# dalek-cryptography/curve25519-dalek

Hardware: NVIDIA H100
Metric: Pippenger MSM points/sec (higher is better)
Workload: dtype exact integers: f64 limbs (radix 2^51, FP64 pipe) in the bucket kernel, u32 limbs (radix 2^25.5) elsewhere

## Files before the change

curve25519_dalek_b200/csrc/api.cu:

```cuda
#include <cstring>
#include <new>
#include <random>

#include "../../include/dalek_b200.h"
#include "engine.h"

extern "C" {

int dalek_b200_init(int device, dalek_b200_ctx **out)
{
    if (!out) return DALEK_E_INVALID_ARG;
    *out = nullptr;
    int count = 0;
    if (cudaGetDeviceCount(&count) != cudaSuccess || count <= 0 || device < 0 || device >= count) return DALEK_E_NO_DEVICE;
    cudaDeviceProp prop;
    if (cudaGetDeviceProperties(&prop, device) != cudaSuccess) return DALEK_E_NO_DEVICE;
    if (prop.major != 9 || prop.minor != 0) return DALEK_E_NO_DEVICE;
    if (cudaSetDevice(device) != cudaSuccess) return DALEK_E_CUDA;
    dalek_b200_ctx *ctx = new (std::nothrow) dalek_b200_ctx();
    if (!ctx) return DALEK_E_NOMEM;
    ctx->device = device;
    ctx->sm_count = prop.multiProcessorCount;
    try { std::random_device rd; for (int i = 0; i < 4; i++) ctx->hash_seed[i] ^= rd(); } catch (...) { }
    int prio_lo = 0, prio_hi = 0;
    cudaDeviceGetStreamPriorityRange(&prio_lo, &prio_hi);
    if (cudaStreamCreateWithPriority(&ctx->stream, cudaStreamNonBlocking, prio_hi) != cudaSuccess ||
        cudaStreamCreateWithPriority(&ctx->stream2, cudaStreamNonBlocking, prio_lo) != cudaSuccess ||
        cudaStreamCreateWithFlags(&ctx->stream_copy, cudaStreamNonBlocking) != cudaSuccess ||
        cudaStreamCreateWithPriority(&ctx->stream3, cudaStreamNonBlocking, prio_hi) != cudaSuccess ||
        cudaStreamCreateWithPriority(&ctx->stream_hash, cudaStreamNonBlocking, prio_hi) != cudaSuccess ||
        cudaEventCreate(&ctx->ev_a) != cudaSuccess || cudaEventCreate(&ctx->ev_b) != cudaSuccess ||
        cudaEventCreate(&ctx->ev_call0) != cudaSuccess || cudaEventCreate(&ctx->ev_call1) != cudaSuccess ||
        cudaEventCreateWithFlags(&ctx->ev_fork, cudaEventDisableTiming) != cudaSuccess ||
        cudaEventCreateWithFlags(&ctx->ev_join, cudaEventDisableTiming) != cudaSuccess ||
        cudaEventCreateWithFlags(&ctx->ev_join2, cudaEventDisableTiming) != cudaSuccess) {
        delete ctx;
        return DALEK_E_CUDA;
    }
    for (int i = 0; i < 8; i++)
        if (cudaEventCreateWithFlags(&ctx->ev_grp[i], cudaEventDisableTiming) != cudaSuccess ||
            cudaEventCreateWithFlags(&ctx->ev_hram[i], cudaEventDisableTiming) != cudaSuccess || cudaEventCreate(&ctx->ev_prep[i][0]) != cudaSuccess ||
            cudaEventCreate(&ctx->ev_prep[i][1]) != cudaSuccess) { delete ctx; return DALEK_E_CUDA; }
    *out = ctx;
    return DALEK_OK;
}

void dalek_b200_destroy(dalek_b200_ctx *ctx)
{
    if (!ctx) return;
    cudaSetDevice(ctx->device);
    cudaStreamSynchronize(ctx->stream);
    cudaStreamSynchronize(ctx->stream2);
    cudaStreamSynchronize(ctx->stream3);
    cudaStreamSynchronize(ctx->stream_hash);
    DevBuf *bufs[] = {&ctx->scalars, &ctx->points_in, &ctx->points, &ctx->digits, &ctx->counts, &ctx->offsets,
                      &ctx->sorted, &ctx->buckets, &ctx->red_a, &ctx->red_b, &ctx->red_c, &ctx->red_d, &ctx->key_pts,
                      &ctx->result, &ctx->flags, &ctx->misc0, &ctx->misc1, &ctx->misc2, &ctx->misc3,
                      &ctx->misc4, &ctx->misc5, &ctx->zs, &ctx->base_table, &ctx->ntasks, &ctx->task_off, &ctx->tasks, &ctx->task_sums, &ctx->msg_offs, &ctx->sum_desc, &ctx->sum_part, &ctx->key_table, &ctx->key_acc, &ctx->task_order, &ctx->sig_status, &ctx->misc6, &ctx->each_pow, &ctx->each_tab, &ctx->each_kstat, &ctx->comb_base_table, &ctx->prep_prod, &ctx->mb_ws[0], &ctx->mb_ws[1]};
    for (DevBuf *b : bufs) if (b->p) cudaFree(b->p);
    if (ctx->h_pinned) cudaFreeHost(ctx->h_pinned);
    cudaEventDestroy(ctx->ev_a); cudaEventDestroy(ctx->ev_b); cudaEventDestroy(ctx->ev_fork); cudaEventDestroy(ctx->ev_join);
    cudaEventDestroy(ctx->ev_join2); cudaEventDestroy(ctx->ev_call0); cudaEventDestroy(ctx->ev_call1);
    for (int i = 0; i < 8; i++) { cudaEventDestroy(ctx->ev_grp[i]); cudaEventDestroy(ctx->ev_hram[i]); cudaEventDestroy(ctx->ev_prep[i][0]); cudaEventDestroy(ctx->ev_prep[i][1]); }
    cudaStreamDestroy(ctx->stream_hash);
    cudaStreamDestroy(ctx->stream); cudaStreamDestroy(ctx->stream2); cudaStreamDestroy(ctx->stream_copy); cudaStreamDestroy(ctx->stream3);
    delete ctx;
}

const char *dalek_b200_last_error(const dalek_b200_ctx *ctx) { return ctx ? ctx->last_error.c_str() : "null context"; }

int dalek_b200_set_option(dalek_b200_ctx *ctx, const char *name, long value)
{
    if (!ctx || !name) return DALEK_E_INVALID_ARG;
    if (!strcmp(name, "window_bits")) { if (value != 0 && (value < 4 || value > 20)) return DALEK_E_INVALID_ARG; ctx->opt_window_bits = value; return 0; }
    if (!strcmp(name, "host_chunks")) { if (value < 1 || value > 8) return DALEK_E_INVALID_ARG; ctx->opt_host_chunks = value; return 0; }
    if (!strcmp(name, "decompress_f64")) { ctx->opt_decompress_f64 = value ? 1 : 0; return 0; }
    if (!strcmp(name, "trace")) { ctx->opt_trace = value ? 1 : 0; return 0; }
    if (!strcmp(name, "precomp_tables")) { ctx->opt_precomp_tables = value ? 1 : 0; return 0; }
    if (!strcmp(name, "double_base_comb")) { ctx->opt_double_base_comb = value ? 1 : 0; return 0; }
    if (!strcmp(name, "dedupe_keys")) { ctx->opt_dedupe_keys = value ? 1 : 0; return 0; }
    if (!strcmp(name, "verify_pieces")) { if (value < 1 || value > 8) return DALEK_E_INVALID_ARG; ctx->opt_verify_pieces = value; return 0; }
    if (!strcmp(name, "transcript_warp")) { ctx->opt_transcript_warp = value ? 1 : 0; return 0; }
    if (!strcmp(name, "transcript_blocks")) { ctx->opt_transcript_blocks = value ? 1 : 0; return 0; }
    if (!strcmp(name, "each_comb")) { if (value < 0 || value > 2) return DALEK_E_INVALID_ARG; ctx->opt_each_comb = value; return 0; }
    if (!strcmp(name, "small_straus")) { ctx->opt_small_straus = value ? 1 : 0; return 0; }
    if (!strcmp(name, "acc_tma")) { ctx->opt_acc_tma = value ? 1 : 0; return 0; }
    if (!strcmp(name, "field_f64")) { ctx->opt_field_f64 = value ? 1 : 0; return 0; }
    if (!strcmp(name, "verify_chunk")) { if (value < 0 || value > (1 << 20)) return DALEK_E_INVALID_ARG; ctx->opt_verify_chunk = value; return 0; }
    return DALEK_E_INVALID_ARG;
}

uint64_t dalek_b200_launch_count(const dalek_b200_ctx *ctx) { return ctx ? ctx->launches : 0; }

int dalek_b200_last_kernel_ms(const dalek_b200_ctx *ctx, float *ms, int *launches)
{
    if (!ctx) return DALEK_E_INVALID_ARG;
    if (ms) *ms = ctx->last_kernel_ms;
    if (launches) *launches = ctx->last_kernel_launches;
    return 0;
}

int dalek_b200_last_stage_ms(const dalek_b200_ctx *ctx, const char *stage, float *ms)
{
    if (!ctx || !stage || !ms) return DALEK_E_INVALID_ARG;
    if (!strcmp(stage, "bucket_accumulate")) { *ms = ctx->last_kernel_ms; return 0; }
    if (!strcmp(stage, "decompress_R")) { *ms = ctx->last_prep_ms; return 0; }
    return DALEK_E_INVALID_ARG;
}

int dalek_b200_last_call_ms(const dalek_b200_ctx *ctx, float *ms)
{
    if (!ctx || !ms) return DALEK_E_INVALID_ARG;
    *ms = ctx->last_call_ms;
    return 0;
}

}

static int run_msm(dalek_b200_ctx *ctx, const void *scalars, const void *points_in, bool on_device, int point_fmt, size_t n,
                   size_t n_window ,
                   ge_p3_raw *d_windows, MsmResult *d_result)
{
    int rc;
    const size_t pin = msm_point_bytes(point_fmt);
    cudaStream_t st = ctx->stream;
    const int c = msm_choose_window_bits(ctx, n_window);
    const bool straus = d_result && n == n_window && n < STRAUS_VT_THRESHOLD && ctx->opt_small_straus && ctx->opt_field_f64;
    const int kind = msm_prepared_kind(point_fmt, straus ? PK_PNIELS : PK_NIELS);
    const size_t psz = kind == PK_NIELS ? sizeof(ge_niels_packed) : sizeof(ge_pniels_packed);
    if ((rc = ws_reserve(ctx, ctx->points, std::max<size_t>(1, n) * psz))) return rc;
    if ((rc = ws_reserve(ctx, ctx->flags, 64))) return rc;
    CUDA_TRY(ctx, cudaMemsetAsync(ctx->flags.p, 0, 64, st));
    if (on_device) {
        if (straus) {
            if ((rc = msm_prepare_points(ctx, points_in, point_fmt, n, ctx->points.p, (int *)ctx->flags.p, kind))) return rc;
            if ((rc = straus_vartime_msm(ctx, (const uint32_t *)scalars, ctx->points.p, kind, n, d_result))) return rc;
        } else {
            CUDA_TRY(ctx, cudaEventRecord(ctx->ev_fork, st));
            CUDA_TRY(ctx, cudaStreamWaitEvent(ctx->stream2, ctx->ev_fork, 0));
            if ((rc = msm_prepare_points_on(ctx, ctx->stream2, points_in, point_fmt, n, ctx->points.p, (int *)ctx->flags.p))) return rc;
            CUDA_TRY(ctx, cudaEventRecord(ctx->ev_join, ctx->stream2));
            if ((rc = msm_accumulate_chunk(ctx, (const uint32_t *)scalars, (const ge_niels_packed *)ctx->points.p, n, c, true, 0, 0, ctx->ev_join))) return rc;
        }
    } else {
        if ((rc = ws_reserve(ctx, ctx->scalars, std::max<size_t>(1, n) * 32))) return rc;
        if ((rc = ws_reserve(ctx, ctx->points_in, std::max<size_t>(1, n) * pin))) return rc;
        int K = n >= (1u << 18) ? (int)std::min<long>(8, std::max<long>(1, ctx->opt_host_chunks)) : 1;
        CUDA_TRY(ctx, cudaEventRecord(ctx->ev_fork, st));
        CUDA_TRY(ctx, cudaStreamWaitEvent(ctx->stream_copy, ctx->ev_fork, 0));
        CUDA_TRY(ctx, cudaStreamWaitEvent(ctx->stream2, ctx->ev_fork, 0));
        for (int k = 0; k < K; k++) {
            const size_t i0 = n * k / K, i1 = n * (k + 1) / K, cnt = i1 - i0;
            char *ds = (char *)ctx->scalars.p + i0 * 32, *dp = (char *)ctx->points_in.p + i0 * pin;
            if (cnt) {
                CUDA_TRY(ctx, cudaMemcpyAsync(ds, (const char *)scalars + i0 * 32, cnt * 32, cudaMemcpyHostToDevice, ctx->stream_copy));
                CUDA_TRY(ctx, cudaMemcpyAsync(dp, (const char *)points_in + i0 * pin, cnt * pin, cudaMemcpyHostToDevice, ctx->stream_copy));
            }
            CUDA_TRY(ctx, cudaEventRecord(ctx->ev_grp[k], ctx->stream_copy));
            CUDA_TRY(ctx, cudaStreamWaitEvent(st, ctx->ev_grp[k], 0));
            char *dq = (char *)ctx->points.p + i0 * psz;
            if (straus) {
                if ((rc = msm_prepare_points(ctx, dp, point_fmt, cnt, dq, (int *)ctx->flags.p, kind))) return rc;
                if ((rc = straus_vartime_msm(ctx, (const uint32_t *)ds, dq, kind, cnt, d_result))) return rc;
            } else {
                CUDA_TRY(ctx, cudaStreamWaitEvent(ctx->stream2, ctx->ev_grp[k], 0));
                if ((rc = msm_prepare_points_on(ctx, ctx->stream2, dp, point_fmt, cnt, dq, (int *)ctx->flags.p))) return rc;
                CUDA_TRY(ctx, cudaEventRecord(ctx->ev_join, ctx->stream2));
                if ((rc = msm_accumulate_chunk(ctx, (const uint32_t *)ds, (const ge_niels_packed *)dq, cnt, c, k == 0, 0, 0, ctx->ev_join))) return rc;
            }
        }
    }
    if (!straus && (rc = msm_reduce_finish(ctx, c, d_windows, d_result))) return rc;
    return 0;
}

int msm_read_result(dalek_b200_ctx *ctx, const MsmResult *d_result, const int *d_bad, const uint32_t *d_enc,
                    uint8_t out_compressed[32], uint64_t out_limbs[20])
{
    int rc;
    cudaStream_t st = ctx->stream;
    if ((rc = pinned_reserve(ctx, sizeof(MsmResult) + 128))) return rc;
    MsmResult *h = (MsmResult *)ctx->h_pinned;
    int *h_bad = (int *)((char *)ctx->h_pinned + sizeof(MsmResult));
    uint8_t *h_enc = (uint8_t *)ctx->h_pinned + sizeof(MsmResult) + 64;
    CUDA_TRY(ctx, cudaMemcpyAsync(h, d_result, sizeof(MsmResult), cudaMemcpyDeviceToHost, st));
    CUDA_TRY(ctx, cudaMemcpyAsync(h_bad, d_bad, sizeof(int), cudaMemcpyDeviceToHost, st));
    if (d_enc) CUDA_TRY(ctx, cudaMemcpyAsync(h_enc, d_enc, 32, cudaMemcpyDeviceToHost, st));
    CUDA_TRY(ctx, cudaStreamSynchronize(st));
    float ms = 0.f;
    if ((ms = elapsed_ms(ctx->ev_a, ctx->ev_b)) >= 0.f) ctx->last_kernel_ms = ms;
    if (out_compressed) memcpy(out_compressed, d_enc ? h_enc : (const uint8_t *)h->compressed, 32);
    if (out_limbs) memcpy(out_limbs, h->limbs, 160);
    return *h_bad ? DALEK_NONE : DALEK_OK;
}

int msm_whole(dalek_b200_ctx *ctx, const void *scalars, const void *points, bool on_device, int point_fmt, size_t n,
              uint8_t out_compressed[32], uint64_t out_limbs[20])
{
    int rc;
    const int nwin = msm_window_count_for_bits(msm_choose_window_bits(ctx, n));
    if ((rc = ws_reserve(ctx, ctx->misc0, (size_t)nwin * sizeof(ge_p3_raw)))) return rc;
    if ((rc = ws_reserve(ctx, ctx->result, sizeof(MsmResult) + 32))) return rc;
    MsmResult *d_res = (MsmResult *)ctx->result.p;
    uint32_t *d_enc = point_fmt == DALEK_POINTS_RISTRETTO ? (uint32_t *)(d_res + 1) : nullptr;
    if ((rc = run_msm(ctx, scalars, points, on_device, point_fmt, n, n, (ge_p3_raw *)ctx->misc0.p, d_res))) return rc;
    if (d_enc && (rc = ristretto_encode_result(ctx, d_res, d_enc))) return rc;
    return msm_read_result(ctx, d_res, (const int *)ctx->flags.p, d_enc, out_compressed, out_limbs);
}

static int msm_common(dalek_b200_ctx *ctx, const void *scalars, const void *points, bool on_device, int point_fmt,
                      size_t n, uint8_t out_compressed[32], uint64_t out_limbs[20])
{
    if (!ctx || (n && (!scalars || !points)) || n >= (1ull << 31)) return DALEK_E_INVALID_ARG;
    CUDA_TRY(ctx, cudaSetDevice(ctx->device));
    CallTimer timer(ctx);
    return msm_whole(ctx, scalars, points, on_device, point_fmt, n, out_compressed, out_limbs);
}

static bool edwards_format(int point_fmt) { return point_fmt == DALEK_POINTS_COMPRESSED || point_fmt == DALEK_POINTS_EXTENDED; }

extern "C" {

int dalek_b200_edwards_vartime_msm(dalek_b200_ctx *ctx, const uint8_t *scalars, const void *points, int point_fmt,
                                   size_t n, uint8_t out_compressed[32], uint64_t out_limbs[20])
{
    if (!edwards_format(point_fmt)) return DALEK_E_INVALID_ARG;
    return msm_common(ctx, scalars, points, false, point_fmt, n, out_compressed, out_limbs);
}

int dalek_b200_edwards_vartime_msm_dev(dalek_b200_ctx *ctx, const void *d_scalars, const void *d_points, int point_fmt,
                                       size_t n, uint8_t out_compressed[32], uint64_t out_limbs[20])
{
    if (!edwards_format(point_fmt)) return DALEK_E_INVALID_ARG;
    return msm_common(ctx, d_scalars, d_points, true, point_fmt, n, out_compressed, out_limbs);
}

int dalek_b200_ristretto_vartime_msm(dalek_b200_ctx *ctx, const uint8_t *scalars, const uint8_t *points, size_t n,
                                     uint8_t out_compressed[32])
{
    if (!out_compressed) return DALEK_E_INVALID_ARG;
    return msm_common(ctx, scalars, points, false, DALEK_POINTS_RISTRETTO, n, out_compressed, nullptr);
}

int dalek_b200_msm_window_count(dalek_b200_ctx *ctx, size_t n_shard)
{
    if (!ctx) return DALEK_E_INVALID_ARG;
    return msm_window_count_for_bits(msm_choose_window_bits(ctx, n_shard));
}

size_t dalek_b200_msm_partial_bytes(dalek_b200_ctx *ctx, size_t n_shard)
{
    if (!ctx) return 0;
    return (size_t)msm_window_count_for_bits(msm_choose_window_bits(ctx, n_shard)) * 160 + 8;
}

void *dalek_b200_stream(dalek_b200_ctx *ctx) { return ctx ? (void *)ctx->stream : nullptr; }

}

__global__ void k_windows_to_record(const ge_p3_raw *__restrict__ win, int nwin, const int *__restrict__ bad, uint64_t *__restrict__ out)
{
    int w = blockIdx.x * blockDim.x + threadIdx.x;
    if (w == nwin) out[20 * (size_t)nwin] = (uint64_t)(*bad != 0);
    if (w >= nwin) return;
    ge_p3 p; ge_p3_raw r = win[w]; ge_p3_load_raw(p, r);
    fe_to_limbs51(out + 20 * w, p.X); fe_to_limbs51(out + 20 * w + 5, p.Y);
    fe_to_limbs51(out + 20 * w + 10, p.Z); fe_to_limbs51(out + 20 * w + 15, p.T);
}
__global__ void k_records_to_windows(const uint64_t *__restrict__ in, int ranks, int nwin, size_t rec_words,
                                     ge_p3_raw *__restrict__ win, int *__restrict__ any_bad)
{
    int t = blockIdx.x * blockDim.x + threadIdx.x;
    if (t >= ranks * nwin) return;
    const int r = t / nwin, w = t % nwin;
    const uint64_t *src = in + (size_t)r * rec_words + 20 * (size_t)w;
    ge_p3 p;
    fe_from_limbs51(p.X, src); fe_from_limbs51(p.Y, src + 5); fe_from_limbs51(p.Z, src + 10); fe_from_limbs51(p.T, src + 15);
    ge_p3_raw o; ge_p3_store_raw(o, p); win[t] = o;
    if (w == 0 && rec_words > 20 * (size_t)nwin && in[(size_t)r * rec_words + 20 * (size_t)nwin]) atomicOr(any_bad, 1);
}

static int partial_enqueue(dalek_b200_ctx *ctx, const void *scalars, const void *points, bool on_device, int point_fmt,
                           size_t n_local, size_t n_shard, int *nwin_out)
{
    if (!ctx || (n_local && (!scalars || !points)) || n_local > n_shard || !edwards_format(point_fmt) || n_local >= (1ull << 31))
        return DALEK_E_INVALID_ARG;
    CUDA_TRY(ctx, cudaSetDevice(ctx->device));
    int rc;
    const int c = msm_choose_window_bits(ctx, n_shard);
    const int nwin = msm_window_count_for_bits(c);
    if ((rc = ws_reserve(ctx, ctx->misc0, (size_t)nwin * sizeof(ge_p3_raw)))) return rc;
    if ((rc = ws_reserve(ctx, ctx->misc1, (size_t)nwin * 160 + 8))) return rc;
    if ((rc = run_msm(ctx, scalars, points, on_device, point_fmt, n_local, n_shard, (ge_p3_raw *)ctx->misc0.p, nullptr))) return rc;
    k_windows_to_record<<<(nwin + 1 + 63) / 64, 64, 0, ctx->stream>>>((const ge_p3_raw *)ctx->misc0.p, nwin, (const int *)ctx->flags.p,
                                                                     (uint64_t *)ctx->misc1.p);
    ctx->launches++;
    CUDA_TRY(ctx, cudaGetLastError());
    *nwin_out = nwin;
    return 0;
}

static void read_kernel_ms(dalek_b200_ctx *ctx)
{
    float ms = 0.f;
    if ((ms = elapsed_ms(ctx->ev_a, ctx->ev_b)) >= 0.f) ctx->last_kernel_ms = ms;
}

static int partial_common(dalek_b200_ctx *ctx, const void *scalars, const void *points, bool on_device, int point_fmt,
                          size_t n_local, size_t n_shard, uint64_t *out_windows)
{
    if (!ctx || !out_windows) return DALEK_E_INVALID_ARG;
    CallTimer timer(ctx);
    int rc, nwin = 0;
    if ((rc = partial_enqueue(ctx, scalars, points, on_device, point_fmt, n_local, n_shard, &nwin))) return rc;
    const size_t bytes = (size_t)nwin * 160 + 8;
    if ((rc = pinned_reserve(ctx, bytes))) return rc;
    CUDA_TRY(ctx, cudaMemcpyAsync(ctx->h_pinned, ctx->misc1.p, bytes, cudaMemcpyDeviceToHost, ctx->stream));
    CUDA_TRY(ctx, cudaStreamSynchronize(ctx->stream));
    read_kernel_ms(ctx);
    memcpy(out_windows, ctx->h_pinned, (size_t)nwin * 160);
    uint64_t status; memcpy(&status, (const char *)ctx->h_pinned + (size_t)nwin * 160, 8);
    return status ? DALEK_NONE : DALEK_OK;
}

int msm_partial_enqueue_record(dalek_b200_ctx *ctx, const void *scalars, const void *points, bool on_device, int point_fmt,
                               size_t n_local, size_t n_shard, void *d_out_record, int dst_device)
{
    if (!ctx || !d_out_record) return DALEK_E_INVALID_ARG;
    CUDA_TRY(ctx, cudaSetDevice(ctx->device));
    CUDA_TRY(ctx, cudaEventRecord(ctx->ev_call0, ctx->stream));
    ctx->async_open = true;
    int rc, nwin = 0;
    if ((rc = partial_enqueue(ctx, scalars, points, on_device, point_fmt, n_local, n_shard, &nwin))) return rc;
    if (dst_device >= 0 && dst_device != ctx->device)
        CUDA_TRY(ctx, cudaMemcpyPeerAsync(d_out_record, dst_device, ctx->misc1.p, ctx->device, (size_t)nwin * 160 + 8, ctx->stream));
    else
        CUDA_TRY(ctx, cudaMemcpyAsync(d_out_record, ctx->misc1.p, (size_t)nwin * 160 + 8, cudaMemcpyDeviceToDevice, ctx->stream));
    return DALEK_OK;
}

int msm_combine_records(dalek_b200_ctx *ctx, const void *records, bool on_device, size_t rec_bytes, int ranks, size_t n_shard,
                        uint8_t out_compressed[32], uint64_t out_limbs[20])
{
    if (!ctx || !records || ranks < 1 || ranks > 1024) return DALEK_E_INVALID_ARG;
    CUDA_TRY(ctx, cudaSetDevice(ctx->device));
    int rc;
    const int c = msm_choose_window_bits(ctx, n_shard);
    const int nwin = msm_window_count_for_bits(c);
    const size_t cnt = (size_t)ranks * nwin;
    if ((rc = ws_reserve(ctx, ctx->red_c, cnt * sizeof(ge_p3_raw)))) return rc;
    if ((rc = ws_reserve(ctx, ctx->flags, 64))) return rc;
    if ((rc = ws_reserve(ctx, ctx->result, sizeof(MsmResult)))) return rc;
    if ((rc = pinned_reserve(ctx, sizeof(MsmResult) + 64))) return rc;
    cudaStream_t st = ctx->stream;
    const void *d_rec = records;
    if (!on_device) {
        if ((rc = ws_reserve(ctx, ctx->red_d, (size_t)ranks * rec_bytes))) return rc;
        CUDA_TRY(ctx, cudaMemcpyAsync(ctx->red_d.p, records, (size_t)ranks * rec_bytes, cudaMemcpyHostToDevice, st));
        d_rec = ctx->red_d.p;
    }
    int *d_bad = (int *)ctx->flags.p + 8;
    CUDA_TRY(ctx, cudaMemsetAsync(d_bad, 0, 4, st));
    k_records_to_windows<<<(unsigned)((cnt + 63) / 64), 64, 0, st>>>((const uint64_t *)d_rec, ranks, nwin, rec_bytes / 8,
                                                                      (ge_p3_raw *)ctx->red_c.p, d_bad);
    ctx->launches++;
    if ((rc = msm_combine_windows(ctx, (const ge_p3_raw *)ctx->red_c.p, ranks, nwin, c, (MsmResult *)ctx->result.p))) return rc;
    MsmResult *h = (MsmResult *)ctx->h_pinned;
    int *h_bad = (int *)((char *)ctx->h_pinned + sizeof(MsmResult));
    CUDA_TRY(ctx, cudaMemcpyAsync(h, ctx->result.p, sizeof(MsmResult), cudaMemcpyDeviceToHost, st));
    CUDA_TRY(ctx, cudaMemcpyAsync(h_bad, d_bad, 4, cudaMemcpyDeviceToHost, st));
    if (ctx->async_open) CUDA_TRY(ctx, cudaEventRecord(ctx->ev_call1, st));
    CUDA_TRY(ctx, cudaStreamSynchronize(st));
    if (ctx->async_open) {
        float ms = 0.f;
        if ((ms = elapsed_ms(ctx->ev_call0, ctx->ev_call1)) >= 0.f) ctx->last_call_ms = ms;
        read_kernel_ms(ctx);
        ctx->async_open = false;
    }
    if (out_compressed) memcpy(out_compressed, h->compressed, 32);
    if (out_limbs) memcpy(out_limbs, h->limbs, 160);
    return *h_bad ? DALEK_NONE : DALEK_OK;
}

extern "C" {

int dalek_b200_edwards_msm_partial(dalek_b200_ctx *ctx, const uint8_t *scalars, const void *points, int point_fmt,
                                   size_t n_local, size_t n_shard, uint64_t *out_windows)
{
    return partial_common(ctx, scalars, points, false, point_fmt, n_local, n_shard, out_windows);
}

int dalek_b200_edwards_msm_partial_dev(dalek_b200_ctx *ctx, const void *d_scalars, const void *d_points, int point_fmt,
                                       size_t n_local, size_t n_shard, uint64_t *out_windows)
{
    return partial_common(ctx, d_scalars, d_points, true, point_fmt, n_local, n_shard, out_windows);
}

int dalek_b200_edwards_msm_partial_async(dalek_b200_ctx *ctx, const uint8_t *scalars, const void *points, int point_fmt,
                                         size_t n_local, size_t n_shard, void *d_out_record)
{
    return msm_partial_enqueue_record(ctx, scalars, points, false, point_fmt, n_local, n_shard, d_out_record, -1);
}

int dalek_b200_edwards_msm_partial_dev_async(dalek_b200_ctx *ctx, const void *d_scalars, const void *d_points, int point_fmt,
                                             size_t n_local, size_t n_shard, void *d_out_record)
{
    return msm_partial_enqueue_record(ctx, d_scalars, d_points, true, point_fmt, n_local, n_shard, d_out_record, -1);
}

int dalek_b200_edwards_msm_combine(dalek_b200_ctx *ctx, const uint64_t *windows, int ranks, size_t n_shard,
                                   uint8_t out_compressed[32], uint64_t out_limbs[20])
{
    if (!ctx) return DALEK_E_INVALID_ARG;
    const size_t rec = (size_t)msm_window_count_for_bits(msm_choose_window_bits(ctx, n_shard)) * 160;
    return msm_combine_records(ctx, windows, false, rec, ranks, n_shard, out_compressed, out_limbs);
}

int dalek_b200_edwards_msm_combine_dev(dalek_b200_ctx *ctx, const void *d_records, int ranks, size_t n_shard,
                                       uint8_t out_compressed[32], uint64_t out_limbs[20])
{
    if (!ctx) return DALEK_E_INVALID_ARG;
    return msm_combine_records(ctx, d_records, true, dalek_b200_msm_partial_bytes(ctx, n_shard), ranks, n_shard, out_compressed, out_limbs);
}

}
```

curve25519_dalek_b200/csrc/engine.h:

```cpp
#pragma once
#include <cuda_runtime.h>
#include <stddef.h>
#include <stdint.h>
#include <cstdio>
#include <string>
#include <utility>
#include <vector>

#include "../../include/dalek_b200.h"
#include "ge.cuh"

struct DevBuf {
    void *p = nullptr;
    size_t cap = 0;
};

struct dalek_b200_ctx {
    int device = 0;
    int sm_count = 132;
    cudaStream_t stream = nullptr;
    cudaStream_t stream2 = nullptr;
    cudaStream_t stream_copy = nullptr;
    cudaStream_t stream3 = nullptr;
    cudaStream_t stream_hash = nullptr;
    cudaEvent_t ev_hram[8] = {};
    cudaEvent_t ev_a = nullptr, ev_b = nullptr, ev_fork = nullptr, ev_join = nullptr, ev_join2 = nullptr;
    cudaEvent_t ev_call0 = nullptr, ev_call1 = nullptr;
    cudaEvent_t ev_prep[8][2] = {};
    int prep_pieces = 0;
    float last_prep_ms = 0.f;
    cudaEvent_t ev_grp[8] = {nullptr, nullptr, nullptr, nullptr, nullptr, nullptr, nullptr, nullptr};
    std::string last_error;
    uint64_t launches = 0;
    long opt_window_bits = 0;
    long opt_verify_chunk = 0;
    long opt_host_chunks = 8;
    long opt_trace = 0;
    long opt_precomp_tables = 0;
    long opt_double_base_comb = 1;
    long opt_dedupe_keys = 1;
    long opt_verify_pieces = 4;
    long opt_decompress_f64 = 1;
    long opt_acc_tma = 0;
    long opt_transcript_warp = 1;
    long opt_transcript_blocks = 1;
    long opt_each_comb = 1;
    long opt_small_straus = 1;
    long opt_field_f64 = 1;
    float last_kernel_ms = 0.f;
    float last_call_ms = 0.f;
    int last_kernel_launches = 0;
    bool async_open = false;
    DevBuf scalars, points_in, points, digits, counts, offsets, sorted, buckets, red_a, red_b, red_c,
        red_d, key_pts, result, flags, misc0, misc1, misc2, misc3, misc4, misc5, zs, base_table, ntasks, task_off, tasks, task_sums, msg_offs, sum_desc, sum_part, key_table, key_acc, task_order, sig_status, misc6, each_pow, each_tab, each_kstat;
    DevBuf prep_prod;
    uint32_t hash_seed[4] = {0x243F6A88u, 0x85A308D3u, 0x13198A2Eu, 0x03707344u};
    int sum_desc_c = -1;
    bool base_table_ready = false;
    bool each_attr_set = false;
    bool comb_attr_set = false;
    DevBuf comb_base_table;
    bool comb_base_table_ready = false;
    DevBuf mb_ws[2];
    void *h_pinned = nullptr;
    size_t h_pinned_cap = 0;
    size_t last_zs_n = 0;
    std::vector<std::pair<const char *, cudaEvent_t>> trace;
};

#define CUDA_TRY(ctx, expr)                                                                      \
    do {                                                                                         \
        cudaError_t _e = (expr);                                                                 \
        if (_e != cudaSuccess) {                                                                 \
            (ctx)->last_error = std::string(#expr) + ": " + cudaGetErrorString(_e);              \
            return -3;                                                                           \
        }                                                                                        \
    } while (0)

inline float elapsed_ms(cudaEvent_t a, cudaEvent_t b)
{
    float ms = 0.f;
    if (cudaEventElapsedTime(&ms, a, b) == cudaSuccess) return ms;
    cudaGetLastError();
    return -1.f;
}

struct CallTimer {
    dalek_b200_ctx *ctx;
    explicit CallTimer(dalek_b200_ctx *c) : ctx(c) { if (ctx) cudaEventRecord(ctx->ev_call0, ctx->stream); }
    ~CallTimer()
    {
        if (!ctx) return;
        float ms = 0.f;
        if (cudaEventRecord(ctx->ev_call1, ctx->stream) == cudaSuccess && cudaEventSynchronize(ctx->ev_call1) == cudaSuccess &&
            (ms = elapsed_ms(ctx->ev_call0, ctx->ev_call1)) >= 0.f)
            ctx->last_call_ms = ms;
    }
};

inline void trace_mark(dalek_b200_ctx *ctx, const char *name, cudaStream_t st)
{
    if (!ctx->opt_trace) return;
    cudaEvent_t e;
    if (cudaEventCreate(&e) != cudaSuccess) return;
    cudaEventRecord(e, st);
    ctx->trace.push_back({name, e});
}
inline void trace_dump(dalek_b200_ctx *ctx)
{
    if (!ctx->opt_trace) return;
    cudaDeviceSynchronize();
    for (auto &m : ctx->trace) {
        float ms = 0.f;
        cudaEventElapsedTime(&ms, ctx->ev_call0, m.second);
        fprintf(stderr, "[trace] %8.3f ms  %s\n", ms, m.first);
        cudaEventDestroy(m.second);
    }
    ctx->trace.clear();
}

inline bool flat_messages_ok(const uint8_t *msgs_flat, const uint64_t *offsets, size_t n)
{
    if (!n) return true;
    if (!offsets || offsets[0] != 0) return false;
    for (size_t i = 0; i < n; i++)
        if (offsets[i] > offsets[i + 1]) return false;
    return msgs_flat || offsets[n] == 0;
}

int ws_reserve(dalek_b200_ctx *ctx, DevBuf &b, size_t bytes);
int pinned_reserve(dalek_b200_ctx *ctx, size_t bytes);

enum { PK_NIELS = 0 , PK_PNIELS = 1  };

inline size_t msm_point_bytes(int point_fmt) { return point_fmt == DALEK_POINTS_EXTENDED ? 160 : 32; }

int msm_prepare_points(dalek_b200_ctx *ctx, const void *d_in, int point_fmt, size_t n, void *d_out,
                       int *d_bad, int kind = PK_NIELS);
int msm_prepared_kind(int point_fmt, int kind);

int msm_choose_window_bits(const dalek_b200_ctx *ctx, size_t n);
int msm_window_count_for_bits(int c);

struct MsmResult { uint32_t compressed[8]; uint64_t limbs[20]; uint32_t is_identity; uint32_t pad; };
int msm_accumulate_chunk(dalek_b200_ctx *ctx, const uint32_t *d_scalars, const ge_niels_packed *d_points, size_t n,
                         int c, bool first, int active_windows = 0, size_t flat = 0, cudaEvent_t points_ready = nullptr);
int msm_prepare_points_on(dalek_b200_ctx *ctx, cudaStream_t st, const void *d_in, int point_fmt, size_t n, void *d_out, int *d_bad,
                          int kind = PK_NIELS);
int msm_choose_window_bits_mixed(const dalek_b200_ctx *ctx, size_t n_short, int short_bits, size_t n_long);
int msm_reduce_finish(dalek_b200_ctx *ctx, int c, ge_p3_raw *d_windows, MsmResult *d_result, bool flat = false);
int msm_combine_windows(dalek_b200_ctx *ctx, const ge_p3_raw *d_windows, int ranks, int nwin, int c,
                        MsmResult *d_result);
int msm_read_result(dalek_b200_ctx *ctx, const MsmResult *d_result, const int *d_bad, const uint32_t *d_enc,
                    uint8_t out_compressed[32], uint64_t out_limbs[20]);

int msm_whole(dalek_b200_ctx *ctx, const void *scalars, const void *points, bool on_device, int point_fmt, size_t n,
              uint8_t out_compressed[32], uint64_t out_limbs[20]);

int msm_partial_enqueue_record(dalek_b200_ctx *ctx, const void *scalars, const void *points, bool on_device, int point_fmt,
                               size_t n_local, size_t n_shard, void *d_out_record, int dst_device);
int msm_combine_records(dalek_b200_ctx *ctx, const void *records, bool on_device, size_t rec_bytes, int ranks, size_t n_shard,
                        uint8_t out_compressed[32], uint64_t out_limbs[20]);

struct EachFront { const uint32_t *hs; const uint8_t *bad_s; const uint32_t *rep, *dense, *uniq; size_t nkeys; };
struct Sha512Prefix;
int verify_each_front(dalek_b200_ctx *ctx, const uint8_t *d_msgs, const uint64_t *d_offs, const uint32_t *d_sigs, const uint32_t *d_keys,
                      size_t n, EachFront *out, const Sha512Prefix *ph_dom = nullptr);

#define STRAUS_VT_THRESHOLD 190
int straus_vartime_msm(dalek_b200_ctx *ctx, const uint32_t *d_scalars, const void *d_points, int point_kind, size_t n,
                       MsmResult *d_result);

int straus_ct_msm(dalek_b200_ctx *ctx, const uint32_t *d_scalars, const void *d_points_pniels, size_t n,
                  MsmResult *d_result);
int base_table_ensure(dalek_b200_ctx *ctx);
#define COMB_BASE_DOUBLES (64 * 8 * 15)
int comb_base_table_ensure(dalek_b200_ctx *ctx);

int ristretto_encode_result(dalek_b200_ctx *ctx, const MsmResult *d_res, uint32_t *d_enc);
```

curve25519_dalek_b200/csrc/msm.cu:

```cuda
#include <algorithm>
#include <cstdio>
#include <utility>
#include <vector>

#include "../../include/dalek_b200.h"
#include "engine.h"
#include "ge64.cuh"
#include "warp4.cuh"
#include "warp4_f64.cuh"

static inline unsigned cdiv(size_t a, unsigned b) { return (unsigned)((a + b - 1) / b); }

int ws_reserve(dalek_b200_ctx *ctx, DevBuf &b, size_t bytes)
{
    if (bytes <= b.cap) return 0;
    if (b.p) { cudaFree(b.p); b.p = nullptr; b.cap = 0; }
    size_t want = bytes + bytes / 8 + 256;
    cudaError_t e = cudaMalloc(&b.p, want);
    if (e != cudaSuccess) { ctx->last_error = std::string("cudaMalloc: ") + cudaGetErrorString(e); return DALEK_E_NOMEM; }
    b.cap = want;
    return 0;
}

int pinned_reserve(dalek_b200_ctx *ctx, size_t bytes)
{
    if (bytes <= ctx->h_pinned_cap) return 0;
    if (ctx->h_pinned) cudaFreeHost(ctx->h_pinned);
    ctx->h_pinned = nullptr; ctx->h_pinned_cap = 0;
    cudaError_t e = cudaMallocHost(&ctx->h_pinned, bytes + 4096);
    if (e != cudaSuccess) { ctx->last_error = std::string("cudaMallocHost: ") + cudaGetErrorString(e); return DALEK_E_NOMEM; }
    ctx->h_pinned_cap = bytes + 4096;
    return 0;
}

template <int F64>
__global__ void __launch_bounds__(128, 3) k_prep_compressed(const uint4 *__restrict__ in, ge_niels_packed *__restrict__ out, size_t n,
                                  int *__restrict__ bad)
{
    size_t i = (size_t)blockIdx.x * blockDim.x + threadIdx.x;
    if (i >= n) return;
    uint4 a = in[2 * i], b = in[2 * i + 1];
    uint32_t s[8] = {a.x, a.y, a.z, a.w, b.x, b.y, b.z, b.w};
    fe x, y;
    uint32_t ok = ge_decompress_affine<F64>(x, y, s);
    if (!ok) { atomicOr(bad, 1); fe_0(x); fe_1(y); }
    ge_niels nl; ge_affine_to_niels(nl, x, y);
    ge_niels_packed p; ge_niels_pack(p, nl);
    uint4 *o = reinterpret_cast<uint4 *>(out + i);
#pragma unroll
    for (int k = 0; k < 6; k++) o[k] = make_uint4(p.w[4 * k], p.w[4 * k + 1], p.w[4 * k + 2], p.w[4 * k + 3]);
}

template <int F64>
__global__ void k_prep_ristretto(const uint32_t *__restrict__ in, ge_niels_packed *__restrict__ out, size_t n, int *__restrict__ bad)
{
    size_t i = (size_t)blockIdx.x * blockDim.x + threadIdx.x;
    if (i >= n) return;
    uint32_t enc[8];
#pragma unroll
    for (int k = 0; k < 8; k++) enc[k] = in[8 * i + k];
    ge_p3 P;
    if (!ristretto_decompress<F64>(P, enc)) { atomicOr(bad, 1); ge_p3_identity(P); }
    ge_niels nl; ge_affine_to_niels(nl, P.X, P.Y);
    ge_niels_packed pk; ge_niels_pack(pk, nl);
    out[i] = pk;
}

#define PREP_THREADS 256
#define PREP_PER_THREAD 4
#define PREP_GROUP (PREP_THREADS * PREP_PER_THREAD)
#define PREP_NW (PREP_THREADS / 32)

__device__ __forceinline__ void load_coord_f64(fe64 &h, const uint64_t *__restrict__ src)
{
    uint64_t l[5];
#pragma unroll
    for (int k = 0; k < 5; k++) l[k] = __ldg(src + k);
    fe t; fe_from_limbs51(t, l);
    fe64_from_fe_limbs(h, t);
}
__device__ __forceinline__ void store_coord(uint4 *o, const fe64 &v, uint32_t ok, uint32_t c)
{
    fe f;
    uint32_t w[8];
    fe64_to_fe(f, v); fe_tobytes_words(w, f);
#pragma unroll
    for (int q = 0; q < 8; q++) w[q] = ok ? w[q] : (q == 0 ? c : 0u);
    o[0] = make_uint4(w[0], w[1], w[2], w[3]);
    o[1] = make_uint4(w[4], w[5], w[6], w[7]);
}
__device__ __forceinline__ uint32_t load_z(fe64 &h, const uint64_t *__restrict__ in, size_t i)
{
    uint64_t l[5];
#pragma unroll
    for (int k = 0; k < 5; k++) l[k] = __ldg(in + 20 * i + 10 + k);
    fe t; fe_from_limbs51(t, l);
    fe64_from_fe_limbs(h, t);
    return 1u - (uint32_t)fe_iszero(t);
}
__device__ __forceinline__ void fe64_shfl_up(fe64 &o, const fe64 &f, int d)
{
#pragma unroll
    for (int k = 0; k < 5; k++) o.v[k] = __shfl_up_sync(0xffffffffu, f.v[k], d);
}
__device__ __forceinline__ void fe64_shfl_down(fe64 &o, const fe64 &f, int d)
{
#pragma unroll
    for (int k = 0; k < 5; k++) o.v[k] = __shfl_down_sync(0xffffffffu, f.v[k], d);
}
__device__ __forceinline__ void fe64_shfl_xor(fe64 &o, const fe64 &f, int m)
{
#pragma unroll
    for (int k = 0; k < 5; k++) o.v[k] = __shfl_xor_sync(0xffffffffu, f.v[k], m);
}
__device__ __forceinline__ void fe64_shfl_idx(fe64 &o, const fe64 &f, int src)
{
#pragma unroll
    for (int k = 0; k < 5; k++) o.v[k] = __shfl_sync(0xffffffffu, f.v[k], src);
}

__device__ __forceinline__ void warp_product(fe64 &p, const fe64 &x, int width)
{
    fe64 t;
    p = x;
#pragma unroll 1
    for (int m = width >> 1; m > 0; m >>= 1) { fe64_shfl_xor(t, p, m); fe64_mul(p, p, t); }
}

__device__ __forceinline__ void warp_other_products(const fe64 &x, fe64 &below, fe64 &above, fe64 &all)
{
    const uint32_t lane = threadIdx.x & 31;
    fe64 lo = x, hi = x, t;
#pragma unroll 1
    for (int d = 1; d < 32; d <<= 1) {
        fe64_shfl_up(t, lo, d);
        if (lane >= (uint32_t)d) fe64_mul(lo, lo, t);
        fe64_shfl_down(t, hi, d);
        if (lane + d < 32) fe64_mul(hi, hi, t);
    }
    fe64_shfl_idx(all, lo, 31);
    fe64_shfl_up(below, lo, 1); if (lane == 0) fe64_1(below);
    fe64_shfl_down(above, hi, 1); if (lane == 31) fe64_1(above);
}

template <bool INVERT>
__device__ __forceinline__ void block_inverse(fe64 &inv, const fe64 &acc, fe64 *s_warp, const fe64 *tot_inv)
{
    const uint32_t lane = threadIdx.x & 31, warp = threadIdx.x >> 5, nw = blockDim.x >> 5;
    fe64 below, above, all;
    warp_other_products(acc, below, above, all);
    if (lane == 0) s_warp[warp] = all;
    __syncthreads();
    if (warp == 0) {
        fe64 x, b, a, t;
        if (lane < nw) x = s_warp[lane]; else fe64_1(x);
        warp_other_products(x, b, a, all);
        if (INVERT) {
            const w20_role r = w20_roles();
            const double inv = w20_invert(w20_limb(all, r.i), r);
#pragma unroll
            for (uint32_t k = 0; k < 5; k++) t.v[k] = w20_shfl(inv, k);
        } else {
            t = *tot_inv;
        }
        fe64_mul(t, t, b); fe64_mul(t, t, a);
        if (lane < nw) s_warp[lane] = t;
    }
    __syncthreads();
    fe64_mul(inv, s_warp[warp], below); fe64_mul(inv, inv, above);
}

__global__ void __launch_bounds__(PREP_THREADS, 2)
k_prep_zprod(const uint64_t *__restrict__ in, fe64 *__restrict__ prod, size_t n)
{
    __shared__ fe64 s_warp[PREP_NW];
    const uint32_t tid = threadIdx.x, lane = tid & 31, warp = tid >> 5;
    const size_t g0 = (size_t)blockIdx.x * PREP_GROUP + tid;
    fe64 z[PREP_PER_THREAD], acc, t;
    uint32_t ok[PREP_PER_THREAD];
#pragma unroll
    for (int k = 0; k < PREP_PER_THREAD; k++) {
        const size_t i = g0 + (size_t)k * PREP_THREADS;
        if (i < n) ok[k] = load_z(z[k], in, i); else { ok[k] = 0; fe64_1(z[k]); }
    }
    acc = z[0];
    if (!ok[0]) fe64_1(acc);
#pragma unroll
    for (int k = 1; k < PREP_PER_THREAD; k++) { fe64_mul(t, acc, z[k]); fe64_cmov(acc, t, ok[k]); }
    warp_product(t, acc, 32);
    if (lane == 0) s_warp[warp] = t;
    __syncthreads();
    if (warp == 0) {
        if (lane < PREP_NW) acc = s_warp[lane]; else fe64_1(acc);
        warp_product(t, acc, PREP_NW);
        if (lane == 0) prod[blockIdx.x] = t;
    }
}

__global__ void __launch_bounds__(PREP_THREADS)
k_prep_invert(fe64 *__restrict__ prod, fe64 *__restrict__ pre, uint32_t G)
{
    __shared__ fe64 s_warp[PREP_NW];
    const uint32_t per = (G + blockDim.x - 1) / blockDim.x, b = min(threadIdx.x * per, G), e = min(b + per, G);
    fe64 acc, inv, t;
    fe64_1(acc);
    for (uint32_t k = b; k < e; k++) { fe64_mul(acc, acc, prod[k]); pre[k] = acc; }
    block_inverse<true>(inv, acc, s_warp, nullptr);
    for (uint32_t k = e; k-- > b;) {
        const fe64 x = prod[k];
        if (k > b) fe64_mul(t, inv, pre[k - 1]); else t = inv;
        prod[k] = t;
        fe64_mul(inv, inv, x);
    }
}

__global__ void __launch_bounds__(PREP_THREADS, 2)
k_prep_finish(const uint64_t *__restrict__ in, const fe64 *__restrict__ ginv, ge_niels_packed *__restrict__ out, size_t n)
{
    __shared__ fe64 s_warp[PREP_NW];
    __shared__ fe64 s_pre[PREP_PER_THREAD - 1][PREP_THREADS];
    const uint32_t tid = threadIdx.x;
    const size_t g0 = (size_t)blockIdx.x * PREP_GROUP + tid;
    fe64 acc, inv;
    uint32_t nz = 0;
    fe64_1(acc);
#pragma unroll 1
    for (int k = 0; k < PREP_PER_THREAD; k++) {
        const size_t i = g0 + (size_t)k * PREP_THREADS;
        if (k > 0) s_pre[k - 1][tid] = acc;
        if (i < n) {
            fe64 z, t;
            const uint32_t ok = load_z(z, in, i);
            fe64_mul(t, acc, z); fe64_cmov(acc, t, ok);
            nz |= ok << k;
        }
    }
    block_inverse<false>(inv, acc, s_warp, ginv + blockIdx.x);
#pragma unroll 1
    for (int k = PREP_PER_THREAD - 1; k >= 0; k--) {
        const size_t i = g0 + (size_t)k * PREP_THREADS;
        if (i >= n) continue;
        const uint32_t ok = (nz >> k) & 1u;
        const uint64_t *src = in + 20 * i;
        fe64 X, Y, zi, u, v;
        load_coord_f64(u, src + 10);
        if (k > 0) fe64_mul(zi, inv, s_pre[k - 1][tid]); else zi = inv;
        fe64_mul(v, inv, u); fe64_cmov(inv, v, ok);
        uint4 *o = reinterpret_cast<uint4 *>(out + i);
        load_coord_f64(X, src); load_coord_f64(Y, src + 5);
        fe64_add(u, Y, X); fe64_mul(v, u, zi);
        store_coord(o, v, ok, 1u);
        fe64_sub(u, Y, X); fe64_mul(v, u, zi);
        store_coord(o + 2, v, ok, 1u);
        load_coord_f64(u, src + 15);
        fe64_mul(v, u, zi); fe64_const_2d(u); fe64_mul(v, v, u);
        store_coord(o + 4, v, ok, 0u);
    }
}

__global__ void k_prep_extended_pniels(const uint64_t *__restrict__ in, ge_pniels_packed *__restrict__ out, size_t n)
{
    size_t i = (size_t)blockIdx.x * blockDim.x + threadIdx.x;
    if (i >= n) return;
    const ulonglong2 *src = reinterpret_cast<const ulonglong2 *>(in + 20 * i);
    uint64_t l[20];
#pragma unroll
    for (int k = 0; k < 10; k++) { ulonglong2 v = src[k]; l[2 * k] = v.x; l[2 * k + 1] = v.y; }
    ge_p3 p;
    fe_from_limbs51(p.X, l); fe_from_limbs51(p.Y, l + 5); fe_from_limbs51(p.Z, l + 10); fe_from_limbs51(p.T, l + 15);
    ge_pniels pn; ge_p3_to_pniels(pn, p);
    ge_pniels_packed pk; ge_pniels_pack(pk, pn);
    uint4 *o = reinterpret_cast<uint4 *>(out + i);
#pragma unroll
    for (int k = 0; k < 8; k++) o[k] = make_uint4(pk.w[4 * k], pk.w[4 * k + 1], pk.w[4 * k + 2], pk.w[4 * k + 3]);
}

int msm_prepared_kind(int point_fmt, int kind)
{
    return point_fmt == DALEK_POINTS_EXTENDED ? kind : PK_NIELS;
}

int msm_prepare_points_on(dalek_b200_ctx *ctx, cudaStream_t st, const void *d_in, int point_fmt, size_t n, void *d_out, int *d_bad,
                          int kind)
{
    if (n == 0) return 0;
    if (point_fmt == DALEK_POINTS_COMPRESSED) {
        if (ctx->opt_decompress_f64) k_prep_compressed<1><<<cdiv(n, 128), 128, 0, st>>>((const uint4 *)d_in, (ge_niels_packed *)d_out, n, d_bad);
        else k_prep_compressed<0><<<cdiv(n, 128), 128, 0, st>>>((const uint4 *)d_in, (ge_niels_packed *)d_out, n, d_bad);
    } else if (point_fmt == DALEK_POINTS_RISTRETTO) {
        if (ctx->opt_decompress_f64) k_prep_ristretto<1><<<cdiv(n, 128), 128, 0, st>>>((const uint32_t *)d_in, (ge_niels_packed *)d_out, n, d_bad);
        else k_prep_ristretto<0><<<cdiv(n, 128), 128, 0, st>>>((const uint32_t *)d_in, (ge_niels_packed *)d_out, n, d_bad);
    } else if (kind == PK_PNIELS) {
        k_prep_extended_pniels<<<cdiv(n, 128), 128, 0, st>>>((const uint64_t *)d_in, (ge_pniels_packed *)d_out, n);
    } else {
        const unsigned G = cdiv(n, PREP_GROUP);
        int rc;
        if ((rc = ws_reserve(ctx, ctx->prep_prod, 2 * (size_t)G * sizeof(fe64)))) return rc;
        fe64 *prod = (fe64 *)ctx->prep_prod.p;
        k_prep_zprod<<<G, PREP_THREADS, 0, st>>>((const uint64_t *)d_in, prod, n);
        k_prep_invert<<<1, PREP_THREADS, 0, st>>>(prod, prod + G, G);
        k_prep_finish<<<G, PREP_THREADS, 0, st>>>((const uint64_t *)d_in, prod, (ge_niels_packed *)d_out, n);
        ctx->launches += 2;
    }
    ctx->launches++;
    CUDA_TRY(ctx, cudaGetLastError());
    return 0;
}

int msm_prepare_points(dalek_b200_ctx *ctx, const void *d_in, int point_fmt, size_t n, void *d_out, int *d_bad, int kind)
{
    return msm_prepare_points_on(ctx, ctx->stream, d_in, point_fmt, n, d_out, d_bad, kind);
}

int msm_window_count_for_bits(int c) { return 256 / c + 1; }

int msm_choose_window_bits(const dalek_b200_ctx *ctx, size_t n)
{
    if (ctx->opt_window_bits >= 4 && ctx->opt_window_bits <= 20) return (int)ctx->opt_window_bits;
    int best = 4; double best_cost = 1e300;
    for (int c = 4; c <= 20; c++) {
        double W = (double)((253 + c - 1) / c);
        double cost = W * ((double)n + 4.0 * (double)(1u << (c - 1)));
        if (cost < best_cost) { best_cost = cost; best = c; }
    }
    return best;
}

int msm_choose_window_bits_mixed(const dalek_b200_ctx *ctx, size_t n_short, int short_bits, size_t n_long)
{
    if (ctx->opt_window_bits >= 4 && ctx->opt_window_bits <= 20) return (int)ctx->opt_window_bits;
    int best = 4; double best_cost = 1e300;
    for (int c = 4; c <= 20; c++) {
        double W = (double)((253 + c - 1) / c), Ws = (double)((short_bits + 1 + c - 1) / c);
        double cost = Ws * (double)n_short + W * ((double)n_long + 4.0 * (double)(1u << (c - 1)));
        if (cost < best_cost) { best_cost = cost; best = c; }
    }
    return best;
}

#define SORT_THREADS 512
#define SORT_COUNT_TILE 4096u
#define SORT_TILE 2048u
#define SORT_HIST_MAX 8192u
#define SORT_NC_MAX 4096u
#define SORT_FINE_MAX 12
#define SORT_BIN_MEAN 4096u
#define SORT_FINE_CAP 8192u

__device__ __forceinline__ int32_t next_digit(uint32_t s[8], uint32_t &carry, int c)
{
    const uint32_t v = (s[0] & ((1u << c) - 1)) + carry;
#pragma unroll
    for (int k = 0; k < 7; k++) s[k] = __funnelshift_r(s[k], s[k + 1], c);
    s[7] >>= c;
    if (v > (1u << (c - 1))) { carry = 1; return (int32_t)v - (int32_t)(1u << c); }
    carry = 0;
    return (int32_t)v;
}

__device__ __forceinline__ void load_scalar(uint32_t s[8], const uint4 *__restrict__ scalars, size_t i)
{
    const uint4 a = scalars[2 * i], b = scalars[2 * i + 1];
    s[0] = a.x; s[1] = a.y; s[2] = a.z; s[3] = a.w; s[4] = b.x; s[5] = b.y; s[6] = b.z; s[7] = b.w;
}

__device__ uint32_t block_excl_scan(uint32_t *v, uint32_t len, uint32_t *scr)
{
    const uint32_t t = threadIdx.x, lane = t & 31, wid = t >> 5, nw = blockDim.x >> 5;
    const uint32_t per = (len + blockDim.x - 1) / blockDim.x, b = min(t * per, len), e = min(b + per, len);
    __syncthreads();
    uint32_t sum = 0;
    for (uint32_t k = b; k < e; k++) sum += v[k];
    uint32_t incl = sum;
    for (int d = 1; d < 32; d <<= 1) { uint32_t x = __shfl_up_sync(0xffffffffu, incl, d); if (lane >= (uint32_t)d) incl += x; }
    if (lane == 31) scr[wid] = incl;
    __syncthreads();
    if (wid == 0) {
        const uint32_t x = lane < nw ? scr[lane] : 0;
        uint32_t y = x;
        for (int d = 1; d < 32; d <<= 1) { uint32_t z = __shfl_up_sync(0xffffffffu, y, d); if (lane >= (uint32_t)d) y += z; }
        if (lane < nw) scr[lane] = y - x;
        if (lane == 31) scr[32] = y;
    }
    __syncthreads();
    uint32_t run = scr[wid] + incl - sum;
    for (uint32_t k = b; k < e; k++) { const uint32_t x = v[k]; v[k] = run; run += x; }
    const uint32_t total = scr[32];
    __syncthreads();
    return total;
}

__device__ __forceinline__ uint32_t warp_claim(uint32_t *ctr, uint32_t key, bool live)
{
    const uint32_t lane = threadIdx.x & 31;
    const uint32_t peers = __match_any_sync(0xffffffffu, live ? key : 0xffffffffu);
    const uint32_t leader = __ffs(peers) - 1;
    uint32_t base = 0;
    if (live && lane == leader) base = atomicAdd(&ctr[key], (uint32_t)__popc(peers));
    base = __shfl_sync(0xffffffffu, base, leader);
    return base + __popc(peers & ((1u << lane) - 1));
}

__global__ void __launch_bounds__(SORT_THREADS)
k_sort_count(const uint4 *__restrict__ scalars, size_t n, int c, int nact, int F, uint32_t nc, int flat,
             uint32_t *__restrict__ ccount)
{
    __shared__ uint32_t h[SORT_HIST_MAX];
    const uint32_t nh = (flat ? 1u : (uint32_t)nact) * nc;
    for (uint32_t k = threadIdx.x; k < nh; k += SORT_THREADS) h[k] = 0;
    __syncthreads();
    for (uint32_t j = 0; j < SORT_COUNT_TILE / SORT_THREADS; j++) {
        const size_t i = (size_t)blockIdx.x * SORT_COUNT_TILE + j * SORT_THREADS + threadIdx.x;
        if (i >= n) break;
        uint32_t s[8], carry = 0;
        load_scalar(s, scalars, i);
        for (int w = 0; w < nact; w++) {
            const int32_t d = next_digit(s, carry, c);
            if (d) atomicAdd(&h[(flat ? 0u : (uint32_t)w * nc) + (((uint32_t)(d < 0 ? -d : d) - 1) >> F)], 1u);
        }
    }
    __syncthreads();
    for (uint32_t k = threadIdx.x; k < nh; k += SORT_THREADS)
        if (h[k]) atomicAdd(&ccount[k], h[k]);
}

__device__ __forceinline__ uint32_t extra_slices(uint32_t cnt) { return cnt > SORT_FINE_CAP ? (cnt - 1) / SORT_FINE_CAP : 0; }

__global__ void __launch_bounds__(SORT_THREADS)
k_sort_bins_scan(const uint32_t *__restrict__ ccount, uint32_t nc, int F, uint32_t nbuckets, uint32_t *__restrict__ ccursor,
                 uint32_t *__restrict__ xpre, uint32_t *__restrict__ xtot, uint32_t *__restrict__ counts,
                 uint32_t *__restrict__ fill)
{
    __shared__ uint32_t v[SORT_NC_MAX], scr[33];
    const size_t o = (size_t)blockIdx.x * nc;
    for (uint32_t k = threadIdx.x; k < nc; k += SORT_THREADS) v[k] = ccount[o + k];
    block_excl_scan(v, nc, scr);
    for (uint32_t k = threadIdx.x; k < nc; k += SORT_THREADS) { ccursor[o + k] = v[k]; v[k] = extra_slices(ccount[o + k]); }
    const uint32_t total = block_excl_scan(v, nc, scr);
    for (uint32_t k = threadIdx.x; k < nc; k += SORT_THREADS) xpre[o + k] = v[k];
    if (threadIdx.x == 0) xtot[blockIdx.x] = total;
    for (uint32_t k = 0; k < nc; k++) {
        if ((k + 1 < nc ? v[k + 1] : total) == v[k]) continue;
        const size_t b0 = (size_t)blockIdx.x * nbuckets + ((size_t)k << F);
        for (uint32_t f = threadIdx.x; f < (1u << F); f += SORT_THREADS) { counts[b0 + f] = 0; fill[b0 + f] = 0; }
    }
}

__global__ void __launch_bounds__(SORT_THREADS, 2)
k_sort_partition(const uint4 *__restrict__ scalars, size_t n, int c, int nact, int F, uint32_t nc, uint32_t nbuckets, size_t flat,
                 const uint32_t *__restrict__ ccount, uint32_t *__restrict__ ccursor, uint2 *__restrict__ records,
                 uint32_t *__restrict__ counts)
{
    constexpr int SPT = SORT_TILE / SORT_THREADS;
    extern __shared__ uint32_t sm[];
    uint2 *stage = reinterpret_cast<uint2 *>(sm);
    uint32_t *cnt = sm + 2 * SORT_TILE, *gbase = cnt + nc, *scr = gbase + nc;
    const uint32_t fmask = (1u << F) - 1;
    uint32_t s[SPT][8], carry[SPT];
    size_t idx[SPT];
#pragma unroll
    for (int j = 0; j < SPT; j++) {
        idx[j] = (size_t)blockIdx.x * SORT_TILE + j * SORT_THREADS + threadIdx.x;
        carry[j] = 0;
        if (idx[j] < n) load_scalar(s[j], scalars, idx[j]);
        else for (int k = 0; k < 8; k++) s[j][k] = 0;
    }
    for (int w = 0; w < nact; w++) {
        const uint32_t wb = flat ? 0u : (uint32_t)w;
        for (uint32_t k = threadIdx.x; k < nc; k += SORT_THREADS) cnt[k] = 0;
        __syncthreads();
        uint32_t bkt[SPT], rank[SPT], neg[SPT];
#pragma unroll
        for (int j = 0; j < SPT; j++) {
            const int32_t d = next_digit(s[j], carry[j], c);
            neg[j] = d < 0;
            bkt[j] = d ? (uint32_t)(d < 0 ? -d : d) - 1 : 0xffffffffu;
            if (d) rank[j] = atomicAdd(&cnt[bkt[j] >> F], 1u);
        }
        __syncthreads();
        for (uint32_t k = threadIdx.x; k < nc; k += SORT_THREADS) {
            const uint32_t v = cnt[k];
            gbase[k] = v ? atomicAdd(&ccursor[(size_t)wb * nc + k], v) : 0;
        }
        const uint32_t total = block_excl_scan(cnt, nc, scr);
#pragma unroll
        for (int j = 0; j < SPT; j++) {
            if (bkt[j] == 0xffffffffu) continue;
            const uint32_t cb = bkt[j] >> F;
            const uint32_t val = (flat ? (uint32_t)((size_t)w * flat + idx[j]) : (uint32_t)idx[j]) | (neg[j] << 31);
            stage[cnt[cb] + rank[j]] = make_uint2(val, (bkt[j] & fmask) | (cb << 16));
        }
        __syncthreads();
        uint2 *dst = records + (flat ? (size_t)0 : (size_t)w * n);
        for (uint32_t k0 = 0; k0 < total; k0 += SORT_THREADS) {
            const uint32_t k = k0 + threadIdx.x;
            const uint2 r = k < total ? stage[k] : make_uint2(0, 0);
            const uint32_t cb = r.y >> 16, f = r.y & 0xffffu;
            if (k < total) dst[gbase[cb] + (k - cnt[cb])] = make_uint2(r.x, f);
            const bool big = k < total && ccount[(size_t)wb * nc + cb] > SORT_FINE_CAP;
            if (__any_sync(0xffffffffu, big)) warp_claim(counts + (size_t)wb * nbuckets, (cb << F) | f, big);
        }
        __syncthreads();
    }
}

__global__ void __launch_bounds__(SORT_THREADS, 2)
k_sort_fine(const uint2 *__restrict__ records, const uint32_t *__restrict__ ccount, const uint32_t *__restrict__ ccursor,
            const uint32_t *__restrict__ xpre, const uint32_t *__restrict__ xtot, size_t n, int F, uint32_t nc,
            uint32_t nbuckets, uint32_t nwin, int flat, uint32_t *__restrict__ counts, uint32_t *__restrict__ offsets,
            uint32_t *__restrict__ sorted, uint32_t *__restrict__ fill)
{
    extern __shared__ uint32_t sm[];
    __shared__ uint32_t s_bin, s_slice;
    uint2 *recs = reinterpret_cast<uint2 *>(sm);
    uint32_t *out = sm + 2 * SORT_FINE_CAP, *h = out + SORT_FINE_CAP, *scr = h + (1u << F);
    const uint32_t nf = 1u << F, nbins = nwin * nc;
    uint32_t bin, slice = 0;
    if (blockIdx.x < nbins) {
        bin = nbins - 1 - blockIdx.x;
    } else {
        if (threadIdx.x == 0) {
            uint32_t t = blockIdx.x - nbins, w = 0;
            while (w < nwin && t >= xtot[w]) t -= xtot[w++];
            s_bin = nbins;
            if (w < nwin) {
                const uint32_t *x = xpre + (size_t)w * nc;
                uint32_t lo = 0, hi = nc - 1;
                while (lo < hi) { const uint32_t mid = (lo + hi + 1) / 2; if (x[mid] <= t) lo = mid; else hi = mid - 1; }
                s_bin = w * nc + lo;
                s_slice = t - x[lo] + 1;
            }
        }
        __syncthreads();
        bin = s_bin; slice = s_slice;
        if (bin >= nbins) return;
    }
    const uint32_t wb = bin / nc, cb = bin % nc;
    const uint32_t cnt = ccount[bin], base = ccursor[bin] - cnt;
    const size_t seg = flat ? (size_t)0 : (size_t)wb * n;
    const size_t b0 = (size_t)wb * nbuckets + ((size_t)cb << F);
    const uint2 *src = records + seg + base;
    uint32_t *dst = sorted + seg + base;
    constexpr uint32_t U = 4;
    if (cnt <= SORT_FINE_CAP) {
        for (uint32_t f = threadIdx.x; f < nf; f += SORT_THREADS) h[f] = 0;
        __syncthreads();
        for (uint32_t k0 = 0; k0 < cnt; k0 += U * SORT_THREADS) {
            uint2 r[U];
#pragma unroll
            for (uint32_t u = 0; u < U; u++) {
                const uint32_t k = k0 + u * SORT_THREADS + threadIdx.x;
                r[u] = k < cnt ? src[k] : make_uint2(0, 0);
            }
#pragma unroll
            for (uint32_t u = 0; u < U; u++) {
                const uint32_t k = k0 + u * SORT_THREADS + threadIdx.x;
                if (k < cnt) { recs[k] = r[u]; atomicAdd(&h[r[u].y], 1u); }
            }
        }
        __syncthreads();
        for (uint32_t f = threadIdx.x; f < nf; f += SORT_THREADS) counts[b0 + f] = h[f];
        block_excl_scan(h, nf, scr);
        for (uint32_t f = threadIdx.x; f < nf; f += SORT_THREADS) offsets[b0 + f] = base + h[f];
        __syncthreads();
        for (uint32_t k = threadIdx.x; k < cnt; k += SORT_THREADS) { const uint2 r = recs[k]; out[atomicAdd(&h[r.y], 1u)] = r.x; }
        __syncthreads();
        for (uint32_t k = threadIdx.x; k < cnt; k += SORT_THREADS) dst[k] = out[k];
        return;
    }
    for (uint32_t f = threadIdx.x; f < nf; f += SORT_THREADS) { h[f] = counts[b0 + f]; out[f] = 0; }
    block_excl_scan(h, nf, scr);
    if (slice == 0)
        for (uint32_t f = threadIdx.x; f < nf; f += SORT_THREADS) offsets[b0 + f] = base + h[f];
    const uint32_t lo = slice * SORT_FINE_CAP, m = min(SORT_FINE_CAP, cnt - lo);
    for (uint32_t k0 = 0; k0 < m; k0 += U * SORT_THREADS) {
        uint2 r[U];
#pragma unroll
        for (uint32_t u = 0; u < U; u++) {
            const uint32_t k = k0 + u * SORT_THREADS + threadIdx.x;
            r[u] = k < m ? src[lo + k] : make_uint2(0, 0);
        }
#pragma unroll
        for (uint32_t u = 0; u < U; u++) {
            const uint32_t k = k0 + u * SORT_THREADS + threadIdx.x;
            if (k < m) recs[k] = r[u];
            warp_claim(out, r[u].y, k < m);
        }
    }
    __syncthreads();
    for (uint32_t f = threadIdx.x; f < nf; f += SORT_THREADS)
        if (out[f]) out[f] = h[f] + atomicAdd(&fill[b0 + f], out[f]);
    __syncthreads();
    for (uint32_t k0 = 0; k0 < m; k0 += SORT_THREADS) {
        const uint32_t k = k0 + threadIdx.x;
        const uint2 r = k < m ? recs[k] : make_uint2(0, 0);
        const uint32_t pos = warp_claim(out, r.y, k < m);
        if (k < m) dst[pos] = r.x;
    }
}

#define SCAN_PART 4096u
__global__ void __launch_bounds__(1024) k_scan_partial(const uint32_t *__restrict__ in, uint32_t nbuckets, uint32_t parts,
                                                       uint32_t *__restrict__ part_sums)
{
    __shared__ uint32_t sh[32];
    uint32_t w = blockIdx.x / parts, part = blockIdx.x % parts;
    const uint32_t *src = in + (size_t)w * nbuckets;
    uint32_t base = part * SCAN_PART + threadIdx.x * 4, sum = 0;
#pragma unroll
    for (int k = 0; k < 4; k++) if (base + k < nbuckets) sum += src[base + k];
    for (int d = 16; d > 0; d >>= 1) sum += __shfl_down_sync(0xffffffffu, sum, d);
    if ((threadIdx.x & 31) == 0) sh[threadIdx.x >> 5] = sum;
    __syncthreads();
    if (threadIdx.x < 32) {
        uint32_t v = sh[threadIdx.x];
        for (int d = 16; d > 0; d >>= 1) v += __shfl_down_sync(0xffffffffu, v, d);
        if (threadIdx.x == 0) part_sums[blockIdx.x] = v;
    }
}
__global__ void k_scan_bases(uint32_t *__restrict__ part_sums, uint32_t parts)
{
    if (threadIdx.x) return;
    uint32_t *p = part_sums + (size_t)blockIdx.x * parts, run = 0;
    for (uint32_t k = 0; k < parts; k++) { uint32_t v = p[k]; p[k] = run; run += v; }
}
__global__ void __launch_bounds__(1024) k_scan_apply(const uint32_t *__restrict__ in, const uint32_t *__restrict__ part_base,
                                                     uint32_t nbuckets, uint32_t parts, uint32_t *__restrict__ out)
{
    __shared__ uint32_t sh[32];
    uint32_t w = blockIdx.x / parts, part = blockIdx.x % parts;
    const uint32_t *src = in + (size_t)w * nbuckets;
    uint32_t *dst = out + (size_t)w * nbuckets;
    uint32_t base = part * SCAN_PART + threadIdx.x * 4;
    uint32_t v[4], sum = 0;
#pragma unroll
    for (int k = 0; k < 4; k++) { v[k] = base + k < nbuckets ? src[base + k] : 0; sum += v[k]; }
    uint32_t incl = sum;
    for (int d = 1; d < 32; d <<= 1) { uint32_t t = __shfl_up_sync(0xffffffffu, incl, d); if ((threadIdx.x & 31) >= d) incl += t; }
    if ((threadIdx.x & 31) == 31) sh[threadIdx.x >> 5] = incl;
    __syncthreads();
    if (threadIdx.x < 32) {
        uint32_t x = sh[threadIdx.x], inc2 = x;
        for (int d = 1; d < 32; d <<= 1) { uint32_t t = __shfl_up_sync(0xffffffffu, inc2, d); if (threadIdx.x >= d) inc2 += t; }
        sh[threadIdx.x] = inc2 - x;
    }
    __syncthreads();
    uint32_t run = part_base[blockIdx.x] + sh[threadIdx.x >> 5] + incl - sum;
#pragma unroll
    for (int k = 0; k < 4; k++) { if (base + k < nbuckets) dst[base + k] = run; run += v[k]; }
}

#define TASK_LEN_MIN 64u
static uint32_t msm_task_len(size_t n, int nwin, uint32_t nb)
{
    const size_t total_buckets = (size_t)nwin * nb;
    const size_t want = total_buckets >= ((size_t)1 << 18) ? 2 * (n / nb) : (n * (size_t)nwin) >> 18;
    uint32_t len = TASK_LEN_MIN;
    while (len < want && len < (1u << 22)) len <<= 1;
    return len;
}
#ifndef ACC_MIN_BLOCKS
#define ACC_MIN_BLOCKS 4
#endif

__global__ void k_task_count(const uint32_t *__restrict__ counts, uint32_t total_buckets, uint32_t task_len,
                             uint32_t *__restrict__ ntasks, uint32_t *__restrict__ heavy)
{
    uint32_t t = blockIdx.x * blockDim.x + threadIdx.x;
    if (t >= total_buckets) return;
    uint32_t c = counts[t];
    uint32_t k = c <= task_len ? 1u : (c + task_len - 1) / task_len;
    ntasks[t] = k;
    if (k > 1) heavy[1 + atomicAdd(&heavy[0], 1u)] = t;
}

__global__ void k_task_bases(const uint32_t *__restrict__ ntasks, const uint32_t *__restrict__ task_off, uint32_t nbuckets,
                             int nwin, uint32_t *__restrict__ win_base )
{
    if (blockIdx.x || threadIdx.x) return;
    uint32_t run = 0;
    for (int w = 0; w < nwin; w++) {
        win_base[w] = run;
        size_t last = (size_t)w * nbuckets + nbuckets - 1;
        run += task_off[last] + ntasks[last];
    }
    win_base[nwin] = run;
}

__global__ void k_task_fill(const uint32_t *__restrict__ ntasks, const uint32_t *__restrict__ task_off,
                            const uint32_t *__restrict__ win_base, uint32_t nbuckets, uint32_t total_buckets,
                            uint2 *__restrict__ tasks)
{
    uint32_t t = blockIdx.x * blockDim.x + threadIdx.x;
    if (t >= total_buckets) return;
    uint32_t w = t / nbuckets;
    uint32_t base = win_base[w] + task_off[t], k = ntasks[t];
    for (uint32_t j = 0; j < k; j++) tasks[base + j] = make_uint2(t, j);
}

#define TASK_BINS 256u
__device__ __forceinline__ uint32_t task_key(uint32_t len, uint32_t task_len)
{
    return (uint32_t)(((uint64_t)len * (TASK_BINS - 1) + task_len - 1) / task_len);
}
__device__ __forceinline__ uint32_t task_length(const uint2 tk, const uint32_t *__restrict__ counts, uint32_t task_len)
{
    return min(task_len, counts[tk.x] - tk.y * task_len);
}

__global__ void __launch_bounds__(256)
k_task_hist(const uint2 *__restrict__ tasks, const uint32_t *__restrict__ counts, const uint32_t *__restrict__ total_ptr,
            uint32_t task_len, uint32_t *__restrict__ hist)
{
    __shared__ uint32_t sh[TASK_BINS];
    sh[threadIdx.x] = 0;
    __syncthreads();
    const uint32_t p = blockIdx.x * blockDim.x + threadIdx.x;
    if (p < *total_ptr) atomicAdd(&sh[task_key(task_length(tasks[p], counts, task_len), task_len)], 1u);
    __syncthreads();
    if (sh[threadIdx.x]) atomicAdd(&hist[threadIdx.x], sh[threadIdx.x]);
}

__global__ void __launch_bounds__(256) k_task_scan(const uint32_t *__restrict__ hist, uint32_t *__restrict__ start)
{
    __shared__ uint32_t sh[TASK_BINS];
    const uint32_t k = TASK_BINS - 1 - threadIdx.x;
    sh[threadIdx.x] = hist[k];
    __syncthreads();
    for (uint32_t d = 1; d < TASK_BINS; d <<= 1) {
        uint32_t v = threadIdx.x >= d ? sh[threadIdx.x - d] : 0;
        __syncthreads();
        sh[threadIdx.x] += v;
        __syncthreads();
    }
    start[k] = sh[threadIdx.x] - hist[k];
}

__global__ void __launch_bounds__(256)
k_task_scatter(const uint2 *__restrict__ tasks, const uint32_t *__restrict__ counts, const uint32_t *__restrict__ total_ptr,
               uint32_t task_len, const uint32_t *__restrict__ start, uint32_t *__restrict__ cursor, uint32_t *__restrict__ order)
{
    __shared__ uint32_t cnt[TASK_BINS], base[TASK_BINS];
    cnt[threadIdx.x] = 0;
    __syncthreads();
    const uint32_t p = blockIdx.x * blockDim.x + threadIdx.x;
    const bool live = p < *total_ptr;
    uint32_t key = 0, rank = 0;
    if (live) { key = task_key(task_length(tasks[p], counts, task_len), task_len); rank = atomicAdd(&cnt[key], 1u); }
    __syncthreads();
    if (cnt[threadIdx.x]) base[threadIdx.x] = start[threadIdx.x] + atomicAdd(&cursor[threadIdx.x], cnt[threadIdx.x]);
    __syncthreads();
    if (live) order[base[key] + rank] = p;
}

__device__ __forceinline__ void load_p3(ge_p3 &p, const ge_p3_raw *src)
{
    const uint4 *s = reinterpret_cast<const uint4 *>(src);
    ge_p3_raw r;
#pragma unroll
    for (int q = 0; q < 10; q++) { uint4 v = s[q]; r.w[4 * q] = v.x; r.w[4 * q + 1] = v.y; r.w[4 * q + 2] = v.z; r.w[4 * q + 3] = v.w; }
    ge_p3_load_raw(p, r);
}

template <int F64, int TMA>
__global__ void __launch_bounds__(128, ACC_MIN_BLOCKS)
k_bucket_accumulate(const ge_niels_packed *__restrict__ points, const uint32_t *__restrict__ sorted,
                    const uint32_t *__restrict__ counts, const uint32_t *__restrict__ offsets,
                    const uint32_t *__restrict__ ntasks, const uint2 *__restrict__ tasks, const uint32_t *__restrict__ order,
                    const uint32_t *__restrict__ win_base, int w0, int w1, size_t n, uint32_t nbuckets, uint32_t task_len,
                    ge_p3_raw *__restrict__ buckets, ge_p3_raw *__restrict__ task_sums, int first)
{
    constexpr int NQ = sizeof(ge_niels_packed) / 16;
    constexpr int TSTRIDE = NQ * 16 + 16;
    __shared__ uint4 s_pts[(F64 && !TMA) ? 2 : 1][(F64 && !TMA) ? NQ : 1][(F64 && !TMA) ? 128 : 1];
    __shared__ __align__(16) unsigned char s_bulk[(F64 && TMA) ? 2 : 1][(F64 && TMA) ? 128 : 1][(F64 && TMA) ? TSTRIDE : 16];
    __shared__ __align__(8) unsigned long long s_bar[(F64 && TMA) ? 2 : 1][(F64 && TMA) ? 128 : 1];
    const uint32_t total_tasks = win_base[w1];
    const uint32_t slot = blockIdx.x * 128u + threadIdx.x;
    if (slot >= total_tasks) return;
    const uint32_t p = order[slot];
    const uint2 tk = tasks[p];
    const uint32_t t = tk.x, w = t / nbuckets;
    const uint32_t cnt = counts[t], start = tk.y * task_len;
    const uint32_t len = min(task_len, cnt - start);
    const bool split = ntasks[t] != 1;
    if (!first && len == 0) return;
    const bool fold_old = !first && !split;
    const uint32_t *idx = sorted + (size_t)w * n + offsets[t] + start;
    ge_p3 acc;
    if (F64) {
        ge64_p3 acc64;
        if (fold_old) {
            ge_p3 old; load_p3(old, buckets + t);
            fe64_from_fe(acc64.X, old.X); fe64_from_fe(acc64.Y, old.Y); fe64_from_fe(acc64.Z, old.Z); fe64_from_fe(acc64.T, old.T);
        } else {
            ge64_identity(acc64);
        }
        uint32_t e_next = len ? idx[0] : 0;
        if (TMA) {
            const uint32_t bar0 = (uint32_t)__cvta_generic_to_shared(&s_bar[0][threadIdx.x]);
            const uint32_t bar1 = (uint32_t)__cvta_generic_to_shared(&s_bar[1][threadIdx.x]);
            asm volatile("mbarrier.init.shared::cta.b64 [%0], 1;" ::"r"(bar0) : "memory");
            asm volatile("mbarrier.init.shared::cta.b64 [%0], 1;" ::"r"(bar1) : "memory");
            asm volatile("fence.mbarrier_init.release.cluster;" ::: "memory");
            asm volatile("fence.proxy.async.shared::cta;" ::: "memory");
        }
        auto prefetch = [&](uint32_t e, int buf) {
            const uint32_t pi = e & 0x7fffffffu;
            const char *src = reinterpret_cast<const char *>(points) + (size_t)pi * (NQ * 16);
            if (TMA) {
                const uint32_t bar = (uint32_t)__cvta_generic_to_shared(&s_bar[buf][threadIdx.x]);
                const uint32_t dst = (uint32_t)__cvta_generic_to_shared(&s_bulk[buf][threadIdx.x][0]);
                asm volatile("mbarrier.arrive.expect_tx.shared::cta.b64 _, [%0], %1;" ::"r"(bar), "r"(NQ * 16) : "memory");
                asm volatile("cp.async.bulk.shared::cluster.global.mbarrier::complete_tx::bytes [%0], [%1], %2, [%3];"
                             ::"r"(dst), "l"(src), "r"(NQ * 16), "r"(bar) : "memory");
            } else {
#pragma unroll
                for (int q = 0; q < NQ; q++) {
                    uint32_t dst = (uint32_t)__cvta_generic_to_shared(&s_pts[buf][q][threadIdx.x]);
                    asm volatile("cp.async.cg.shared.global [%0], [%1], 16;" ::"r"(dst), "l"(src + 16 * q) : "memory");
                }
            }
        };
        if (len) prefetch(e_next, 0);
        if (!TMA) asm volatile("cp.async.commit_group;" ::: "memory");
        for (uint32_t k = 0; k < len; k++) {
            const uint32_t e = e_next, neg = e >> 31;
            const int buf = k & 1;
            if (k + 1 < len) { e_next = idx[k + 1]; prefetch(e_next, buf ^ 1); }
            uint32_t words[NQ * 4];
            if (TMA) {
                const uint32_t bar = (uint32_t)__cvta_generic_to_shared(&s_bar[buf][threadIdx.x]);
                const uint32_t parity = (k >> 1) & 1u;
                uint32_t done;
                do {
                    asm volatile("{ .reg .pred p; mbarrier.try_wait.parity.shared::cta.b64 p, [%1], %2; selp.u32 %0, 1, 0, p; }"
                                 : "=r"(done) : "r"(bar), "r"(parity) : "memory");
                } while (!done);
                const uint4 *sp = reinterpret_cast<const uint4 *>(&s_bulk[buf][threadIdx.x][0]);
#pragma unroll
                for (int q = 0; q < NQ; q++) { uint4 v = sp[q]; words[4 * q] = v.x; words[4 * q + 1] = v.y; words[4 * q + 2] = v.z; words[4 * q + 3] = v.w; }
            } else {
                asm volatile("cp.async.commit_group;" ::: "memory");
                asm volatile("cp.async.wait_group 1;" ::: "memory");
#pragma unroll
                for (int q = 0; q < NQ; q++) { uint4 v = s_pts[buf][q][threadIdx.x]; words[4 * q] = v.x; words[4 * q + 1] = v.y; words[4 * q + 2] = v.z; words[4 * q + 3] = v.w; }
            }
            ge_niels_packed pk;
#pragma unroll
            for (int q = 0; q < 24; q++) pk.w[q] = words[q];
            ge64_niels nl; ge64_niels_unpack(nl, pk);
            ge64_madd(acc64, acc64, nl, neg);
        }
        ge64_to_p3(acc, acc64);
    } else {
    if (fold_old) load_p3(acc, buckets + t); else ge_p3_identity(acc);
    for (uint32_t k = 0; k < len; k++) {
        uint32_t e = idx[k];
        uint32_t neg = e >> 31, pi = e & 0x7fffffffu;
        const uint4 *src = reinterpret_cast<const uint4 *>(reinterpret_cast<const ge_niels_packed *>(points) + pi);
        ge_niels_packed pk;
#pragma unroll
        for (int q = 0; q < 6; q++) { uint4 v = __ldg(src + q); pk.w[4 * q] = v.x; pk.w[4 * q + 1] = v.y; pk.w[4 * q + 2] = v.z; pk.w[4 * q + 3] = v.w; }
        ge_niels nl; ge_niels_unpack(nl, pk);
        ge_madd(acc, acc, nl, neg);
    }
    }
    ge_p3_raw r; ge_p3_store_raw(r, acc);
    uint4 *o = reinterpret_cast<uint4 *>(!split ? buckets + t : task_sums + p);
#pragma unroll
    for (int q = 0; q < 10; q++) o[q] = make_uint4(r.w[4 * q], r.w[4 * q + 1], r.w[4 * q + 2], r.w[4 * q + 3]);
}


__global__ void __launch_bounds__(128)
k_heavy_fixup(const uint32_t *__restrict__ heavy, const uint32_t *__restrict__ ntasks, const uint32_t *__restrict__ task_off,
              const uint32_t *__restrict__ win_base, uint32_t nbuckets, uint32_t w0, uint32_t w1,
              const ge_p3_raw *__restrict__ task_sums, ge_p3_raw *__restrict__ buckets, int first)
{
    const uint32_t lane = threadIdx.x & 31, role = lane & 3, grp = lane >> 2;
    const uint32_t nwarps = (gridDim.x * blockDim.x) >> 5;
    const uint32_t nheavy = heavy[0];
    for (uint32_t h = (blockIdx.x * blockDim.x + threadIdx.x) >> 5; h < nheavy; h += nwarps) {
        uint32_t tb = heavy[1 + h];
        if (tb / nbuckets < w0 || tb / nbuckets >= w1) continue;
        uint32_t kk = ntasks[tb];
        uint32_t base = win_base[tb / nbuckets] + task_off[tb];
        w4_point acc, x;
        if (first || grp != 0) w4_identity(acc); else w4_load(acc, buckets + tb);
        for (uint32_t j0 = 0; j0 < kk; j0 += 8) {
            uint32_t j = j0 + grp;
            if (j < kk) w4_load(x, task_sums + base + j); else w4_identity(x);
            w4_add(acc, x, role);
        }
        for (int d = 16; d >= 4; d >>= 1) { w4_shfl_down(x, acc, d); w4_add(acc, x, role); }
        if (grp == 0) w4_store(buckets + tb, acc, role);
    }
}

__device__ __forceinline__ void load_p3_f64(ge64_p3 &o, const ge_p3_raw *src)
{
    ge_p3 q; load_p3(q, src);
    fe64_from_fe_limbs(o.X, q.X); fe64_from_fe_limbs(o.Y, q.Y); fe64_from_fe_limbs(o.Z, q.Z); fe64_from_fe_limbs(o.T, q.T);
}

__global__ void __launch_bounds__(32)
k_chunk_reduce_f64(const ge_p3_raw *__restrict__ S_in, uint32_t n_in, uint32_t m, uint32_t n_out, uint32_t nwin,
                   ge_p3_raw *__restrict__ S_out, ge_p3_raw *__restrict__ W_out)
{
    const uint32_t t = blockIdx.x * blockDim.x + threadIdx.x;
    if (t >= n_out * nwin) return;
    const uint32_t w = t / n_out, q = t % n_out;
    const ge_p3_raw *S = S_in + (size_t)w * n_in + (size_t)q * m;
    fe64 d2; fe64_const_2d(d2);
    ge64_p3 run, acc, x;
    load_p3_f64(run, S + (m - 1));
    acc = run;
    ge_p3 nxt;
    if (m > 1) load_p3(nxt, S + (m - 2));
#pragma unroll 1
    for (uint32_t r = m - 1; r-- > 0;) {
        fe64_from_fe_limbs(x.X, nxt.X); fe64_from_fe_limbs(x.Y, nxt.Y); fe64_from_fe_limbs(x.Z, nxt.Z); fe64_from_fe_limbs(x.T, nxt.T);
        if (r > 0) load_p3(nxt, S + (r - 1));
        ge64_add_p3(run, run, x, d2);
        ge64_add_p3(acc, acc, run, d2);
    }
    ge_p3 o; ge_p3_raw raw;
    ge64_to_p3(o, run); ge_p3_store_raw(raw, o);
    uint4 *d = reinterpret_cast<uint4 *>(S_out + t);
#pragma unroll
    for (int k = 0; k < 10; k++) d[k] = make_uint4(raw.w[4 * k], raw.w[4 * k + 1], raw.w[4 * k + 2], raw.w[4 * k + 3]);
    ge64_to_p3(o, acc); ge_p3_store_raw(raw, o);
    d = reinterpret_cast<uint4 *>(W_out + t);
#pragma unroll
    for (int k = 0; k < 10; k++) d[k] = make_uint4(raw.w[4 * k], raw.w[4 * k + 1], raw.w[4 * k + 2], raw.w[4 * k + 3]);
}

__global__ void __launch_bounds__(128)
k_chunk_reduce(const ge_p3_raw *__restrict__ S_in, uint32_t n_in, uint32_t m, uint32_t one_based, uint32_t n_out,
               uint32_t nwin, ge_p3_raw *__restrict__ S_out, ge_p3_raw *__restrict__ W_out)
{
    const uint32_t t = (blockIdx.x * blockDim.x + threadIdx.x) >> 5;
    if (t >= n_out * nwin) return;
    const w20_role rl = w20_roles();
    const double d2 = w20_const_2d(rl);
    const uint32_t w = t / n_out, q = t % n_out;
    const ge_p3_raw *S = S_in + (size_t)w * n_in + (size_t)q * m;
    double run = w20_load(S + (m - 1), rl), acc = run;
#pragma unroll 1
    for (uint32_t r = m - 1; r-- > 1;) {
        w20_add(run, w20_load(S + r, rl), d2, rl);
        w20_add(acc, run, d2, rl);
    }
    if (m > 1) {
        w20_add(run, w20_load(S, rl), d2, rl);
        if (one_based) w20_add(acc, run, d2, rl);
    } else if (!one_based) {
        acc = w20_identity(rl);
    }
    w20_store(S_out + t, run);
    w20_store(W_out + t, acc);
}

#define SUM_PIECE 256u
__global__ void __launch_bounds__(128)
k_plain_sum(const ge_p3_raw *__restrict__ pool, const uint2 *__restrict__ desc, ge_p3_raw *__restrict__ out)
{
    __shared__ ge_p3_raw sh[32];
    const uint32_t role = threadIdx.x & 3, grp = threadIdx.x >> 2;
    const uint2 d = desc[blockIdx.x];
    const ge_p3_raw *a = pool + d.x;
    const uint32_t len = d.y;
    w4_point acc, x;
    w4_identity(acc);
    for (uint32_t i0 = 0; i0 < len; i0 += 32) {
        uint32_t i = i0 + grp;
        if (i < len) w4_load(x, a + i); else w4_identity(x);
        w4_add(acc, x, role);
    }
    w4_store(&sh[grp], acc, role);
    __syncthreads();
    for (uint32_t d = 16; d > 0; d >>= 1) {
        if (threadIdx.x < 32 * ((d + 7) / 8)) {
            uint32_t g2 = grp < d ? grp + d : grp;
            w4_load(acc, &sh[grp]); w4_load(x, &sh[g2]);
            w4_add(acc, x, role);
        }
        __syncthreads();
        if (grp < d) w4_store(&sh[grp], acc, role);
        __syncthreads();
    }
    if (grp == 0) { w4_load(acc, &sh[0]); w4_store(out + blockIdx.x, acc, role); }
}

struct LevelInfo { int nlevels; int log2m[16]; };
__global__ void __launch_bounds__(128)
k_finish_windows(const ge_p3_raw *__restrict__ S_top, const ge_p3_raw *__restrict__ A, LevelInfo li, uint32_t nwin,
                 ge_p3_raw *__restrict__ out)
{
    const uint32_t w = (blockIdx.x * blockDim.x + threadIdx.x) >> 5;
    if (w >= nwin) return;
    const w20_role rl = w20_roles();
    double t;
    if (li.nlevels > 0) {
        const double d2 = w20_const_2d(rl);
        t = w20_load(A + (size_t)(li.nlevels - 1) * nwin + w, rl);
#pragma unroll 1
        for (int l = li.nlevels - 2; l >= 0; l--) {
#pragma unroll 1
            for (int k = 0; k < li.log2m[l]; k++) w20_dbl(t, rl);
            w20_add(t, w20_load(A + (size_t)l * nwin + w, rl), d2, rl);
        }
    } else {
        t = w20_load(S_top + w, rl);
    }
    w20_store(out + w, t);
}

__global__ void __launch_bounds__(32)
k_combine(const ge_p3_raw *__restrict__ windows, int ranks, int nwin, int c, MsmResult *__restrict__ res)
{
    const w20_role r = w20_roles();
    uint32_t s[8];
    ge_p3 total;
    w20_encode(s, total, w20_horner(windows, ranks, nwin, c, r), r);
    if (threadIdx.x != 0) return;
#pragma unroll
    for (int i = 0; i < 8; i++) res->compressed[i] = s[i];
    fe_to_limbs51(res->limbs, total.X); fe_to_limbs51(res->limbs + 5, total.Y);
    fe_to_limbs51(res->limbs + 10, total.Z); fe_to_limbs51(res->limbs + 15, total.T);
    res->is_identity = ge_is_identity(total);
    res->pad = 0;
}

static int msm_sort_fine_bits(size_t entries_per_window, int c, int hist_windows)
{
    int lg = std::max(0, c - 1 - SORT_FINE_MAX);
    while (lg < c - 1 && ((size_t)SORT_BIN_MEAN << lg) < entries_per_window && (2u << lg) <= SORT_NC_MAX &&
           ((size_t)hist_windows << (lg + 1)) <= SORT_HIST_MAX)
        lg++;
    return c - 1 - lg;
}

int msm_accumulate_chunk(dalek_b200_ctx *ctx, const uint32_t *d_scalars, const ge_niels_packed *d_points, size_t n,
                         int c, bool first, int active_windows, size_t flat, cudaEvent_t points_ready)
{
    const int nwin_d = msm_window_count_for_bits(c);
    const int nact = active_windows > 0 && active_windows < nwin_d ? active_windows : nwin_d;
    const int nwin = flat ? 1 : nwin_d;
    const uint32_t nb = 1u << (c - 1);
    const size_t total_buckets = (size_t)nwin * nb;
    const uint32_t task_len = flat ? msm_task_len(n * (size_t)nact, 1, nb) : msm_task_len(n, nact, nb);
    const size_t max_tasks = total_buckets + (std::max<size_t>(1, n) * nact) / task_len + 1;
    const size_t max_heavy = (std::max<size_t>(1, n) * nact) / task_len + 1;
    const uint32_t parts = (nb + SCAN_PART - 1) / SCAN_PART;
    const int F = msm_sort_fine_bits(flat ? n * (size_t)nact : n, c, flat ? 1 : nact);
    const uint32_t nc = nb >> F;
    cudaStream_t st = ctx->stream;
    int rc;
    if ((rc = ws_reserve(ctx, ctx->counts, (total_buckets + (size_t)nwin * nc + 1 + max_heavy) * 4))) return rc;
    if ((rc = ws_reserve(ctx, ctx->offsets, (total_buckets + (size_t)nwin * parts + 2 * (size_t)nwin * nc + nwin) * 4))) return rc;
    if ((rc = ws_reserve(ctx, ctx->ntasks, total_buckets * 4))) return rc;
    if ((rc = ws_reserve(ctx, ctx->task_off, total_buckets * 4 + (nwin + 1) * 4))) return rc;
    if ((rc = ws_reserve(ctx, ctx->tasks, max_tasks * 8))) return rc;
    if ((rc = ws_reserve(ctx, ctx->task_sums, max_tasks * sizeof(ge_p3_raw)))) return rc;
    if ((rc = ws_reserve(ctx, ctx->task_order, (3 * TASK_BINS + max_tasks) * 4))) return rc;
    if ((rc = ws_reserve(ctx, ctx->digits, std::max<size_t>(1, n) * nact * 8))) return rc;
    if ((rc = ws_reserve(ctx, ctx->sorted, std::max<size_t>(1, n) * nact * 4))) return rc;
    if ((rc = ws_reserve(ctx, ctx->buckets, total_buckets * sizeof(ge_p3_raw)))) return rc;
    uint32_t *counts = (uint32_t *)ctx->counts.p, *offsets = (uint32_t *)ctx->offsets.p;
    uint32_t *ntasks = (uint32_t *)ctx->ntasks.p, *task_off = (uint32_t *)ctx->task_off.p;
    uint32_t *win_base = task_off + total_buckets;
    uint32_t *ccount = counts + total_buckets, *heavy = ccount + (size_t)nwin * nc;
    uint32_t *part_sums = offsets + total_buckets, *ccursor = part_sums + (size_t)nwin * parts;
    uint32_t *xpre = ccursor + (size_t)nwin * nc, *xtot = xpre + (size_t)nwin * nc;
    uint2 *tasks = (uint2 *)ctx->tasks.p;
    uint32_t *t_hist = (uint32_t *)ctx->task_order.p, *t_cursor = t_hist + TASK_BINS, *t_start = t_cursor + TASK_BINS;
    uint32_t *order = t_start + TASK_BINS;
    ge_p3_raw *task_sums = (ge_p3_raw *)ctx->task_sums.p;
    uint2 *records = (uint2 *)ctx->digits.p;
    uint32_t *sorted = (uint32_t *)ctx->sorted.p;
    ge_p3_raw *buckets = (ge_p3_raw *)ctx->buckets.p;

    const size_t part_smem = SORT_TILE * 8 + (2 * (size_t)nc + 33) * 4;
    const size_t fine_smem = SORT_FINE_CAP * 12 + ((1u << F) + 33) * 4;
    CUDA_TRY(ctx, cudaFuncSetAttribute(k_sort_partition, cudaFuncAttributeMaxDynamicSharedMemorySize, (int)part_smem));
    CUDA_TRY(ctx, cudaFuncSetAttribute(k_sort_fine, cudaFuncAttributeMaxDynamicSharedMemorySize, (int)fine_smem));
    CUDA_TRY(ctx, cudaMemsetAsync(ccount, 0, ((size_t)nwin * nc + 1) * 4, st));
    CUDA_TRY(ctx, cudaMemsetAsync(t_hist, 0, 2 * TASK_BINS * 4, st));
    if (n) {
        k_sort_count<<<cdiv(n, SORT_COUNT_TILE), SORT_THREADS, 0, st>>>((const uint4 *)d_scalars, n, c, nact, F, nc, flat ? 1 : 0, ccount);
        ctx->launches++;
    }
    k_sort_bins_scan<<<nwin, SORT_THREADS, 0, st>>>(ccount, nc, F, nb, ccursor, xpre, xtot, counts, ntasks);
    if (n) {
        k_sort_partition<<<cdiv(n, SORT_TILE), SORT_THREADS, part_smem, st>>>((const uint4 *)d_scalars, n, c, nact, F, nc, nb, flat,
                                                                              ccount, ccursor, records, counts);
        ctx->launches++;
    }
    const size_t extra = n * (size_t)nact / SORT_FINE_CAP;
    k_sort_fine<<<(unsigned)(nwin * nc + extra), SORT_THREADS, fine_smem, st>>>(records, ccount, ccursor, xpre, xtot, n, F, nc, nb,
                                                                               (uint32_t)nwin, flat ? 1 : 0, counts, offsets, sorted, ntasks);
    k_task_count<<<cdiv(total_buckets, 256), 256, 0, st>>>(counts, (uint32_t)total_buckets, task_len, ntasks, heavy);
    k_scan_partial<<<nwin * parts, 1024, 0, st>>>(ntasks, nb, parts, part_sums);
    k_scan_bases<<<nwin, 32, 0, st>>>(part_sums, parts);
    k_scan_apply<<<nwin * parts, 1024, 0, st>>>(ntasks, part_sums, nb, parts, task_off);
    k_task_bases<<<1, 32, 0, st>>>(ntasks, task_off, nb, nwin, win_base);
    k_task_fill<<<cdiv(total_buckets, 256), 256, 0, st>>>(ntasks, task_off, win_base, nb, (uint32_t)total_buckets, tasks);
    k_task_hist<<<cdiv(max_tasks, 256), 256, 0, st>>>(tasks, counts, win_base + nwin, task_len, t_hist);
    k_task_scan<<<1, 256, 0, st>>>(t_hist, t_start);
    k_task_scatter<<<cdiv(max_tasks, 256), 256, 0, st>>>(tasks, counts, win_base + nwin, task_len, t_start, t_cursor, order);
    ctx->launches += 11;
    if (points_ready) CUDA_TRY(ctx, cudaStreamWaitEvent(st, points_ready, 0));
    if (first) CUDA_TRY(ctx, cudaEventRecord(ctx->ev_a, st));
    {
        const unsigned grid = cdiv(max_tasks, 128);
        const int f = first ? 1 : 0;
#define LAUNCH_ACC(F64_, TMA_) k_bucket_accumulate<F64_, TMA_><<<grid, 128, 0, st>>>(d_points, sorted, counts, offsets, ntasks, tasks, order, win_base, 0, nwin, n, nb, task_len, buckets, task_sums, f)
        const bool tma = ctx->opt_field_f64 && ctx->opt_acc_tma;
        if (tma) LAUNCH_ACC(1, 1); else if (ctx->opt_field_f64) LAUNCH_ACC(1, 0); else LAUNCH_ACC(0, 0);
#undef LAUNCH_ACC
        k_heavy_fixup<<<ctx->sm_count * 4, 128, 0, st>>>(heavy, ntasks, task_off, win_base, nb, 0u, (uint32_t)nwin, task_sums, buckets, f);
        ctx->launches += 2;
    }
    CUDA_TRY(ctx, cudaEventRecord(ctx->ev_b, st));
    ctx->last_kernel_launches = first ? 1 : ctx->last_kernel_launches + 1;
    CUDA_TRY(ctx, cudaGetLastError());
    return 0;
}

int msm_reduce_finish(dalek_b200_ctx *ctx, int c, ge_p3_raw *d_windows, MsmResult *d_result, bool flat)
{
    const int nwin = flat ? 1 : msm_window_count_for_bits(c);
    const int desc_key = c + (flat ? 64 : 0);
    const uint32_t nb = 1u << (c - 1);
    cudaStream_t st = ctx->stream;
    int rc;
    ge_p3_raw *buckets = (ge_p3_raw *)ctx->buckets.p;
    LevelInfo li; li.nlevels = 0;
    std::vector<uint32_t> lvl_m, lvl_nout;
    size_t pool_pts = 0;
    {
        uint32_t n_in = nb; bool first = true;
        while (n_in > 1) {
            uint32_t m = first ? std::min<uint32_t>(n_in, 16) : std::min<uint32_t>(n_in, 8);
            uint32_t n_out = (n_in + m - 1) / m;
            lvl_m.push_back(m); lvl_nout.push_back(n_out);
            int lg = 0; while ((1u << lg) < m) lg++;
            li.log2m[li.nlevels++] = lg;
            pool_pts += 2 * (size_t)n_out * nwin;
            n_in = n_out; first = false;
        }
    }
    if ((rc = ws_reserve(ctx, ctx->red_a, std::max<size_t>(1, pool_pts) * sizeof(ge_p3_raw)))) return rc;
    if ((rc = ws_reserve(ctx, ctx->red_b, (size_t)16 * nwin * sizeof(ge_p3_raw)))) return rc;
    ge_p3_raw *pool = (ge_p3_raw *)ctx->red_a.p, *A = (ge_p3_raw *)ctx->red_b.p;
    const ge_p3_raw *S_in = buckets;
    uint32_t n_in = nb;
    size_t pos = 0;
    std::vector<std::pair<size_t, uint32_t>> w_arrays;
    for (int l = 0; l < li.nlevels; l++) {
        uint32_t m = lvl_m[l], n_out = lvl_nout[l];
        ge_p3_raw *S_out = pool + pos, *W_out = pool + pos + (size_t)n_out * nwin;
        if (l == 0 && ctx->opt_field_f64 && n_in % m == 0)
            k_chunk_reduce_f64<<<cdiv((size_t)n_out * nwin, 32), 32, 0, st>>>(S_in, n_in, m, n_out, nwin, S_out, W_out);
        else
            k_chunk_reduce<<<cdiv((size_t)n_out * nwin * 32, 128), 128, 0, st>>>(S_in, n_in, m, l == 0 ? 1u : 0u, n_out, nwin, S_out, W_out);
        ctx->launches++;
        w_arrays.push_back({pos + (size_t)n_out * nwin, n_out});
        S_in = S_out; n_in = n_out; pos += 2 * (size_t)n_out * nwin;
    }
    {
        std::vector<uint2> d1, d2;
        for (int l = 0; l < li.nlevels; l++)
            for (int w = 0; w < nwin; w++) {
                uint32_t off = (uint32_t)(w_arrays[l].first + (size_t)w * w_arrays[l].second), len = w_arrays[l].second;
                uint32_t first_piece = (uint32_t)d1.size();
                for (uint32_t o = 0; o < len; o += SUM_PIECE) d1.push_back(make_uint2(off + o, std::min(SUM_PIECE, len - o)));
                d2.push_back(make_uint2(first_piece, (uint32_t)d1.size() - first_piece));
            }
        const size_t n1 = d1.size(), n2 = d2.size();
        if ((rc = ws_reserve(ctx, ctx->sum_desc, (n1 + n2) * sizeof(uint2)))) return rc;
        if ((rc = ws_reserve(ctx, ctx->sum_part, n1 * sizeof(ge_p3_raw)))) return rc;
        uint2 *dd1 = (uint2 *)ctx->sum_desc.p, *dd2 = dd1 + n1;
        if (ctx->sum_desc_c != desc_key) {
            CUDA_TRY(ctx, cudaMemcpyAsync(dd1, d1.data(), n1 * sizeof(uint2), cudaMemcpyHostToDevice, st));
            CUDA_TRY(ctx, cudaMemcpyAsync(dd2, d2.data(), n2 * sizeof(uint2), cudaMemcpyHostToDevice, st));
            CUDA_TRY(ctx, cudaStreamSynchronize(st));
            ctx->sum_desc_c = desc_key;
        }
        ge_p3_raw *parts = (ge_p3_raw *)ctx->sum_part.p;
        k_plain_sum<<<(unsigned)n1, 128, 0, st>>>(pool, dd1, parts);
        k_plain_sum<<<(unsigned)n2, 128, 0, st>>>(parts, dd2, A);
        ctx->launches += 2;
    }
    k_finish_windows<<<cdiv((size_t)nwin * 32, 128), 128, 0, st>>>(S_in, A, li, nwin, d_windows);
    ctx->launches++;
    if (d_result) {
        k_combine<<<1, 32, 0, st>>>(d_windows, 1, nwin, c, d_result);
        ctx->launches++;
    }
    CUDA_TRY(ctx, cudaGetLastError());
    return 0;
}

int msm_combine_windows(dalek_b200_ctx *ctx, const ge_p3_raw *d_windows, int ranks, int nwin, int c, MsmResult *d_result)
{
    k_combine<<<1, 32, 0, ctx->stream>>>(d_windows, ranks, nwin, c, d_result);
    ctx->launches++;
    CUDA_TRY(ctx, cudaGetLastError());
    return 0;
}
```

curve25519_dalek_b200/engine.py:

```python
import ctypes as C
import os

HERE = os.path.dirname(os.path.abspath(__file__))
POINTS_RISTRETTO = 2
POINTS_COMPRESSED = 0
POINTS_EXTENDED = 1

_lib = None


def library_path():
    return os.environ.get("DALEK_B200_LIB") or os.path.join(HERE, "libdalek_b200.so")


def load_library():
    global _lib
    if _lib is not None:
        return _lib
    path = library_path()
    if not os.path.exists(path):
        raise RuntimeError("libdalek_b200.so is missing: run `python -m curve25519_dalek_b200.build` "
                           "(or __graft_entry__.build()); there is no CPU fallback")
    lib = C.CDLL(path)
    vp, sz, u8p, u64p = C.c_void_p, C.c_size_t, C.c_char_p, C.c_void_p
    lib.dalek_b200_init.argtypes = [C.c_int, C.POINTER(vp)]
    lib.dalek_b200_destroy.argtypes = [vp]
    lib.dalek_b200_destroy.restype = None
    lib.dalek_b200_last_error.argtypes = [vp]
    lib.dalek_b200_last_error.restype = C.c_char_p
    lib.dalek_b200_set_option.argtypes = [vp, C.c_char_p, C.c_long]
    lib.dalek_b200_launch_count.argtypes = [vp]
    lib.dalek_b200_launch_count.restype = C.c_uint64
    lib.dalek_b200_last_kernel_ms.argtypes = [vp, C.POINTER(C.c_float), C.POINTER(C.c_int)]
    lib.dalek_b200_last_call_ms.argtypes = [vp, C.POINTER(C.c_float)]
    lib.dalek_b200_last_stage_ms.argtypes = [vp, C.c_char_p, C.POINTER(C.c_float)]
    for name in ("dalek_b200_edwards_vartime_msm", "dalek_b200_edwards_ct_msm", "dalek_b200_edwards_vartime_msm_dev"):
        getattr(lib, name).argtypes = [vp, vp, vp, C.c_int, sz, vp, vp]
    lib.dalek_b200_msm_window_count.argtypes = [vp, sz]
    lib.dalek_b200_edwards_msm_partial.argtypes = [vp, vp, vp, C.c_int, sz, sz, vp]
    lib.dalek_b200_edwards_msm_partial_dev.argtypes = [vp, vp, vp, C.c_int, sz, sz, vp]
    lib.dalek_b200_edwards_msm_combine.argtypes = [vp, vp, C.c_int, sz, vp, vp]
    lib.dalek_b200_edwards_msm_combine_dev.argtypes = [vp, vp, C.c_int, sz, vp, vp]
    lib.dalek_b200_edwards_msm_partial_async.argtypes = [vp, vp, vp, C.c_int, sz, sz, vp]
    lib.dalek_b200_edwards_msm_partial_dev_async.argtypes = [vp, vp, vp, C.c_int, sz, sz, vp]
    lib.dalek_b200_msm_partial_bytes.argtypes = [vp, sz]
    lib.dalek_b200_msm_partial_bytes.restype = sz
    lib.dalek_b200_stream.argtypes = [vp]
    lib.dalek_b200_stream.restype = vp
    lib.dalek_b200_init_multi.argtypes = [C.POINTER(C.c_int), C.c_int, C.POINTER(vp)]
    lib.dalek_b200_destroy_multi.argtypes = [vp]
    lib.dalek_b200_destroy_multi.restype = None
    lib.dalek_b200_multi_device_count.argtypes = [vp]
    lib.dalek_b200_multi_ctx.argtypes = [vp, C.c_int]
    lib.dalek_b200_multi_ctx.restype = vp
    lib.dalek_b200_multi_last_error.argtypes = [vp]
    lib.dalek_b200_multi_last_error.restype = C.c_char_p
    lib.dalek_b200_edwards_vartime_msm_multi.argtypes = [vp, vp, vp, C.c_int, sz, vp, vp]
    lib.dalek_b200_ristretto_double_base_batch.argtypes = [vp, vp, vp, vp, vp, sz, vp]
    lib.dalek_b200_ristretto_vartime_msm.argtypes = [vp, vp, vp, sz, vp]
    lib.ed25519_b200_verify_batch.argtypes = [vp, vp, vp, vp, vp, sz]
    lib.ed25519_b200_verify_batch_flat.argtypes = [vp, vp, vp, vp, vp, sz]
    lib.ed25519_b200_verify_batch_flat_dev.argtypes = [vp, vp, vp, vp, vp, sz, sz]
    lib.ed25519_b200_verify_batches_flat.argtypes = [vp, vp, vp, vp, vp, sz, sz, vp]
    lib.ed25519_b200_verify_batch_flat_points.argtypes = [vp, vp, vp, vp, vp, vp, sz]
    lib.ed25519_b200_verify_batch_flat_points_dev.argtypes = [vp, vp, vp, vp, vp, vp, sz]
    lib.ed25519_b200_verify_batches_flat_points.argtypes = [vp, vp, vp, vp, vp, vp, sz, sz, vp]
    lib.ed25519_b200_verify_batches_flat_points_dev.argtypes = [vp, vp, vp, vp, vp, vp, sz, sz, vp]
    lib.ed25519_b200_verify_batches_flat_dev.argtypes = [vp, vp, vp, vp, vp, sz, sz, vp]
    lib.dalek_b200_precomp_new.argtypes = [vp, vp, C.c_int, sz, C.POINTER(vp)]
    lib.dalek_b200_precomp_len.argtypes = [vp]
    lib.dalek_b200_precomp_len.restype = sz
    lib.dalek_b200_precomp_destroy.argtypes = [vp]
    lib.dalek_b200_precomp_destroy.restype = None
    lib.dalek_b200_precomp_mixed_msm.argtypes = [vp, vp, vp, sz, vp, vp, C.c_int, sz, vp, vp]
    lib.dalek_b200_edwards_decompress_batch.argtypes = [vp, vp, sz, vp, vp]
    lib.dalek_b200_ristretto_decompress_batch.argtypes = [vp, vp, sz, vp, vp]
    lib.dalek_b200_edwards_compress_batch.argtypes = [vp, vp, sz, vp]
    lib.dalek_b200_ristretto_double_and_compress_batch.argtypes = [vp, vp, sz, vp]
    lib.ed25519_b200_verify_each_flat.argtypes = [vp, vp, vp, vp, vp, sz, C.c_int, vp]
    lib.ed25519_b200_verify_each_flat_dev.argtypes = [vp, vp, vp, vp, vp, sz, C.c_int, vp]
    lib.dalek_b200_scalar_from_wide_batch.argtypes = [vp, vp, sz, vp]
    lib.dalek_b200_scalar_invert_batch.argtypes = [vp, vp, sz, vp, vp]
    lib.ed25519_b200_last_zs.argtypes = [vp, vp, sz]
    lib.dalek_b200_edwards_mul_base_batch.argtypes = [vp, vp, sz, vp, vp]
    lib.ed25519_b200_sign_batch_flat.argtypes = [vp, vp, vp, vp, sz, vp, vp]
    lib.ed25519_b200_verifying_keys.argtypes = [vp, vp, sz, vp]
    lib.ed25519_b200_sign_flat.argtypes = [vp, vp, sz, vp, vp, sz, vp]
    lib.ed25519_b200_sign_prehashed.argtypes = [vp, vp, sz, vp, sz, vp, sz, vp]
    lib.ed25519_b200_verify_prehashed_each.argtypes = [vp, vp, vp, sz, vp, vp, sz, C.c_int, vp]
    lib.dalek_b200_edwards_to_montgomery_batch.argtypes = [vp, vp, sz, vp]
    lib.dalek_b200_x25519_batch.argtypes = [vp, vp, vp, sz, vp, vp]
    lib.dalek_b200_x25519_batch_dev.argtypes = [vp, vp, vp, sz, vp, vp]
    lib.dalek_b200_x25519_public_keys.argtypes = [vp, vp, sz, vp]
    lib.dalek_b200_mul_batch.argtypes = [vp, vp, sz, vp, C.c_int, sz, sz, C.c_int, vp, vp]
    lib.dalek_b200_mul_batch_dev.argtypes = [vp, vp, sz, vp, C.c_int, sz, sz, C.c_int, vp, vp]
    lib.dalek_b200_edwards_torsion_batch.argtypes = [vp, vp, C.c_int, sz, vp]
    lib.dalek_b200_vartime_double_base_batch.argtypes = [vp, vp, vp, C.c_int, sz, vp, vp]
    lib.dalek_b200_vartime_double_base_batch_dev.argtypes = [vp, vp, vp, C.c_int, sz, vp, vp]
    lib.dalek_b200_msm_batch.argtypes = [vp, vp, vp, C.c_int, vp, sz, C.c_int, vp, vp, vp]
    lib.dalek_b200_msm_batch_dev.argtypes = [vp, vp, vp, C.c_int, vp, sz, C.c_int, vp, vp, vp]
    lib.dalek_b200_ristretto_from_uniform_bytes_batch.argtypes = [vp, vp, sz, vp]
    lib.dalek_b200_ristretto_hash_from_bytes_batch.argtypes = [vp, vp, vp, sz, vp]
    lib.dalek_b200_edwards_hash_to_curve_batch.argtypes = [vp, vp, vp, sz, vp, sz, vp]
    lib.dalek_b200_edwards_encode_to_curve_batch.argtypes = [vp, vp, vp, sz, vp, sz, vp]
    lib.dalek_b200_ristretto_map_to_curve_batch.argtypes = [vp, vp, sz, vp]
    lib.dalek_b200_ristretto_lizard_encode_batch.argtypes = [vp, vp, sz, vp]
    lib.dalek_b200_ristretto_lizard_decode_batch.argtypes = [vp, vp, C.c_int, sz, vp, vp]
    lib.dalek_b200_ristretto_map_to_curve_inverse_batch.argtypes = [vp, vp, C.c_int, sz, vp, vp]
    _lib = lib
    return lib


class EngineError(RuntimeError):
    pass


class SignatureError(Exception):
    KINDS = {1: "Verify", 2: "ArrayLength", 3: "ScalarFormat", 4: "PointDecompression", 5: "PrehashedContextLength"}

    def __init__(self, code):
        self.code = code
        self.kind = self.KINDS.get(code, "Unknown")
        super().__init__(self.kind)


def _ptr(obj):
    if obj is None:
        return None
    if isinstance(obj, int):
        return obj
    if isinstance(obj, bytes):
        return C.cast(C.c_char_p(obj), C.c_void_p).value
    if isinstance(obj, bytearray):
        return C.addressof((C.c_char * len(obj)).from_buffer(obj)) if len(obj) else None
    if isinstance(obj, C.Array):
        return C.addressof(obj)
    if hasattr(obj, "data_ptr"):
        return obj.data_ptr()
    if hasattr(obj, "ctypes"):
        return obj.ctypes.data
    raise TypeError("unsupported buffer type %r" % type(obj))


class Engine:

    def __init__(self, device=0):
        self.lib = load_library()
        h = C.c_void_p()
        rc = self.lib.dalek_b200_init(device, C.byref(h))
        if rc != 0:
            raise EngineError("dalek_b200_init(device=%d) failed with %d: no usable sm_90 CUDA device "
                              "(the engine has no CPU fallback)" % (device, rc))
        self.h = h
        self.device = device

    def close(self):
        if getattr(self, "h", None):
            self.lib.dalek_b200_destroy(self.h)
            self.h = None

    def __del__(self):
        try:
            self.close()
        except Exception:
            pass

    def _check(self, rc):
        if rc < 0:
            raise EngineError("engine error %d: %s" % (rc, self.lib.dalek_b200_last_error(self.h).decode()))
        return rc

    def set_option(self, name, value):
        self._check(self.lib.dalek_b200_set_option(self.h, name.encode(), int(value)))

    def launch_count(self):
        return int(self.lib.dalek_b200_launch_count(self.h))

    def last_call_ms(self):
        ms = C.c_float()
        self.lib.dalek_b200_last_call_ms(self.h, C.byref(ms))
        return float(ms.value)

    def last_stage_ms(self, stage):
        ms = C.c_float()
        self._check(self.lib.dalek_b200_last_stage_ms(self.h, stage.encode(), C.byref(ms)))
        return float(ms.value)

    def last_kernel_ms(self):
        ms, n = C.c_float(), C.c_int()
        self.lib.dalek_b200_last_kernel_ms(self.h, C.byref(ms), C.byref(n))
        return ms.value, n.value

    def edwards_vartime_msm(self, scalars, points, n, point_fmt=POINTS_COMPRESSED, device_ptrs=False, want_limbs=False):
        out = (C.c_uint8 * 32)()
        limbs = (C.c_uint64 * 20)() if want_limbs else None
        fn = self.lib.dalek_b200_edwards_vartime_msm_dev if device_ptrs else self.lib.dalek_b200_edwards_vartime_msm
        keep = (scalars, points)
        rc = self._check(fn(self.h, _ptr(scalars), _ptr(points), point_fmt, n, C.addressof(out),
                            C.addressof(limbs) if want_limbs else None))
        del keep
        return rc, bytes(out), (list(limbs) if want_limbs else None)

    def edwards_ct_msm(self, scalars, points, n, point_fmt=POINTS_COMPRESSED, want_limbs=False):
        out = (C.c_uint8 * 32)()
        limbs = (C.c_uint64 * 20)() if want_limbs else None
        rc = self._check(self.lib.dalek_b200_edwards_ct_msm(self.h, _ptr(scalars), _ptr(points), point_fmt, n,
                                                            C.addressof(out), C.addressof(limbs) if want_limbs else None))
        return rc, bytes(out), (list(limbs) if want_limbs else None)

    def msm_window_count(self, n_shard):
        return self._check(self.lib.dalek_b200_msm_window_count(self.h, n_shard))

    def msm_partial_bytes(self, n_shard):
        return int(self.lib.dalek_b200_msm_partial_bytes(self.h, n_shard))

    def stream_ptr(self):
        return int(self.lib.dalek_b200_stream(self.h) or 0)

    def edwards_msm_partial(self, scalars, points, n_local, n_shard, point_fmt=POINTS_COMPRESSED, device_ptrs=False):
        nwin = self.msm_window_count(n_shard)
        out = (C.c_uint64 * (20 * nwin))()
        fn = self.lib.dalek_b200_edwards_msm_partial_dev if device_ptrs else self.lib.dalek_b200_edwards_msm_partial
        rc = self._check(fn(self.h, _ptr(scalars), _ptr(points), point_fmt, n_local, n_shard, C.addressof(out)))
        return rc, out

    def edwards_msm_combine(self, windows, ranks, n_shard, want_limbs=False):
        out = (C.c_uint8 * 32)()
        limbs = (C.c_uint64 * 20)() if want_limbs else None
        self._check(self.lib.dalek_b200_edwards_msm_combine(self.h, _ptr(windows) if not isinstance(windows, C.Array) else C.addressof(windows),
                                                            ranks, n_shard, C.addressof(out),
                                                            C.addressof(limbs) if want_limbs else None))
        return bytes(out), (list(limbs) if want_limbs else None)

    def edwards_msm_partial_async(self, scalars, points, n_local, n_shard, d_out_record, point_fmt=POINTS_COMPRESSED,
                                  device_ptrs=False):
        fn = self.lib.dalek_b200_edwards_msm_partial_dev_async if device_ptrs else self.lib.dalek_b200_edwards_msm_partial_async
        return self._check(fn(self.h, _ptr(scalars), _ptr(points), point_fmt, n_local, n_shard, _ptr(d_out_record)))

    def edwards_msm_combine_dev(self, d_records, ranks, n_shard, want_limbs=False):
        out = (C.c_uint8 * 32)()
        limbs = (C.c_uint64 * 20)() if want_limbs else None
        rc = self._check(self.lib.dalek_b200_edwards_msm_combine_dev(self.h, _ptr(d_records), ranks, n_shard, C.addressof(out),
                                                                     C.addressof(limbs) if want_limbs else None))
        return rc, bytes(out), (list(limbs) if want_limbs else None)

    def ristretto_double_base_batch(self, a, b, G, H, n, out=None):
        if out is not None:
            rc = self._check(self.lib.dalek_b200_ristretto_double_base_batch(self.h, _ptr(a), _ptr(b), _ptr(G), _ptr(H), n, _ptr(out)))
            return rc, out
        buf = (C.c_uint8 * (32 * max(n, 1)))()
        rc = self._check(self.lib.dalek_b200_ristretto_double_base_batch(self.h, _ptr(a), _ptr(b), _ptr(G), _ptr(H), n,
                                                                         C.addressof(buf)))
        return rc, bytes(buf)[:32 * n]

    def ristretto_vartime_msm(self, scalars, points, n):
        out = (C.c_uint8 * 32)()
        rc = self._check(self.lib.dalek_b200_ristretto_vartime_msm(self.h, _ptr(scalars), _ptr(points), n, C.addressof(out)))
        return rc, bytes(out)

    def scalar_from_wide_batch(self, wide, n):
        out = (C.c_uint8 * (32 * max(n, 1)))()
        self._check(self.lib.dalek_b200_scalar_from_wide_batch(self.h, _ptr(wide), n, C.addressof(out)))
        return bytes(out)[:32 * n]

    def scalar_invert_batch(self, scalars, n):
        out = (C.c_uint8 * (32 * max(n, 1)))()
        prod = (C.c_uint8 * 32)()
        self._check(self.lib.dalek_b200_scalar_invert_batch(self.h, _ptr(scalars), n, C.addressof(out), C.addressof(prod)))
        return bytes(out)[:32 * n], bytes(prod)

    def decompress_batch(self, encodings, n, ristretto=False):
        limbs = (C.c_uint64 * (20 * max(n, 1)))()
        ok = (C.c_uint8 * max(n, 1))()
        fn = self.lib.dalek_b200_ristretto_decompress_batch if ristretto else self.lib.dalek_b200_edwards_decompress_batch
        rc = self._check(fn(self.h, _ptr(encodings), n, C.addressof(limbs), C.addressof(ok)))
        return rc, limbs, bytes(ok)[:n]

    def compress_batch(self, limbs, n):
        out = (C.c_uint8 * (32 * max(n, 1)))()
        self._check(self.lib.dalek_b200_edwards_compress_batch(self.h, _ptr(limbs), n, C.addressof(out)))
        return bytes(out)[:32 * n]

    def ristretto_double_and_compress_batch(self, limbs, n):
        out = (C.c_uint8 * (32 * max(n, 1)))()
        self._check(self.lib.dalek_b200_ristretto_double_and_compress_batch(self.h, _ptr(limbs), n, C.addressof(out)))
        return bytes(out)[:32 * n]

    def edwards_to_montgomery_batch(self, limbs, n):
        out = (C.c_uint8 * (32 * max(n, 1)))()
        self._check(self.lib.dalek_b200_edwards_to_montgomery_batch(self.h, _ptr(limbs), n, C.addressof(out)))
        return bytes(out)[:32 * n]

    def x25519_batch(self, scalars, us, n, device_ptrs=False, want_contributory=False, out=None, contributory=None):
        if device_ptrs:
            if out is None or (want_contributory and contributory is None):
                import torch
                dev = torch.device("cuda", self.device)
                if out is None:
                    out = torch.empty(32 * max(n, 1), dtype=torch.uint8, device=dev)
                if want_contributory and contributory is None:
                    contributory = torch.empty(max(n, 1), dtype=torch.uint8, device=dev)
            self._check(self.lib.dalek_b200_x25519_batch_dev(self.h, _ptr(scalars), _ptr(us), n, _ptr(out),
                                                             _ptr(contributory) if want_contributory else None))
            return out, (contributory if want_contributory else None)
        res = (C.c_uint8 * (32 * max(n, 1)))()
        flags = (C.c_uint8 * max(n, 1))() if want_contributory else None
        self._check(self.lib.dalek_b200_x25519_batch(self.h, _ptr(scalars), _ptr(us), n, C.addressof(res),
                                                     C.addressof(flags) if want_contributory else None))
        return bytes(res)[:32 * n], (bytes(flags)[:n] if want_contributory else None)

    def x25519_public_keys(self, scalars, n):
        out = (C.c_uint8 * (32 * max(n, 1)))()
        self._check(self.lib.dalek_b200_x25519_public_keys(self.h, _ptr(scalars), n, C.addressof(out)))
        return bytes(out)[:32 * n]

    def mul_batch(self, scalars, n_scalars, points, n_points, n, point_fmt=POINTS_COMPRESSED, clamped=False, device_ptrs=False,
                  out=None, want_ok=False):
        flags = 1 if clamped else 0
        if device_ptrs:
            ok = None
            if out is None or want_ok:
                import torch
                dev = torch.device("cuda", self.device)
                if out is None:
                    out = torch.empty(32 * max(n, 1), dtype=torch.uint8, device=dev)
                if want_ok:
                    ok = torch.empty(max(n, 1), dtype=torch.uint8, device=dev)
            rc = self._check(self.lib.dalek_b200_mul_batch_dev(self.h, _ptr(scalars), n_scalars, _ptr(points), point_fmt, n_points, n,
                                                               flags, _ptr(out), _ptr(ok)))
            return rc, out, ok
        res = (C.c_uint8 * (32 * max(n, 1)))() if out is None else out
        ok = (C.c_uint8 * max(n, 1))() if want_ok else None
        rc = self._check(self.lib.dalek_b200_mul_batch(self.h, _ptr(scalars), n_scalars, _ptr(points), point_fmt, n_points, n, flags,
                                                       _ptr(res), C.addressof(ok) if want_ok else None))
        return rc, (bytes(res)[:32 * n] if out is None else out), (bytes(ok)[:n] if want_ok else None)

    def vartime_double_base_batch(self, ab, points, n, point_fmt=POINTS_COMPRESSED, device_ptrs=False, out=None, want_ok=False):
        if device_ptrs:
            ok = None
            if out is None or want_ok:
                import torch
                dev = torch.device("cuda", self.device)
                if out is None:
                    out = torch.empty(32 * max(n, 1), dtype=torch.uint8, device=dev)
                if want_ok:
                    ok = torch.empty(max(n, 1), dtype=torch.uint8, device=dev)
            rc = self._check(self.lib.dalek_b200_vartime_double_base_batch_dev(self.h, _ptr(ab), _ptr(points), point_fmt, n, _ptr(out),
                                                                               _ptr(ok)))
            return rc, out, ok
        res = (C.c_uint8 * (32 * max(n, 1)))() if out is None else out
        ok = (C.c_uint8 * max(n, 1))() if want_ok else None
        rc = self._check(self.lib.dalek_b200_vartime_double_base_batch(self.h, _ptr(ab), _ptr(points), point_fmt, n, _ptr(res),
                                                                       C.addressof(ok) if want_ok else None))
        return rc, (bytes(res)[:32 * n] if out is None else out), (bytes(ok)[:n] if want_ok else None)

    def msm_batch(self, scalars, points, offsets, m, point_fmt=POINTS_COMPRESSED, constant_time=False, device_ptrs=False,
                  want_limbs=False):
        out = (C.c_uint8 * (32 * max(m, 1)))()
        ok = (C.c_uint8 * max(m, 1))()
        limbs = (C.c_uint64 * (20 * max(m, 1)))() if want_limbs else None
        fn = self.lib.dalek_b200_msm_batch_dev if device_ptrs else self.lib.dalek_b200_msm_batch
        keep = (scalars, points, offsets)
        rc = self._check(fn(self.h, _ptr(scalars), _ptr(points), point_fmt, _ptr(offsets), m, 1 if constant_time else 0,
                            C.addressof(out), C.addressof(limbs) if want_limbs else None, C.addressof(ok)))
        del keep
        return rc, bytes(out)[:32 * m], bytes(ok)[:m], (list(limbs)[:20 * m] if want_limbs else None)

    def torsion_batch(self, points, n, point_fmt=POINTS_COMPRESSED):
        out = (C.c_uint8 * max(n, 1))()
        self._check(self.lib.dalek_b200_edwards_torsion_batch(self.h, _ptr(points), point_fmt, n, C.addressof(out)))
        return bytes(out)[:n]

    def ristretto_from_uniform_bytes_batch(self, data, n):
        out = (C.c_uint8 * (32 * max(n, 1)))()
        self._check(self.lib.dalek_b200_ristretto_from_uniform_bytes_batch(self.h, _ptr(data), n, C.addressof(out)))
        return bytes(out)[:32 * n]

    def ristretto_hash_from_bytes_batch(self, msgs_flat, offsets, n):
        out = (C.c_uint8 * (32 * max(n, 1)))()
        self._check(self.lib.dalek_b200_ristretto_hash_from_bytes_batch(self.h, _ptr(msgs_flat), _ptr(offsets), n, C.addressof(out)))
        return bytes(out)[:32 * n]

    def _edwards_h2c(self, fn, msgs_flat, offsets, n, dst):
        out = (C.c_uint8 * (32 * max(n, 1)))()
        dst = bytes(dst)
        self._check(fn(self.h, _ptr(msgs_flat), _ptr(offsets), n, _ptr(dst) if dst else None, len(dst), C.addressof(out)))
        return bytes(out)[:32 * n]

    def edwards_hash_to_curve_batch(self, msgs_flat, offsets, n, dst):
        return self._edwards_h2c(self.lib.dalek_b200_edwards_hash_to_curve_batch, msgs_flat, offsets, n, dst)

    def edwards_encode_to_curve_batch(self, msgs_flat, offsets, n, dst):
        return self._edwards_h2c(self.lib.dalek_b200_edwards_encode_to_curve_batch, msgs_flat, offsets, n, dst)

    def ristretto_map_to_curve_batch(self, data, n):
        out = (C.c_uint8 * (32 * max(n, 1)))()
        self._check(self.lib.dalek_b200_ristretto_map_to_curve_batch(self.h, _ptr(data), n, C.addressof(out)))
        return bytes(out)[:32 * n]

    def ristretto_lizard_encode_batch(self, data, n):
        out = (C.c_uint8 * (32 * max(n, 1)))()
        self._check(self.lib.dalek_b200_ristretto_lizard_encode_batch(self.h, _ptr(data), n, C.addressof(out)))
        return bytes(out)[:32 * n]

    def ristretto_lizard_decode_batch(self, points, n, point_fmt=POINTS_RISTRETTO):
        out = (C.c_uint8 * (16 * max(n, 1)))()
        st = (C.c_uint8 * max(n, 1))()
        rc = self._check(self.lib.dalek_b200_ristretto_lizard_decode_batch(self.h, _ptr(points), point_fmt, n, C.addressof(out),
                                                                           C.addressof(st)))
        return rc, bytes(out)[:16 * n], bytes(st)[:n]

    def ristretto_map_to_curve_inverse_batch(self, points, n, point_fmt=POINTS_RISTRETTO):
        out = (C.c_uint8 * (512 * max(n, 1)))()
        mask = (C.c_uint16 * max(n, 1))()
        rc = self._check(self.lib.dalek_b200_ristretto_map_to_curve_inverse_batch(self.h, _ptr(points), point_fmt, n,
                                                                                  C.addressof(out), C.addressof(mask)))
        return rc, bytes(out)[:512 * n], list(mask)[:n]

    def verify_batch_raw(self, messages, sigs, pubkeys):
        n = len(messages)
        bufs = [C.create_string_buffer(m, max(len(m), 1)) for m in messages]
        ptrs = (C.c_void_p * max(n, 1))(*[C.addressof(b) for b in bufs])
        lens = (C.c_size_t * max(n, 1))(*[len(m) for m in messages])
        return self._check(self.lib.ed25519_b200_verify_batch(self.h, C.addressof(ptrs), C.addressof(lens),
                                                              _ptr(sigs), _ptr(pubkeys), n))

    def verify_batch_flat(self, msgs_flat, offsets, sigs, pubkeys, n, device_ptrs=False, msgs_bytes=0):
        if device_ptrs:
            return self._check(self.lib.ed25519_b200_verify_batch_flat_dev(self.h, _ptr(msgs_flat), _ptr(offsets), _ptr(sigs),
                                                                           _ptr(pubkeys), n, msgs_bytes))
        return self._check(self.lib.ed25519_b200_verify_batch_flat(self.h, _ptr(msgs_flat), _ptr(offsets), _ptr(sigs),
                                                                   _ptr(pubkeys), n))

    def verify_batch_flat_points(self, msgs_flat, offsets, sigs, pubkeys, key_points, n, device_ptrs=False):
        fn = self.lib.ed25519_b200_verify_batch_flat_points_dev if device_ptrs else self.lib.ed25519_b200_verify_batch_flat_points
        return self._check(fn(self.h, _ptr(msgs_flat), _ptr(offsets), _ptr(sigs), _ptr(pubkeys), _ptr(key_points), n))

    def verify_batches_flat(self, msgs_flat, offsets, sigs, pubkeys, n, batch_size, device_ptrs=False):
        nb = (n + batch_size - 1) // batch_size
        verdicts = (C.c_int32 * max(nb, 1))()
        fn = self.lib.ed25519_b200_verify_batches_flat_dev if device_ptrs else self.lib.ed25519_b200_verify_batches_flat
        rc = self._check(fn(self.h, _ptr(msgs_flat), _ptr(offsets), _ptr(sigs), _ptr(pubkeys), n, batch_size, C.addressof(verdicts)))
        return rc, list(verdicts)[:nb]

    def verify_batches_flat_points(self, msgs_flat, offsets, sigs, pubkeys, key_points, n, batch_size, device_ptrs=False):
        nb = (n + batch_size - 1) // batch_size
        verdicts = (C.c_int32 * max(nb, 1))()
        fn = self.lib.ed25519_b200_verify_batches_flat_points_dev if device_ptrs else self.lib.ed25519_b200_verify_batches_flat_points
        rc = self._check(fn(self.h, _ptr(msgs_flat), _ptr(offsets), _ptr(sigs), _ptr(pubkeys), _ptr(key_points), n, batch_size, C.addressof(verdicts)))
        return rc, list(verdicts)[:nb]

    def verify_each_flat(self, msgs_flat, offsets, sigs, pubkeys, n, strict=False, device_ptrs=False):
        res = (C.c_uint8 * max(n, 1))()
        fn = self.lib.ed25519_b200_verify_each_flat_dev if device_ptrs else self.lib.ed25519_b200_verify_each_flat
        rc = self._check(fn(self.h, _ptr(msgs_flat), _ptr(offsets), _ptr(sigs), _ptr(pubkeys), n, 1 if strict else 0, C.addressof(res)))
        return rc, list(res)[:n]

    def last_zs(self, n):
        out = (C.c_uint8 * (16 * max(n, 1)))()
        self._check(self.lib.ed25519_b200_last_zs(self.h, C.addressof(out), n))
        return bytes(out)[:16 * n]

    def mul_base_batch(self, scalars, n, want_compressed=True):
        limbs = (C.c_uint64 * (20 * max(n, 1)))()
        comp = (C.c_uint8 * (32 * max(n, 1)))() if want_compressed else None
        self._check(self.lib.dalek_b200_edwards_mul_base_batch(self.h, _ptr(scalars), n, C.addressof(limbs),
                                                               C.addressof(comp) if want_compressed else None))
        return limbs, (bytes(comp)[:32 * n] if want_compressed else None)

    def verifying_keys(self, seeds, n):
        out = (C.c_uint8 * (32 * max(n, 1)))()
        self._check(self.lib.ed25519_b200_verifying_keys(self.h, _ptr(seeds), n, C.addressof(out)))
        return bytes(out)[:32 * n]

    def sign_flat(self, seeds, n_seeds, msgs_flat, offsets, n):
        out = (C.c_uint8 * (64 * max(n, 1)))()
        self._check(self.lib.ed25519_b200_sign_flat(self.h, _ptr(seeds), n_seeds, _ptr(msgs_flat), _ptr(offsets), n,
                                                    C.addressof(out)))
        return bytes(out)[:64 * n]

    def sign_prehashed(self, seeds, n_seeds, prehashes, n, context=None):
        out = (C.c_uint8 * (64 * max(n, 1)))()
        ctx = bytes(context) if context is not None else b""
        rc = self._check(self.lib.ed25519_b200_sign_prehashed(self.h, _ptr(seeds), n_seeds, _ptr(prehashes), n,
                                                              _ptr(ctx) if ctx else None, len(ctx), C.addressof(out)))
        return rc, bytes(out)[:64 * n]

    def verify_prehashed_each(self, prehashes, sigs, pubkeys, n, context=None, strict=False):
        res = (C.c_uint8 * max(n, 1))()
        ctx = bytes(context) if context is not None else b""
        rc = self._check(self.lib.ed25519_b200_verify_prehashed_each(self.h, _ptr(prehashes), _ptr(ctx) if ctx else None, len(ctx),
                                                                     _ptr(sigs), _ptr(pubkeys), n, 1 if strict else 0,
                                                                     C.addressof(res)))
        return rc, list(res)[:n]

    def sign_batch_flat(self, seeds, msgs_flat, offsets, n):
        pks = (C.c_uint8 * (32 * max(n, 1)))()
        sigs = (C.c_uint8 * (64 * max(n, 1)))()
        self._check(self.lib.ed25519_b200_sign_batch_flat(self.h, _ptr(seeds), _ptr(msgs_flat), _ptr(offsets), n,
                                                          C.addressof(pks), C.addressof(sigs)))
        return bytes(pks)[:32 * n], bytes(sigs)[:64 * n]


class MultiEngine:

    def __init__(self, devices):
        self.lib = load_library()
        devs = (C.c_int * len(devices))(*devices)
        h = C.c_void_p()
        rc = self.lib.dalek_b200_init_multi(devs, len(devices), C.byref(h))
        if rc != 0:
            raise EngineError("dalek_b200_init_multi(%r) failed with %d (the engine has no CPU fallback)" % (list(devices), rc))
        self.h = h
        self.devices = list(devices)

    def close(self):
        if getattr(self, "h", None):
            self.lib.dalek_b200_destroy_multi(self.h)
            self.h = None

    def __del__(self):
        try:
            self.close()
        except Exception:
            pass

    def set_option(self, name, value):
        for i in range(len(self.devices)):
            rc = self.lib.dalek_b200_set_option(self.lib.dalek_b200_multi_ctx(self.h, i), name.encode(), int(value))
            if rc:
                raise EngineError("set_option(%s) failed" % name)

    def last_call_ms(self):
        ms = C.c_float()
        self.lib.dalek_b200_last_call_ms(self.lib.dalek_b200_multi_ctx(self.h, 0), C.byref(ms))
        return float(ms.value)

    def edwards_vartime_msm(self, scalars, points, n, point_fmt=POINTS_COMPRESSED, want_limbs=False):
        out = (C.c_uint8 * 32)()
        limbs = (C.c_uint64 * 20)() if want_limbs else None
        keep = (scalars, points)
        rc = self.lib.dalek_b200_edwards_vartime_msm_multi(self.h, _ptr(scalars), _ptr(points), point_fmt, n, C.addressof(out),
                                                           C.addressof(limbs) if want_limbs else None)
        del keep
        if rc < 0:
            raise EngineError("engine error %d: %s" % (rc, self.lib.dalek_b200_multi_last_error(self.h).decode()))
        return rc, bytes(out), (list(limbs) if want_limbs else None)


_default = None


def default_engine():
    global _default
    if _default is None:
        _default = Engine(int(os.environ.get("LOCAL_RANK", "0")))
    return _default


def _msm_batch(scalar_lists, point_lists, fmt, constant_time, engine):
    import array
    scalar_lists, point_lists = [list(s) for s in scalar_lists], [list(p) for p in point_lists]
    assert len(scalar_lists) == len(point_lists), "one point list per scalar list"
    for s, p in zip(scalar_lists, point_lists):
        assert len(s) == len(p), "scalars and points must have the same length"
    m = len(scalar_lists)
    none = [any(q is None for q in p) for p in point_lists]
    if constant_time and any(none):
        raise ValueError("multiscalar_mul takes points, not Options")
    offs = array.array("Q", [0])
    for s, skip in zip(scalar_lists, none):
        offs.append(offs[-1] + (0 if skip else len(s)))
    flat_s = b"".join(b"".join(s) for s, skip in zip(scalar_lists, none) if not skip)
    flat_p = b"".join(b"".join(p) for p, skip in zip(point_lists, none) if not skip)
    eng = engine or default_engine()
    rc, out, ok, _ = eng.msm_batch(flat_s, flat_p, offs.tobytes(), m, point_fmt=fmt, constant_time=constant_time)
    return [None if (skip or not ok[j]) else out[32 * j:32 * j + 32] for j, skip in enumerate(none)]


def _expect_all(results):
    if any(r is None for r in results):
        raise ValueError("should return some point")
    return results


class EdwardsPoint:

    @staticmethod
    def optional_multiscalar_mul(scalars, points, engine=None):
        scalars, points = list(scalars), list(points)
        assert len(scalars) == len(points), "scalars and points must have the same length"
        if any(p is None for p in points):
            return None
        eng = engine or default_engine()
        rc, comp, _ = eng.edwards_vartime_msm(b"".join(scalars), b"".join(points), len(scalars))
        return None if rc == 1 else comp

    @staticmethod
    def vartime_multiscalar_mul(scalars, points, engine=None):
        r = EdwardsPoint.optional_multiscalar_mul(scalars, points, engine)
        if r is None:
            raise ValueError("should return some point")
        return r

    @staticmethod
    def multiscalar_mul(scalars, points, engine=None):
        scalars, points = list(scalars), list(points)
        assert len(scalars) == len(points), "scalars and points must have the same length"
        eng = engine or default_engine()
        rc, comp, _ = eng.edwards_ct_msm(b"".join(scalars), b"".join(points), len(scalars))
        return comp

    @staticmethod
    def optional_multiscalar_mul_batch(scalar_lists, point_lists, engine=None):
        return _msm_batch(scalar_lists, point_lists, POINTS_COMPRESSED, False, engine)

    @staticmethod
    def vartime_multiscalar_mul_batch(scalar_lists, point_lists, engine=None):
        return _expect_all(_msm_batch(scalar_lists, point_lists, POINTS_COMPRESSED, False, engine))

    @staticmethod
    def multiscalar_mul_batch(scalar_lists, point_lists, engine=None):
        return _msm_batch(scalar_lists, point_lists, POINTS_COMPRESSED, True, engine)

    @staticmethod
    def to_montgomery_batch(limbs, n=None, engine=None):
        n = len(limbs) // 20 if n is None else n
        eng = engine or default_engine()
        raw = eng.edwards_to_montgomery_batch(limbs, n)
        return [raw[32 * i:32 * i + 32] for i in range(n)]

    @staticmethod
    def mul_batch(scalars, points, engine=None):
        return _mul_batch(scalars, points, POINTS_COMPRESSED, False, engine)

    @staticmethod
    def mul_clamped_batch(bytes_list, points, engine=None):
        return _mul_batch(bytes_list, points, POINTS_COMPRESSED, True, engine)

    @staticmethod
    def vartime_double_scalar_mul_basepoint_batch(a_list, points, b_list, engine=None):
        return _double_base_batch(a_list, points, b_list, POINTS_COMPRESSED, engine)

    @staticmethod
    def is_small_order_batch(points, engine=None):
        return [bool(f & 1) for f in _torsion_flags(points, engine)]

    @staticmethod
    def is_torsion_free_batch(points, engine=None):
        return [bool(f & 2) for f in _torsion_flags(points, engine)]

    @staticmethod
    def hash_to_curve_batch(messages, dst, engine=None):
        eng = engine or default_engine()
        flat, offs, n = _flat_messages(messages)
        raw = eng.edwards_hash_to_curve_batch(flat, offs, n, dst)
        return [raw[32 * i:32 * i + 32] for i in range(n)]

    @staticmethod
    def encode_to_curve_batch(messages, dst, engine=None):
        eng = engine or default_engine()
        flat, offs, n = _flat_messages(messages)
        raw = eng.edwards_encode_to_curve_batch(flat, offs, n, dst)
        return [raw[32 * i:32 * i + 32] for i in range(n)]


def _mul_batch(scalars, points, fmt, clamped, engine):
    single_s, ss = _items(scalars, 32, "scalars")
    single_p, ps = _items(points, 32, "points")
    if not single_s and not single_p and len(ss) != len(ps):
        raise ValueError("scalars and points must have the same length (or one of them be a single item)")
    n = len(ps) if single_s else len(ss)
    if n == 0:
        return []
    if not clamped and any(s[31] & 0x80 for s in ss):
        raise ValueError("a scalar has bit 255 set")
    eng = engine or default_engine()
    rc, raw, _ = eng.mul_batch(b"".join(ss), len(ss), b"".join(ps), len(ps), n, fmt, clamped=clamped)
    if rc == 1:
        raise ValueError("a point does not decode")
    outs = [raw[32 * i:32 * i + 32] for i in range(n)]
    return outs[0] if single_s and single_p else outs


def _double_base_batch(a_list, points, b_list, fmt, engine):
    _, as_ = _items(a_list, 32, "scalars")
    _, bs = _items(b_list, 32, "scalars")
    _, ps = _items(points, 32, "points")
    if not len(as_) == len(bs) == len(ps):
        raise ValueError("a_list, points and b_list must have the same length")
    n = len(ps)
    if n == 0:
        return []
    if any((a[31] | b[31]) & 0x80 for a, b in zip(as_, bs)):
        raise ValueError("a scalar has bit 255 set")
    eng = engine or default_engine()
    rc, raw, _ = eng.vartime_double_base_batch(b"".join(a + b for a, b in zip(as_, bs)), b"".join(ps), n, fmt)
    if rc == 1:
        raise ValueError("a point does not decode")
    return [raw[32 * i:32 * i + 32] for i in range(n)]


def _torsion_flags(points, engine):
    _, ps = _items(points, 32, "points")
    if not ps:
        return []
    eng = engine or default_engine()
    flags = eng.torsion_batch(b"".join(ps), len(ps))
    if any(f == 0 for f in flags):
        raise ValueError("a point does not decode")
    return flags


def _flat_messages(messages):
    msgs = [bytes(m) for m in messages]
    n = len(msgs)
    offs = (C.c_uint64 * (n + 1))()
    acc = 0
    for i, m in enumerate(msgs):
        offs[i] = acc
        acc += len(m)
    offs[n] = acc
    flat = b"".join(msgs) + b"\0"
    return flat, offs, n


X25519_BASEPOINT_BYTES = bytes([9]) + bytes(31)


def _x25519_items(xs):
    single = isinstance(xs, (bytes, bytearray))
    items = [bytes(xs)] if single else [bytes(x) for x in xs]
    if any(len(x) != 32 for x in items):
        raise ValueError("X25519 secrets and u coordinates are 32 bytes each")
    return single, items


def x25519(scalars, us, engine=None):
    single, ks = _x25519_items(scalars)
    _, vs = _x25519_items(us)
    if len(ks) != len(vs):
        raise ValueError("scalars and us must have the same length")
    eng = engine or default_engine()
    raw, _ = eng.x25519_batch(b"".join(ks), b"".join(vs), len(ks))
    outs = [raw[32 * i:32 * i + 32] for i in range(len(ks))]
    return outs[0] if single else outs


def x25519_public_keys(secrets, engine=None):
    single, ks = _x25519_items(secrets)
    eng = engine or default_engine()
    raw = eng.x25519_public_keys(b"".join(ks), len(ks))
    outs = [raw[32 * i:32 * i + 32] for i in range(len(ks))]
    return outs[0] if single else outs


def _items(xs, size, what):
    single = isinstance(xs, (bytes, bytearray))
    items = [bytes(xs)] if single else [bytes(x) for x in xs]
    if any(len(x) != size for x in items):
        raise ValueError("%s are %d bytes each" % (what, size))
    return single, items


def ed25519_verifying_keys(seeds, engine=None):
    single, ks = _items(seeds, 32, "Ed25519 seeds")
    eng = engine or default_engine()
    raw = eng.verifying_keys(b"".join(ks), len(ks))
    outs = [raw[32 * i:32 * i + 32] for i in range(len(ks))]
    return outs[0] if single else outs


def _sign_args(seeds, n):
    single_key, ks = _items(seeds, 32, "Ed25519 seeds")
    if not single_key and len(ks) not in (1, n):
        raise ValueError("one seed, or one seed per message")
    return ks


def ed25519_sign(seeds, messages, engine=None):
    single = isinstance(messages, (bytes, bytearray))
    msgs = [bytes(messages)] if single else [bytes(m) for m in messages]
    ks = _sign_args(seeds, len(msgs))
    eng = engine or default_engine()
    flat, offs, n = _flat_messages(msgs)
    raw = eng.sign_flat(b"".join(ks), len(ks) if n else 0, flat, offs, n) if n else b""
    outs = [raw[64 * i:64 * i + 64] for i in range(n)]
    return outs[0] if single else outs


def _prehash_items(prehashed):
    single = isinstance(prehashed, (bytes, bytearray)) or hasattr(prehashed, "digest")
    items = [prehashed] if single else list(prehashed)
    out = [bytes(p.digest()) if hasattr(p, "digest") else bytes(p) for p in items]
    if any(len(p) != 64 for p in out):
        raise ValueError("Ed25519ph prehashes are 64-byte digests")
    return single, out


def ed25519_sign_prehashed(seeds, prehashed, context=None, engine=None):
    single, phs = _prehash_items(prehashed)
    ks = _sign_args(seeds, len(phs))
    eng = engine or default_engine()
    n = len(phs)
    rc, raw = eng.sign_prehashed(b"".join(ks), len(ks) if n else 0, b"".join(phs), n, context)
    if rc:
        raise SignatureError(rc)
    outs = [raw[64 * i:64 * i + 64] for i in range(n)]
    return outs[0] if single else outs


def ed25519_verify_prehashed(prehashed, signatures, verifying_keys, context=None, strict=False, engine=None):
    single, phs = _prehash_items(prehashed)
    _, sigs = _items([signatures] if single else signatures, 64, "signatures")
    _, keys = _items([verifying_keys] if single else verifying_keys, 32, "verifying keys")
    if not (len(phs) == len(sigs) == len(keys)):
        raise ValueError("prehashes, signatures and verifying keys must have the same length")
    if context is not None and len(bytes(context)) > 255:
        raise ValueError("an Ed25519ph context is at most 255 bytes")
    eng = engine or default_engine()
    _, res = eng.verify_prehashed_each(b"".join(phs), b"".join(sigs), b"".join(keys), len(phs), context, strict)
    return res[0] if single else res


class _Precomputation:
    _FMT = POINTS_COMPRESSED

    def __init__(self, static_points, engine=None, fmt=None):
        self.eng = engine or default_engine()
        fmt = self._FMT if fmt is None else fmt
        if fmt == POINTS_EXTENDED:
            buf, n = static_points
        else:
            pts = list(static_points)
            buf, n = b"".join(pts), len(pts)
        h = C.c_void_p()
        rc = self.eng._check(self.eng.lib.dalek_b200_precomp_new(self.eng.h, _ptr(buf) if n else None, fmt, n, C.byref(h)))
        if rc == 1:
            raise ValueError("a static point does not decode")
        self.h = h

    def __len__(self):
        return int(self.eng.lib.dalek_b200_precomp_len(self.h))

    def is_empty(self):
        return len(self) == 0

    def close(self):
        if getattr(self, "h", None):
            self.eng.lib.dalek_b200_precomp_destroy(self.h)
            self.h = None

    def __del__(self):
        try:
            self.close()
        except Exception:
            pass

    def optional_mixed_multiscalar_mul(self, static_scalars, dynamic_scalars, dynamic_points, dynamic_fmt=None):
        ss, ds, dp = list(static_scalars), list(dynamic_scalars), list(dynamic_points)
        assert len(ss) <= len(self), "more static scalars than static points"
        assert len(ds) == len(dp), "dynamic scalars and points must have the same length"
        if any(p is None for p in dp):
            return None
        out = (C.c_uint8 * 32)()
        sb, db, pb = b"".join(ss), b"".join(ds), b"".join(dp)
        rc = self.eng._check(self.eng.lib.dalek_b200_precomp_mixed_msm(
            self.eng.h, self.h, _ptr(sb) if ss else None, len(ss), _ptr(db) if ds else None, _ptr(pb) if dp else None,
            self._FMT if dynamic_fmt is None else dynamic_fmt, len(ds), C.addressof(out), None))
        return None if rc == 1 else bytes(out)

    def vartime_mixed_multiscalar_mul(self, static_scalars, dynamic_scalars, dynamic_points):
        r = self.optional_mixed_multiscalar_mul(static_scalars, dynamic_scalars, dynamic_points)
        if r is None:
            raise ValueError("should return some point")
        return r

    def vartime_multiscalar_mul(self, static_scalars):
        return self.vartime_mixed_multiscalar_mul(static_scalars, [], [])


class VartimeEdwardsPrecomputation(_Precomputation):
    _FMT = POINTS_COMPRESSED


class VartimeRistrettoPrecomputation(_Precomputation):
    _FMT = POINTS_RISTRETTO


class RistrettoPoint:

    @staticmethod
    def vartime_multiscalar_mul(scalars, points, engine=None):
        scalars, points = list(scalars), list(points)
        assert len(scalars) == len(points)
        eng = engine or default_engine()
        rc, comp = eng.ristretto_vartime_msm(b"".join(scalars), b"".join(points), len(scalars))
        if rc == 1:
            raise ValueError("should return some point")
        return comp

    @staticmethod
    def optional_multiscalar_mul_batch(scalar_lists, point_lists, engine=None):
        return _msm_batch(scalar_lists, point_lists, POINTS_RISTRETTO, False, engine)

    @staticmethod
    def vartime_multiscalar_mul_batch(scalar_lists, point_lists, engine=None):
        return _expect_all(_msm_batch(scalar_lists, point_lists, POINTS_RISTRETTO, False, engine))

    @staticmethod
    def multiscalar_mul_batch(scalar_lists, point_lists, engine=None):
        return _msm_batch(scalar_lists, point_lists, POINTS_RISTRETTO, True, engine)

    @staticmethod
    def double_base_batch(a, b, G, H, engine=None):
        eng = engine or default_engine()
        n = len(a) // 32
        rc, out = eng.ristretto_double_base_batch(a, b, G, H, n)
        if rc == 1:
            raise ValueError("G or H is not a valid Ristretto encoding")
        return out

    @staticmethod
    def mul_batch(scalars, points, engine=None):
        return _mul_batch(scalars, points, POINTS_RISTRETTO, False, engine)

    @staticmethod
    def vartime_double_scalar_mul_basepoint_batch(a_list, points, b_list, engine=None):
        return _double_base_batch(a_list, points, b_list, POINTS_RISTRETTO, engine)

    @staticmethod
    def from_uniform_bytes_batch(data, engine=None):
        items = [bytes(x) for x in data]
        if any(len(x) != 64 for x in items):
            raise ValueError("from_uniform_bytes takes 64 bytes per item")
        eng = engine or default_engine()
        raw = eng.ristretto_from_uniform_bytes_batch(b"".join(items), len(items))
        return [raw[32 * i:32 * i + 32] for i in range(len(items))]

    @staticmethod
    def hash_from_bytes_batch(messages, engine=None):
        eng = engine or default_engine()
        flat, offs, n = _flat_messages(messages)
        raw = eng.ristretto_hash_from_bytes_batch(flat, offs, n)
        return [raw[32 * i:32 * i + 32] for i in range(n)]

    @staticmethod
    def map_to_curve_batch(data, engine=None):
        _, items = _items(list(data), 32, "map_to_curve inputs")
        if not items:
            return []
        eng = engine or default_engine()
        raw = eng.ristretto_map_to_curve_batch(b"".join(items), len(items))
        return [raw[32 * i:32 * i + 32] for i in range(len(items))]

    @staticmethod
    def lizard_encode_batch(data, engine=None):
        _, items = _items(list(data), 16, "Lizard payloads")
        if not items:
            return []
        eng = engine or default_engine()
        raw = eng.ristretto_lizard_encode_batch(b"".join(items), len(items))
        return [raw[32 * i:32 * i + 32] for i in range(len(items))]

    @staticmethod
    def lizard_decode_batch(points, engine=None):
        _, items = _items(list(points), 32, "points")
        if not items:
            return []
        eng = engine or default_engine()
        _, raw, st = eng.ristretto_lizard_decode_batch(b"".join(items), len(items))
        if any(s == 2 for s in st):
            raise ValueError("a point does not decode")
        return [raw[16 * i:16 * i + 16] if st[i] == 0 else None for i in range(len(items))]

    @staticmethod
    def map_to_curve_inverse_batch(points, engine=None):
        _, items = _items(list(points), 32, "points")
        if not items:
            return []
        eng = engine or default_engine()
        rc, raw, masks = eng.ristretto_map_to_curve_inverse_batch(b"".join(items), len(items))
        if rc == 1:
            raise ValueError("a point does not decode")
        return [[raw[512 * i + 32 * j:512 * i + 32 * j + 32] if masks[i] >> j & 1 else None for j in range(16)]
                for i in range(len(items))]


def verify_batch(messages, signatures, verifying_keys, engine=None):
    messages, signatures, verifying_keys = list(messages), list(signatures), list(verifying_keys)
    if not (len(messages) == len(signatures) == len(verifying_keys)):
        raise SignatureError(2)
    eng = engine or default_engine()
    rc = eng.verify_batch_raw(messages, b"".join(signatures), b"".join(verifying_keys))
    if rc != 0:
        raise SignatureError(rc)
    return None
```

include/dalek_b200.h:

```cpp
#ifndef DALEK_B200_H
#define DALEK_B200_H
#include <stddef.h>
#include <stdint.h>

#ifdef __cplusplus
extern "C" {
#endif

typedef struct dalek_b200_ctx dalek_b200_ctx;

#define DALEK_OK 0
#define DALEK_NONE 1
#define ED25519_ERR_VERIFY 1
#define ED25519_ERR_ARRAY_LENGTH 2
#define ED25519_ERR_SCALAR_FORMAT 3
#define ED25519_ERR_POINT_DECOMPRESSION 4
#define ED25519_ERR_PREHASHED_CONTEXT_LENGTH 5
#define DALEK_E_INVALID_ARG (-1)
#define DALEK_E_NO_DEVICE (-2)
#define DALEK_E_CUDA (-3)
#define DALEK_E_NOMEM (-4)

#define DALEK_POINTS_COMPRESSED 0
#define DALEK_POINTS_EXTENDED 1
#define DALEK_POINTS_RISTRETTO 2

int dalek_b200_init(int device, dalek_b200_ctx **out);
void dalek_b200_destroy(dalek_b200_ctx *ctx);
const char *dalek_b200_last_error(const dalek_b200_ctx *ctx);
int dalek_b200_set_option(dalek_b200_ctx *ctx, const char *name, long value);
uint64_t dalek_b200_launch_count(const dalek_b200_ctx *ctx);
int dalek_b200_last_kernel_ms(const dalek_b200_ctx *ctx, float *ms, int *launches);
int dalek_b200_last_stage_ms(const dalek_b200_ctx *ctx, const char *stage, float *ms);
int dalek_b200_last_call_ms(const dalek_b200_ctx *ctx, float *ms);

int dalek_b200_edwards_vartime_msm(dalek_b200_ctx *ctx, const uint8_t *scalars, const void *points,
                                   int point_fmt, size_t n, uint8_t out_compressed[32],
                                   uint64_t out_limbs[20]);
int dalek_b200_edwards_ct_msm(dalek_b200_ctx *ctx, const uint8_t *scalars, const void *points,
                              int point_fmt, size_t n, uint8_t out_compressed[32],
                              uint64_t out_limbs[20]);
int dalek_b200_edwards_vartime_msm_dev(dalek_b200_ctx *ctx, const void *d_scalars, const void *d_points,
                                       int point_fmt, size_t n, uint8_t out_compressed[32],
                                       uint64_t out_limbs[20]);

int dalek_b200_msm_window_count(dalek_b200_ctx *ctx, size_t n_shard);
size_t dalek_b200_msm_partial_bytes(dalek_b200_ctx *ctx, size_t n_shard);
int dalek_b200_edwards_msm_partial(dalek_b200_ctx *ctx, const uint8_t *scalars, const void *points,
                                   int point_fmt, size_t n_local, size_t n_shard,
                                   uint64_t *out_windows);
int dalek_b200_edwards_msm_partial_dev(dalek_b200_ctx *ctx, const void *d_scalars, const void *d_points,
                                       int point_fmt, size_t n_local, size_t n_shard,
                                       uint64_t *out_windows);
int dalek_b200_edwards_msm_combine(dalek_b200_ctx *ctx, const uint64_t *windows, int ranks,
                                   size_t n_shard, uint8_t out_compressed[32], uint64_t out_limbs[20]);
int dalek_b200_edwards_msm_partial_async(dalek_b200_ctx *ctx, const uint8_t *scalars, const void *points,
                                         int point_fmt, size_t n_local, size_t n_shard, void *d_out_record);
int dalek_b200_edwards_msm_partial_dev_async(dalek_b200_ctx *ctx, const void *d_scalars, const void *d_points,
                                             int point_fmt, size_t n_local, size_t n_shard, void *d_out_record);
int dalek_b200_edwards_msm_combine_dev(dalek_b200_ctx *ctx, const void *d_records, int ranks, size_t n_shard,
                                       uint8_t out_compressed[32], uint64_t out_limbs[20]);
void *dalek_b200_stream(dalek_b200_ctx *ctx);

typedef struct dalek_b200_multi dalek_b200_multi;
int dalek_b200_init_multi(const int *devices, int ndev, dalek_b200_multi **out);
void dalek_b200_destroy_multi(dalek_b200_multi *m);
int dalek_b200_multi_device_count(const dalek_b200_multi *m);
dalek_b200_ctx *dalek_b200_multi_ctx(dalek_b200_multi *m, int i);
const char *dalek_b200_multi_last_error(const dalek_b200_multi *m);
int dalek_b200_edwards_vartime_msm_multi(dalek_b200_multi *m, const uint8_t *scalars, const void *points,
                                         int point_fmt, size_t n, uint8_t out_compressed[32],
                                         uint64_t out_limbs[20]);

typedef struct dalek_b200_precomp dalek_b200_precomp;
int dalek_b200_precomp_new(dalek_b200_ctx *ctx, const void *static_points, int point_fmt, size_t n,
                           dalek_b200_precomp **out);
size_t dalek_b200_precomp_len(const dalek_b200_precomp *pre);
void dalek_b200_precomp_destroy(dalek_b200_precomp *pre);
int dalek_b200_precomp_mixed_msm(dalek_b200_ctx *ctx, const dalek_b200_precomp *pre,
                                 const uint8_t *static_scalars, size_t n_static,
                                 const uint8_t *dynamic_scalars, const void *dynamic_points,
                                 int dynamic_fmt, size_t n_dynamic, uint8_t out_compressed[32],
                                 uint64_t out_limbs[20]);

int dalek_b200_edwards_decompress_batch(dalek_b200_ctx *ctx, const uint8_t *in, size_t n,
                                        uint64_t *out_limbs, uint8_t *ok);
int dalek_b200_edwards_compress_batch(dalek_b200_ctx *ctx, const uint64_t *limbs, size_t n, uint8_t *out);
int dalek_b200_ristretto_decompress_batch(dalek_b200_ctx *ctx, const uint8_t *in, size_t n,
                                          uint64_t *out_limbs, uint8_t *ok);
int dalek_b200_ristretto_double_and_compress_batch(dalek_b200_ctx *ctx, const uint64_t *limbs, size_t n,
                                                   uint8_t *out);
int dalek_b200_edwards_to_montgomery_batch(dalek_b200_ctx *ctx, const uint64_t *limbs, size_t n, uint8_t *out);

int dalek_b200_x25519_batch(dalek_b200_ctx *ctx, const uint8_t *scalars, const uint8_t *us, size_t n,
                            uint8_t *out, uint8_t *contributory);
int dalek_b200_x25519_batch_dev(dalek_b200_ctx *ctx, const void *d_scalars, const void *d_us, size_t n,
                                void *d_out, void *d_contributory);
int dalek_b200_x25519_public_keys(dalek_b200_ctx *ctx, const uint8_t *scalars, size_t n, uint8_t *out);

#define DALEK_MUL_CLAMPED 1
int dalek_b200_mul_batch(dalek_b200_ctx *ctx, const uint8_t *scalars, size_t n_scalars, const void *points, int point_fmt,
                         size_t n_points, size_t n, int flags, uint8_t *out , uint8_t *ok );
int dalek_b200_mul_batch_dev(dalek_b200_ctx *ctx, const void *d_scalars, size_t n_scalars, const void *d_points, int point_fmt,
                             size_t n_points, size_t n, int flags, void *d_out, void *d_ok);
int dalek_b200_edwards_torsion_batch(dalek_b200_ctx *ctx, const void *points, int point_fmt, size_t n, uint8_t *out);

int dalek_b200_vartime_double_base_batch(dalek_b200_ctx *ctx, const uint8_t *ab ,
                                         const void *points, int point_fmt, size_t n,
                                         uint8_t *out , uint8_t *ok );
int dalek_b200_vartime_double_base_batch_dev(dalek_b200_ctx *ctx, const void *d_ab, const void *d_points, int point_fmt,
                                             size_t n, void *d_out, void *d_ok);

int dalek_b200_msm_batch(dalek_b200_ctx *ctx, const uint8_t *scalars , const void *points, int point_fmt,
                         const uint64_t *offsets , size_t m, int constant_time, uint8_t *out ,
                         uint64_t *out_limbs , uint8_t *ok );
int dalek_b200_msm_batch_dev(dalek_b200_ctx *ctx, const void *d_scalars, const void *d_points, int point_fmt, const void *d_offsets,
                             size_t m, int constant_time, uint8_t *out, uint64_t *out_limbs, uint8_t *ok);

int dalek_b200_ristretto_from_uniform_bytes_batch(dalek_b200_ctx *ctx, const uint8_t *in, size_t n, uint8_t *out);
int dalek_b200_ristretto_hash_from_bytes_batch(dalek_b200_ctx *ctx, const uint8_t *msgs_flat, const uint64_t *msg_offsets,
                                               size_t n, uint8_t *out);
int dalek_b200_edwards_hash_to_curve_batch(dalek_b200_ctx *ctx, const uint8_t *msgs_flat, const uint64_t *msg_offsets,
                                           size_t n, const uint8_t *dst, size_t dst_len, uint8_t *out);
int dalek_b200_edwards_encode_to_curve_batch(dalek_b200_ctx *ctx, const uint8_t *msgs_flat, const uint64_t *msg_offsets,
                                             size_t n, const uint8_t *dst, size_t dst_len, uint8_t *out);

int dalek_b200_ristretto_map_to_curve_batch(dalek_b200_ctx *ctx, const uint8_t *in, size_t n, uint8_t *out);
int dalek_b200_ristretto_lizard_encode_batch(dalek_b200_ctx *ctx, const uint8_t *data, size_t n, uint8_t *out);
int dalek_b200_ristretto_lizard_decode_batch(dalek_b200_ctx *ctx, const void *points, int point_fmt, size_t n,
                                             uint8_t *data_out, uint8_t *status);
int dalek_b200_ristretto_map_to_curve_inverse_batch(dalek_b200_ctx *ctx, const void *points, int point_fmt, size_t n,
                                                    uint8_t *out, uint16_t *mask);

int dalek_b200_scalar_from_wide_batch(dalek_b200_ctx *ctx, const uint8_t *in, size_t n, uint8_t *out);
int dalek_b200_scalar_invert_batch(dalek_b200_ctx *ctx, const uint8_t *in, size_t n, uint8_t *out,
                                   uint8_t out_product[32]);

int dalek_b200_ristretto_double_base_batch(dalek_b200_ctx *ctx, const uint8_t *a, const uint8_t *b,
                                           const uint8_t G[32], const uint8_t H[32], size_t n,
                                           uint8_t *out);
int dalek_b200_ristretto_vartime_msm(dalek_b200_ctx *ctx, const uint8_t *scalars,
                                     const uint8_t *points, size_t n, uint8_t out_compressed[32]);

int ed25519_b200_verify_batch(dalek_b200_ctx *ctx, const uint8_t *const *msgs, const size_t *msg_lens,
                              const uint8_t *sigs, const uint8_t *pubkeys, size_t n);
int ed25519_b200_verify_batch_flat(dalek_b200_ctx *ctx, const uint8_t *msgs_flat,
                                   const uint64_t *msg_offsets, const uint8_t *sigs,
                                   const uint8_t *pubkeys, size_t n);
int ed25519_b200_verify_batch_flat_dev(dalek_b200_ctx *ctx, const void *d_msgs_flat,
                                       const void *d_msg_offsets, const void *d_sigs,
                                       const void *d_pubkeys, size_t n, size_t msgs_bytes);
int ed25519_b200_verify_batch_flat_points(dalek_b200_ctx *ctx, const uint8_t *msgs_flat, const uint64_t *msg_offsets,
                                          const uint8_t *sigs, const uint8_t *pubkeys, const uint64_t *key_points, size_t n);
int ed25519_b200_verify_batch_flat_points_dev(dalek_b200_ctx *ctx, const void *d_msgs_flat, const void *d_msg_offsets,
                                              const void *d_sigs, const void *d_pubkeys, const void *d_key_points, size_t n);
int ed25519_b200_verify_batches_flat(dalek_b200_ctx *ctx, const uint8_t *msgs_flat,
                                     const uint64_t *msg_offsets, const uint8_t *sigs,
                                     const uint8_t *pubkeys, size_t n, size_t batch_size, int32_t *verdicts);
int ed25519_b200_verify_batches_flat_dev(dalek_b200_ctx *ctx, const void *d_msgs_flat,
                                         const void *d_msg_offsets, const void *d_sigs,
                                         const void *d_pubkeys, size_t n, size_t batch_size, int32_t *verdicts);
int ed25519_b200_verify_batches_flat_points(dalek_b200_ctx *ctx, const uint8_t *msgs_flat, const uint64_t *msg_offsets,
                                            const uint8_t *sigs, const uint8_t *pubkeys, const uint64_t *key_points, size_t n,
                                            size_t batch_size, int32_t *verdicts);
int ed25519_b200_verify_batches_flat_points_dev(dalek_b200_ctx *ctx, const void *d_msgs_flat, const void *d_msg_offsets,
                                                const void *d_sigs, const void *d_pubkeys, const void *d_key_points, size_t n,
                                                size_t batch_size, int32_t *verdicts);
int ed25519_b200_verify_each_flat(dalek_b200_ctx *ctx, const uint8_t *msgs_flat, const uint64_t *msg_offsets,
                                  const uint8_t *sigs, const uint8_t *pubkeys, size_t n, int strict,
                                  uint8_t *results);
int ed25519_b200_verify_each_flat_dev(dalek_b200_ctx *ctx, const void *d_msgs_flat, const void *d_msg_offsets,
                                      const void *d_sigs, const void *d_pubkeys, size_t n, int strict,
                                      uint8_t *results);
int ed25519_b200_last_zs(dalek_b200_ctx *ctx, uint8_t *zs_out, size_t n);

int ed25519_b200_verifying_keys(dalek_b200_ctx *ctx, const uint8_t *seeds, size_t n, uint8_t *pubkeys_out);
int ed25519_b200_sign_flat(dalek_b200_ctx *ctx, const uint8_t *seeds, size_t n_seeds, const uint8_t *msgs_flat,
                           const uint64_t *msg_offsets, size_t n, uint8_t *sigs_out);
int ed25519_b200_sign_prehashed(dalek_b200_ctx *ctx, const uint8_t *seeds, size_t n_seeds, const uint8_t *prehashes, size_t n,
                                const uint8_t *context, size_t context_len, uint8_t *sigs_out);
int ed25519_b200_verify_prehashed_each(dalek_b200_ctx *ctx, const uint8_t *prehashes, const uint8_t *context,
                                       size_t context_len, const uint8_t *sigs, const uint8_t *pubkeys, size_t n,
                                       int strict, uint8_t *results);

int dalek_b200_edwards_mul_base_batch(dalek_b200_ctx *ctx, const uint8_t *scalars, size_t n,
                                      uint64_t *out_limbs , uint8_t *out_compressed );
int ed25519_b200_sign_batch_flat(dalek_b200_ctx *ctx, const uint8_t *seeds, const uint8_t *msgs_flat,
                                 const uint64_t *msg_offsets, size_t n, uint8_t *pubkeys_out,
                                 uint8_t *sigs_out);

#ifdef __cplusplus
}
#endif
#endif
```

Measured before the change: 374.8 million.

## Fuse task building into fine sort and collapse niels prep to one kernel

The Niels-point preparation drops the three-kernel grid-wide batched inversion (zprod, invert, finish). A single kernel now does a per-block inversion with 8 points per thread and dynamic shared memory. The multi-kernel task construction pipeline (count, three-stage scan, bases, fill, hist, scan, scatter) is folded into k_sort_fine via a bin_tasks helper, followed by one offset-scan kernel and one emit kernel, cutting launches from 11 to 4. A host-side debug API for reading task lists is also added. The costs are one field inversion per block instead of one per batch, more shared memory, and a single-block serial scan over all bins.

```diff
diff --git a/curve25519_dalek_b200/csrc/api.cu b/curve25519_dalek_b200/csrc/api.cu
--- a/curve25519_dalek_b200/csrc/api.cu
+++ b/curve25519_dalek_b200/csrc/api.cu
@@ -56,7 +56,7 @@
     DevBuf *bufs[] = {&ctx->scalars, &ctx->points_in, &ctx->points, &ctx->digits, &ctx->counts, &ctx->offsets,
                       &ctx->sorted, &ctx->buckets, &ctx->red_a, &ctx->red_b, &ctx->red_c, &ctx->red_d, &ctx->key_pts,
                       &ctx->result, &ctx->flags, &ctx->misc0, &ctx->misc1, &ctx->misc2, &ctx->misc3,
-                      &ctx->misc4, &ctx->misc5, &ctx->zs, &ctx->base_table, &ctx->ntasks, &ctx->task_off, &ctx->tasks, &ctx->task_sums, &ctx->msg_offs, &ctx->sum_desc, &ctx->sum_part, &ctx->key_table, &ctx->key_acc, &ctx->task_order, &ctx->sig_status, &ctx->misc6, &ctx->each_pow, &ctx->each_tab, &ctx->each_kstat, &ctx->comb_base_table, &ctx->prep_prod, &ctx->mb_ws[0], &ctx->mb_ws[1]};
+                      &ctx->misc4, &ctx->misc5, &ctx->zs, &ctx->base_table, &ctx->ntasks, &ctx->task_off, &ctx->tasks, &ctx->task_sums, &ctx->msg_offs, &ctx->sum_desc, &ctx->sum_part, &ctx->key_table, &ctx->key_acc, &ctx->task_order, &ctx->sig_status, &ctx->misc6, &ctx->each_pow, &ctx->each_tab, &ctx->each_kstat, &ctx->comb_base_table, &ctx->mb_ws[0], &ctx->mb_ws[1]};
     for (DevBuf *b : bufs) if (b->p) cudaFree(b->p);
     if (ctx->h_pinned) cudaFreeHost(ctx->h_pinned);
     cudaEventDestroy(ctx->ev_a); cudaEventDestroy(ctx->ev_b); cudaEventDestroy(ctx->ev_fork); cudaEventDestroy(ctx->ev_join);
diff --git a/curve25519_dalek_b200/csrc/engine.h b/curve25519_dalek_b200/csrc/engine.h
--- a/curve25519_dalek_b200/csrc/engine.h
+++ b/curve25519_dalek_b200/csrc/engine.h
@@ -50,10 +50,10 @@
     float last_kernel_ms = 0.f;
     float last_call_ms = 0.f;
     int last_kernel_launches = 0;
+    size_t last_task_dims[4] = {0, 0, 0, 0};
     bool async_open = false;
     DevBuf scalars, points_in, points, digits, counts, offsets, sorted, buckets, red_a, red_b, red_c,
         red_d, key_pts, result, flags, misc0, misc1, misc2, misc3, misc4, misc5, zs, base_table, ntasks, task_off, tasks, task_sums, msg_offs, sum_desc, sum_part, key_table, key_acc, task_order, sig_status, misc6, each_pow, each_tab, each_kstat;
-    DevBuf prep_prod;
     uint32_t hash_seed[4] = {0x243F6A88u, 0x85A308D3u, 0x13198A2Eu, 0x03707344u};
     int sum_desc_c = -1;
     bool base_table_ready = false;
diff --git a/curve25519_dalek_b200/csrc/msm.cu b/curve25519_dalek_b200/csrc/msm.cu
--- a/curve25519_dalek_b200/csrc/msm.cu
+++ b/curve25519_dalek_b200/csrc/msm.cu
@@ -67,7 +67,7 @@
 }
 
 #define PREP_THREADS 256
-#define PREP_PER_THREAD 4
+#define PREP_PER_THREAD 8
 #define PREP_GROUP (PREP_THREADS * PREP_PER_THREAD)
 #define PREP_NW (PREP_THREADS / 32)
 
@@ -108,23 +108,10 @@
 #pragma unroll
     for (int k = 0; k < 5; k++) o.v[k] = __shfl_down_sync(0xffffffffu, f.v[k], d);
 }
-__device__ __forceinline__ void fe64_shfl_xor(fe64 &o, const fe64 &f, int m)
-{
-#pragma unroll
-    for (int k = 0; k < 5; k++) o.v[k] = __shfl_xor_sync(0xffffffffu, f.v[k], m);
-}
 __device__ __forceinline__ void fe64_shfl_idx(fe64 &o, const fe64 &f, int src)
 {
 #pragma unroll
     for (int k = 0; k < 5; k++) o.v[k] = __shfl_sync(0xffffffffu, f.v[k], src);
-}
-
-__device__ __forceinline__ void warp_product(fe64 &p, const fe64 &x, int width)
-{
-    fe64 t;
-    p = x;
-#pragma unroll 1
-    for (int m = width >> 1; m > 0; m >>= 1) { fe64_shfl_xor(t, p, m); fe64_mul(p, p, t); }
 }
 
 __device__ __forceinline__ void warp_other_products(const fe64 &x, fe64 &below, fe64 &above, fe64 &all)
@@ -143,8 +130,7 @@
     fe64_shfl_down(above, hi, 1); if (lane == 31) fe64_1(above);
 }
 
-template <bool INVERT>
-__device__ __forceinline__ void block_inverse(fe64 &inv, const fe64 &acc, fe64 *s_warp, const fe64 *tot_inv)
+__device__ __forceinline__ void block_inverse(fe64 &inv, const fe64 &acc, fe64 *s_warp)
 {
     const uint32_t lane = threadIdx.x & 31, warp = threadIdx.x >> 5, nw = blockDim.x >> 5;
     fe64 below, above, all;
@@ -155,14 +141,10 @@
         fe64 x, b, a, t;
         if (lane < nw) x = s_warp[lane]; else fe64_1(x);
         warp_other_products(x, b, a, all);
-        if (INVERT) {
-            const w20_role r = w20_roles();
-            const double inv = w20_invert(w20_limb(all, r.i), r);
-#pragma unroll
-            for (uint32_t k = 0; k < 5; k++) t.v[k] = w20_shfl(inv, k);
-        } else {
-            t = *tot_inv;
-        }
+        const w20_role r = w20_roles();
+        const double iv = w20_invert(w20_limb(all, r.i), r);
+#pragma unroll
+        for (uint32_t k = 0; k < 5; k++) t.v[k] = w20_shfl(iv, k);
         fe64_mul(t, t, b); fe64_mul(t, t, a);
         if (lane < nw) s_warp[lane] = t;
     }
@@ -170,55 +152,12 @@
     fe64_mul(inv, s_warp[warp], below); fe64_mul(inv, inv, above);
 }
 
-__global__ void __launch_bounds__(PREP_THREADS, 2)
-k_prep_zprod(const uint64_t *__restrict__ in, fe64 *__restrict__ prod, size_t n)
+__global__ void __launch_bounds__(PREP_THREADS, 512 / PREP_THREADS)
+k_prep_niels(const uint64_t *__restrict__ in, ge_niels_packed *__restrict__ out, size_t n)
 {
     __shared__ fe64 s_warp[PREP_NW];
-    const uint32_t tid = threadIdx.x, lane = tid & 31, warp = tid >> 5;
-    const size_t g0 = (size_t)blockIdx.x * PREP_GROUP + tid;
-    fe64 z[PREP_PER_THREAD], acc, t;
-    uint32_t ok[PREP_PER_THREAD];
-#pragma unroll
-    for (int k = 0; k < PREP_PER_THREAD; k++) {
-        const size_t i = g0 + (size_t)k * PREP_THREADS;
-        if (i < n) ok[k] = load_z(z[k], in, i); else { ok[k] = 0; fe64_1(z[k]); }
-    }
-    acc = z[0];
-    if (!ok[0]) fe64_1(acc);
-#pragma unroll
-    for (int k = 1; k < PREP_PER_THREAD; k++) { fe64_mul(t, acc, z[k]); fe64_cmov(acc, t, ok[k]); }
-    warp_product(t, acc, 32);
-    if (lane == 0) s_warp[warp] = t;
-    __syncthreads();
-    if (warp == 0) {
-        if (lane < PREP_NW) acc = s_warp[lane]; else fe64_1(acc);
-        warp_product(t, acc, PREP_NW);
-        if (lane == 0) prod[blockIdx.x] = t;
-    }
-}
-
-__global__ void __launch_bounds__(PREP_THREADS)
-k_prep_invert(fe64 *__restrict__ prod, fe64 *__restrict__ pre, uint32_t G)
-{
-    __shared__ fe64 s_warp[PREP_NW];
-    const uint32_t per = (G + blockDim.x - 1) / blockDim.x, b = min(threadIdx.x * per, G), e = min(b + per, G);
-    fe64 acc, inv, t;
-    fe64_1(acc);
-    for (uint32_t k = b; k < e; k++) { fe64_mul(acc, acc, prod[k]); pre[k] = acc; }
-    block_inverse<true>(inv, acc, s_warp, nullptr);
-    for (uint32_t k = e; k-- > b;) {
-        const fe64 x = prod[k];
-        if (k > b) fe64_mul(t, inv, pre[k - 1]); else t = inv;
-        prod[k] = t;
-        fe64_mul(inv, inv, x);
-    }
-}
-
-__global__ void __launch_bounds__(PREP_THREADS, 2)
-k_prep_finish(const uint64_t *__restrict__ in, const fe64 *__restrict__ ginv, ge_niels_packed *__restrict__ out, size_t n)
-{
-    __shared__ fe64 s_warp[PREP_NW];
-    __shared__ fe64 s_pre[PREP_PER_THREAD - 1][PREP_THREADS];
+    extern __shared__ __align__(16) unsigned char prep_smem[];
+    fe64 (*s_pre)[PREP_THREADS] = reinterpret_cast<fe64 (*)[PREP_THREADS]>(prep_smem);
     const uint32_t tid = threadIdx.x;
     const size_t g0 = (size_t)blockIdx.x * PREP_GROUP + tid;
     fe64 acc, inv;
@@ -235,7 +174,7 @@
             nz |= ok << k;
         }
     }
-    block_inverse<false>(inv, acc, s_warp, ginv + blockIdx.x);
+    block_inverse(inv, acc, s_warp);
 #pragma unroll 1
     for (int k = PREP_PER_THREAD - 1; k >= 0; k--) {
         const size_t i = g0 + (size_t)k * PREP_THREADS;
@@ -293,14 +232,9 @@
     } else if (kind == PK_PNIELS) {
         k_prep_extended_pniels<<<cdiv(n, 128), 128, 0, st>>>((const uint64_t *)d_in, (ge_pniels_packed *)d_out, n);
     } else {
-        const unsigned G = cdiv(n, PREP_GROUP);
-        int rc;
-        if ((rc = ws_reserve(ctx, ctx->prep_prod, 2 * (size_t)G * sizeof(fe64)))) return rc;
-        fe64 *prod = (fe64 *)ctx->prep_prod.p;
-        k_prep_zprod<<<G, PREP_THREADS, 0, st>>>((const uint64_t *)d_in, prod, n);
-        k_prep_invert<<<1, PREP_THREADS, 0, st>>>(prod, prod + G, G);
-        k_prep_finish<<<G, PREP_THREADS, 0, st>>>((const uint64_t *)d_in, prod, (ge_niels_packed *)d_out, n);
-        ctx->launches += 2;
+        const size_t smem = (size_t)(PREP_PER_THREAD - 1) * PREP_THREADS * sizeof(fe64);
+        CUDA_TRY(ctx, cudaFuncSetAttribute(k_prep_niels, cudaFuncAttributeMaxDynamicSharedMemorySize, (int)smem));
+        k_prep_niels<<<cdiv(n, PREP_GROUP), PREP_THREADS, smem, st>>>((const uint64_t *)d_in, (ge_niels_packed *)d_out, n);
     }
     ctx->launches++;
     CUDA_TRY(ctx, cudaGetLastError());
@@ -400,6 +334,39 @@
     base = __shfl_sync(0xffffffffu, base, leader);
     return base + __popc(peers & ((1u << lane) - 1));
 }
+
+#define TASK_BINS 256u
+__device__ __forceinline__ uint32_t task_key(uint32_t len, uint32_t task_len)
+{
+    return (uint32_t)(((uint64_t)len * (TASK_BINS - 1) + task_len - 1) / task_len);
+}
+__device__ __forceinline__ uint32_t task_count(uint32_t cnt, uint32_t task_len)
+{
+    return cnt <= task_len ? 1u : (cnt + task_len - 1) / task_len;
+}
+
+__device__ void bin_tasks(const uint32_t *h, uint32_t *tk, uint32_t *scr, uint32_t nf, size_t b0, uint32_t bin,
+                          uint32_t task_len, uint32_t *__restrict__ ntasks, uint32_t *__restrict__ task_off,
+                          uint32_t *__restrict__ heavy, uint32_t *__restrict__ bin_tasks, uint32_t *__restrict__ hist)
+{
+    uint32_t *th = tk + (1u << SORT_FINE_MAX);
+    for (uint32_t k = threadIdx.x; k < TASK_BINS; k += blockDim.x) th[k] = 0;
+    __syncthreads();
+    for (uint32_t f = threadIdx.x; f < nf; f += blockDim.x) {
+        const uint32_t cnt = h[f], k = task_count(cnt, task_len);
+        tk[f] = k;
+        ntasks[b0 + f] = k;
+        if (k > 1) { heavy[1 + atomicAdd(&heavy[0], 1u)] = (uint32_t)(b0 + f); atomicAdd(&th[TASK_BINS - 1], k - 1); }
+        atomicAdd(&th[task_key(cnt - (k - 1) * task_len, task_len)], 1u);
+    }
+    const uint32_t total = block_excl_scan(tk, nf, scr);
+    for (uint32_t f = threadIdx.x; f < nf; f += blockDim.x) task_off[b0 + f] = tk[f];
+    if (threadIdx.x == 0) bin_tasks[bin] = total;
+    for (uint32_t k = threadIdx.x; k < TASK_BINS; k += blockDim.x)
+        if (th[k]) atomicAdd(&hist[k], th[k]);
+    __syncthreads();
+}
+static_assert((1u << SORT_FINE_MAX) + TASK_BINS <= SORT_FINE_CAP, "bin_tasks scratch inside k_sort_fine's out[]");
 
 __global__ void __launch_bounds__(SORT_THREADS)
 k_sort_count(const uint4 *__restrict__ scalars, size_t n, int c, int nact, int F, uint32_t nc, int flat,
@@ -507,8 +474,10 @@
 __global__ void __launch_bounds__(SORT_THREADS, 2)
 k_sort_fine(const uint2 *__restrict__ records, const uint32_t *__restrict__ ccount, const uint32_t *__restrict__ ccursor,
             const uint32_t *__restrict__ xpre, const uint32_t *__restrict__ xtot, size_t n, int F, uint32_t nc,
-            uint32_t nbuckets, uint32_t nwin, int flat, uint32_t *__restrict__ counts, uint32_t *__restrict__ offsets,
-            uint32_t *__restrict__ sorted, uint32_t *__restrict__ fill)
+            uint32_t nbuckets, uint32_t nwin, int flat, uint32_t task_len, uint32_t *__restrict__ counts,
+            uint32_t *__restrict__ offsets, uint32_t *__restrict__ sorted, uint32_t *__restrict__ fill,
+            uint32_t *__restrict__ ntasks, uint32_t *__restrict__ task_off, uint32_t *__restrict__ heavy,
+            uint32_t *__restrict__ bin_tasks_out, uint32_t *__restrict__ hist)
 {
     extern __shared__ uint32_t sm[];
     __shared__ uint32_t s_bin, s_slice;
@@ -560,6 +529,7 @@
         }
         __syncthreads();
         for (uint32_t f = threadIdx.x; f < nf; f += SORT_THREADS) counts[b0 + f] = h[f];
+        bin_tasks(h, out, scr, nf, b0, bin, task_len, ntasks, task_off, heavy, bin_tasks_out, hist);
         block_excl_scan(h, nf, scr);
         for (uint32_t f = threadIdx.x; f < nf; f += SORT_THREADS) offsets[b0 + f] = base + h[f];
         __syncthreads();
@@ -569,6 +539,8 @@
         return;
     }
     for (uint32_t f = threadIdx.x; f < nf; f += SORT_THREADS) { h[f] = counts[b0 + f]; out[f] = 0; }
+    if (slice == 0)
+        bin_tasks(h, reinterpret_cast<uint32_t *>(recs), scr, nf, b0, bin, task_len, ntasks, task_off, heavy, bin_tasks_out, hist);
     block_excl_scan(h, nf, scr);
     if (slice == 0)
         for (uint32_t f = threadIdx.x; f < nf; f += SORT_THREADS) offsets[b0 + f] = base + h[f];
@@ -599,55 +571,61 @@
     }
 }
 
-#define SCAN_PART 4096u
-__global__ void __launch_bounds__(1024) k_scan_partial(const uint32_t *__restrict__ in, uint32_t nbuckets, uint32_t parts,
-                                                       uint32_t *__restrict__ part_sums)
-{
-    __shared__ uint32_t sh[32];
-    uint32_t w = blockIdx.x / parts, part = blockIdx.x % parts;
-    const uint32_t *src = in + (size_t)w * nbuckets;
-    uint32_t base = part * SCAN_PART + threadIdx.x * 4, sum = 0;
-#pragma unroll
-    for (int k = 0; k < 4; k++) if (base + k < nbuckets) sum += src[base + k];
-    for (int d = 16; d > 0; d >>= 1) sum += __shfl_down_sync(0xffffffffu, sum, d);
-    if ((threadIdx.x & 31) == 0) sh[threadIdx.x >> 5] = sum;
-    __syncthreads();
-    if (threadIdx.x < 32) {
-        uint32_t v = sh[threadIdx.x];
-        for (int d = 16; d > 0; d >>= 1) v += __shfl_down_sync(0xffffffffu, v, d);
-        if (threadIdx.x == 0) part_sums[blockIdx.x] = v;
-    }
-}
-__global__ void k_scan_bases(uint32_t *__restrict__ part_sums, uint32_t parts)
-{
-    if (threadIdx.x) return;
-    uint32_t *p = part_sums + (size_t)blockIdx.x * parts, run = 0;
-    for (uint32_t k = 0; k < parts; k++) { uint32_t v = p[k]; p[k] = run; run += v; }
-}
-__global__ void __launch_bounds__(1024) k_scan_apply(const uint32_t *__restrict__ in, const uint32_t *__restrict__ part_base,
-                                                     uint32_t nbuckets, uint32_t parts, uint32_t *__restrict__ out)
-{
-    __shared__ uint32_t sh[32];
-    uint32_t w = blockIdx.x / parts, part = blockIdx.x % parts;
-    const uint32_t *src = in + (size_t)w * nbuckets;
-    uint32_t *dst = out + (size_t)w * nbuckets;
-    uint32_t base = part * SCAN_PART + threadIdx.x * 4;
-    uint32_t v[4], sum = 0;
-#pragma unroll
-    for (int k = 0; k < 4; k++) { v[k] = base + k < nbuckets ? src[base + k] : 0; sum += v[k]; }
-    uint32_t incl = sum;
-    for (int d = 1; d < 32; d <<= 1) { uint32_t t = __shfl_up_sync(0xffffffffu, incl, d); if ((threadIdx.x & 31) >= d) incl += t; }
-    if ((threadIdx.x & 31) == 31) sh[threadIdx.x >> 5] = incl;
-    __syncthreads();
-    if (threadIdx.x < 32) {
-        uint32_t x = sh[threadIdx.x], inc2 = x;
-        for (int d = 1; d < 32; d <<= 1) { uint32_t t = __shfl_up_sync(0xffffffffu, inc2, d); if (threadIdx.x >= d) inc2 += t; }
-        sh[threadIdx.x] = inc2 - x;
-    }
-    __syncthreads();
-    uint32_t run = part_base[blockIdx.x] + sh[threadIdx.x >> 5] + incl - sum;
-#pragma unroll
-    for (int k = 0; k < 4; k++) { if (base + k < nbuckets) dst[base + k] = run; run += v[k]; }
+#define TASK_SCAN_THREADS 1024u
+#define TASK_SCAN_CHUNK 8192u
+__global__ void __launch_bounds__(TASK_SCAN_THREADS)
+k_task_offsets(uint32_t *__restrict__ bin_tasks, uint32_t nbins, uint32_t nc, uint32_t nwin, const uint32_t *__restrict__ hist,
+               uint32_t *__restrict__ start, uint32_t *__restrict__ win_base)
+{
+    __shared__ uint32_t v[TASK_SCAN_CHUNK], scr[33];
+    uint32_t carry = 0;
+    for (uint32_t b0 = 0; b0 < nbins; b0 += TASK_SCAN_CHUNK) {
+        const uint32_t len = min(TASK_SCAN_CHUNK, nbins - b0);
+        for (uint32_t k = threadIdx.x; k < len; k += TASK_SCAN_THREADS) v[k] = bin_tasks[b0 + k];
+        const uint32_t total = block_excl_scan(v, len, scr);
+        for (uint32_t k = threadIdx.x; k < len; k += TASK_SCAN_THREADS) {
+            const uint32_t g = carry + v[k];
+            bin_tasks[b0 + k] = g;
+            if ((b0 + k) % nc == 0) win_base[(b0 + k) / nc] = g;
+        }
+        carry += total;
+        __syncthreads();
+    }
+    if (threadIdx.x == 0) win_base[nwin] = carry;
+    if (threadIdx.x < TASK_BINS) v[threadIdx.x] = hist[TASK_BINS - 1 - threadIdx.x];
+    block_excl_scan(v, TASK_BINS, scr);
+    if (threadIdx.x < TASK_BINS) start[TASK_BINS - 1 - threadIdx.x] = v[threadIdx.x];
+}
+
+__global__ void __launch_bounds__(TASK_BINS)
+k_task_emit(const uint32_t *__restrict__ counts, const uint32_t *__restrict__ ntasks, uint32_t *__restrict__ task_off,
+            const uint32_t *__restrict__ bin_base, const uint32_t *__restrict__ win_base, const uint32_t *__restrict__ start,
+            uint32_t *__restrict__ cursor, uint32_t total_buckets, uint32_t nbuckets, int F, uint32_t task_len,
+            uint2 *__restrict__ tasks, uint32_t *__restrict__ order)
+{
+    __shared__ uint32_t cnt[TASK_BINS], base[TASK_BINS];
+    cnt[threadIdx.x] = 0;
+    __syncthreads();
+    const uint32_t t = blockIdx.x * TASK_BINS + threadIdx.x;
+    const bool live = t < total_buckets;
+    uint32_t k = 0, p0 = 0, key = 0, rank = 0, rank_full = 0;
+    if (live) {
+        const uint32_t w = t / nbuckets;
+        k = ntasks[t];
+        const uint32_t off = bin_base[t >> F] - win_base[w] + task_off[t];
+        task_off[t] = off;
+        p0 = win_base[w] + off;
+        key = task_key(counts[t] - (k - 1) * task_len, task_len);
+        rank = atomicAdd(&cnt[key], 1u);
+        if (k > 1) rank_full = atomicAdd(&cnt[TASK_BINS - 1], k - 1);
+    }
+    __syncthreads();
+    if (cnt[threadIdx.x]) base[threadIdx.x] = start[threadIdx.x] + atomicAdd(&cursor[threadIdx.x], cnt[threadIdx.x]);
+    __syncthreads();
+    if (!live) return;
+    for (uint32_t j = 0; j < k; j++) tasks[p0 + j] = make_uint2(t, j);
+    for (uint32_t j = 0; j + 1 < k; j++) order[base[TASK_BINS - 1] + rank_full + j] = p0 + j;
+    order[base[key] + rank] = p0 + k - 1;
 }
 
 #define TASK_LEN_MIN 64u
@@ -662,96 +640,6 @@
 #ifndef ACC_MIN_BLOCKS
 #define ACC_MIN_BLOCKS 4
 #endif
-
-__global__ void k_task_count(const uint32_t *__restrict__ counts, uint32_t total_buckets, uint32_t task_len,
-                             uint32_t *__restrict__ ntasks, uint32_t *__restrict__ heavy)
-{
-    uint32_t t = blockIdx.x * blockDim.x + threadIdx.x;
-    if (t >= total_buckets) return;
-    uint32_t c = counts[t];
-    uint32_t k = c <= task_len ? 1u : (c + task_len - 1) / task_len;
-    ntasks[t] = k;
-    if (k > 1) heavy[1 + atomicAdd(&heavy[0], 1u)] = t;
-}
-
-__global__ void k_task_bases(const uint32_t *__restrict__ ntasks, const uint32_t *__restrict__ task_off, uint32_t nbuckets,
-                             int nwin, uint32_t *__restrict__ win_base )
-{
-    if (blockIdx.x || threadIdx.x) return;
-    uint32_t run = 0;
-    for (int w = 0; w < nwin; w++) {
-        win_base[w] = run;
-        size_t last = (size_t)w * nbuckets + nbuckets - 1;
-        run += task_off[last] + ntasks[last];
-    }
-    win_base[nwin] = run;
-}
-
-__global__ void k_task_fill(const uint32_t *__restrict__ ntasks, const uint32_t *__restrict__ task_off,
-                            const uint32_t *__restrict__ win_base, uint32_t nbuckets, uint32_t total_buckets,
-                            uint2 *__restrict__ tasks)
-{
-    uint32_t t = blockIdx.x * blockDim.x + threadIdx.x;
-    if (t >= total_buckets) return;
-    uint32_t w = t / nbuckets;
-    uint32_t base = win_base[w] + task_off[t], k = ntasks[t];
-    for (uint32_t j = 0; j < k; j++) tasks[base + j] = make_uint2(t, j);
-}
-
-#define TASK_BINS 256u
-__device__ __forceinline__ uint32_t task_key(uint32_t len, uint32_t task_len)
-{
-    return (uint32_t)(((uint64_t)len * (TASK_BINS - 1) + task_len - 1) / task_len);
-}
-__device__ __forceinline__ uint32_t task_length(const uint2 tk, const uint32_t *__restrict__ counts, uint32_t task_len)
-{
-    return min(task_len, counts[tk.x] - tk.y * task_len);
-}
-
-__global__ void __launch_bounds__(256)
-k_task_hist(const uint2 *__restrict__ tasks, const uint32_t *__restrict__ counts, const uint32_t *__restrict__ total_ptr,
-            uint32_t task_len, uint32_t *__restrict__ hist)
-{
-    __shared__ uint32_t sh[TASK_BINS];
-    sh[threadIdx.x] = 0;
-    __syncthreads();
-    const uint32_t p = blockIdx.x * blockDim.x + threadIdx.x;
-    if (p < *total_ptr) atomicAdd(&sh[task_key(task_length(tasks[p], counts, task_len), task_len)], 1u);
-    __syncthreads();
-    if (sh[threadIdx.x]) atomicAdd(&hist[threadIdx.x], sh[threadIdx.x]);
-}
-
-__global__ void __launch_bounds__(256) k_task_scan(const uint32_t *__restrict__ hist, uint32_t *__restrict__ start)
-{
-    __shared__ uint32_t sh[TASK_BINS];
-    const uint32_t k = TASK_BINS - 1 - threadIdx.x;
-    sh[threadIdx.x] = hist[k];
-    __syncthreads();
-    for (uint32_t d = 1; d < TASK_BINS; d <<= 1) {
-        uint32_t v = threadIdx.x >= d ? sh[threadIdx.x - d] : 0;
-        __syncthreads();
-        sh[threadIdx.x] += v;
-        __syncthreads();
-    }
-    start[k] = sh[threadIdx.x] - hist[k];
-}
-
-__global__ void __launch_bounds__(256)
-k_task_scatter(const uint2 *__restrict__ tasks, const uint32_t *__restrict__ counts, const uint32_t *__restrict__ total_ptr,
-               uint32_t task_len, const uint32_t *__restrict__ start, uint32_t *__restrict__ cursor, uint32_t *__restrict__ order)
-{
-    __shared__ uint32_t cnt[TASK_BINS], base[TASK_BINS];
-    cnt[threadIdx.x] = 0;
-    __syncthreads();
-    const uint32_t p = blockIdx.x * blockDim.x + threadIdx.x;
-    const bool live = p < *total_ptr;
-    uint32_t key = 0, rank = 0;
-    if (live) { key = task_key(task_length(tasks[p], counts, task_len), task_len); rank = atomicAdd(&cnt[key], 1u); }
-    __syncthreads();
-    if (cnt[threadIdx.x]) base[threadIdx.x] = start[threadIdx.x] + atomicAdd(&cursor[threadIdx.x], cnt[threadIdx.x]);
-    __syncthreads();
-    if (live) order[base[key] + rank] = p;
-}
 
 __device__ __forceinline__ void load_p3(ge_p3 &p, const ge_p3_raw *src)
 {
@@ -1053,13 +941,12 @@
     const uint32_t task_len = flat ? msm_task_len(n * (size_t)nact, 1, nb) : msm_task_len(n, nact, nb);
     const size_t max_tasks = total_buckets + (std::max<size_t>(1, n) * nact) / task_len + 1;
     const size_t max_heavy = (std::max<size_t>(1, n) * nact) / task_len + 1;
-    const uint32_t parts = (nb + SCAN_PART - 1) / SCAN_PART;
     const int F = msm_sort_fine_bits(flat ? n * (size_t)nact : n, c, flat ? 1 : nact);
     const uint32_t nc = nb >> F;
     cudaStream_t st = ctx->stream;
     int rc;
     if ((rc = ws_reserve(ctx, ctx->counts, (total_buckets + (size_t)nwin * nc + 1 + max_heavy) * 4))) return rc;
-    if ((rc = ws_reserve(ctx, ctx->offsets, (total_buckets + (size_t)nwin * parts + 2 * (size_t)nwin * nc + nwin) * 4))) return rc;
+    if ((rc = ws_reserve(ctx, ctx->offsets, (total_buckets + 3 * (size_t)nwin * nc + nwin) * 4))) return rc;
     if ((rc = ws_reserve(ctx, ctx->ntasks, total_buckets * 4))) return rc;
     if ((rc = ws_reserve(ctx, ctx->task_off, total_buckets * 4 + (nwin + 1) * 4))) return rc;
     if ((rc = ws_reserve(ctx, ctx->tasks, max_tasks * 8))) return rc;
@@ -1072,9 +959,10 @@
     uint32_t *ntasks = (uint32_t *)ctx->ntasks.p, *task_off = (uint32_t *)ctx->task_off.p;
     uint32_t *win_base = task_off + total_buckets;
     uint32_t *ccount = counts + total_buckets, *heavy = ccount + (size_t)nwin * nc;
-    uint32_t *part_sums = offsets + total_buckets, *ccursor = part_sums + (size_t)nwin * parts;
+    uint32_t *bin_tasks = offsets + total_buckets, *ccursor = bin_tasks + (size_t)nwin * nc;
     uint32_t *xpre = ccursor + (size_t)nwin * nc, *xtot = xpre + (size_t)nwin * nc;
     uint2 *tasks = (uint2 *)ctx->tasks.p;
+    uint32_t *fill = (uint32_t *)ctx->tasks.p;
     uint32_t *t_hist = (uint32_t *)ctx->task_order.p, *t_cursor = t_hist + TASK_BINS, *t_start = t_cursor + TASK_BINS;
     uint32_t *order = t_start + TASK_BINS;
     ge_p3_raw *task_sums = (ge_p3_raw *)ctx->task_sums.p;
@@ -1092,7 +980,7 @@
         k_sort_count<<<cdiv(n, SORT_COUNT_TILE), SORT_THREADS, 0, st>>>((const uint4 *)d_scalars, n, c, nact, F, nc, flat ? 1 : 0, ccount);
         ctx->launches++;
     }
-    k_sort_bins_scan<<<nwin, SORT_THREADS, 0, st>>>(ccount, nc, F, nb, ccursor, xpre, xtot, counts, ntasks);
+    k_sort_bins_scan<<<nwin, SORT_THREADS, 0, st>>>(ccount, nc, F, nb, ccursor, xpre, xtot, counts, fill);
     if (n) {
         k_sort_partition<<<cdiv(n, SORT_TILE), SORT_THREADS, part_smem, st>>>((const uint4 *)d_scalars, n, c, nact, F, nc, nb, flat,
                                                                               ccount, ccursor, records, counts);
@@ -1100,17 +988,12 @@
     }
     const size_t extra = n * (size_t)nact / SORT_FINE_CAP;
     k_sort_fine<<<(unsigned)(nwin * nc + extra), SORT_THREADS, fine_smem, st>>>(records, ccount, ccursor, xpre, xtot, n, F, nc, nb,
-                                                                               (uint32_t)nwin, flat ? 1 : 0, counts, offsets, sorted, ntasks);
-    k_task_count<<<cdiv(total_buckets, 256), 256, 0, st>>>(counts, (uint32_t)total_buckets, task_len, ntasks, heavy);
-    k_scan_partial<<<nwin * parts, 1024, 0, st>>>(ntasks, nb, parts, part_sums);
-    k_scan_bases<<<nwin, 32, 0, st>>>(part_sums, parts);
-    k_scan_apply<<<nwin * parts, 1024, 0, st>>>(ntasks, part_sums, nb, parts, task_off);
-    k_task_bases<<<1, 32, 0, st>>>(ntasks, task_off, nb, nwin, win_base);
-    k_task_fill<<<cdiv(total_buckets, 256), 256, 0, st>>>(ntasks, task_off, win_base, nb, (uint32_t)total_buckets, tasks);
-    k_task_hist<<<cdiv(max_tasks, 256), 256, 0, st>>>(tasks, counts, win_base + nwin, task_len, t_hist);
-    k_task_scan<<<1, 256, 0, st>>>(t_hist, t_start);
-    k_task_scatter<<<cdiv(max_tasks, 256), 256, 0, st>>>(tasks, counts, win_base + nwin, task_len, t_start, t_cursor, order);
-    ctx->launches += 11;
+                                                                               (uint32_t)nwin, flat ? 1 : 0, task_len, counts, offsets,
+                                                                               sorted, fill, ntasks, task_off, heavy, bin_tasks, t_hist);
+    k_task_offsets<<<1, TASK_SCAN_THREADS, 0, st>>>(bin_tasks, (uint32_t)nwin * nc, nc, (uint32_t)nwin, t_hist, t_start, win_base);
+    k_task_emit<<<cdiv(total_buckets, TASK_BINS), TASK_BINS, 0, st>>>(counts, ntasks, task_off, bin_tasks, win_base, t_start, t_cursor,
+                                                                     (uint32_t)total_buckets, nb, F, task_len, tasks, order);
+    ctx->launches += 4;
     if (points_ready) CUDA_TRY(ctx, cudaStreamWaitEvent(st, points_ready, 0));
     if (first) CUDA_TRY(ctx, cudaEventRecord(ctx->ev_a, st));
     {
@@ -1124,8 +1007,33 @@
         ctx->launches += 2;
     }
     CUDA_TRY(ctx, cudaEventRecord(ctx->ev_b, st));
+    ctx->last_task_dims[0] = (size_t)nwin; ctx->last_task_dims[1] = nb; ctx->last_task_dims[2] = task_len;
+    ctx->last_task_dims[3] = (size_t)(heavy - counts);
     ctx->last_kernel_launches = first ? 1 : ctx->last_kernel_launches + 1;
     CUDA_TRY(ctx, cudaGetLastError());
+    return 0;
+}
+
+int dalek_b200_msm_task_lists(dalek_b200_ctx *ctx, uint32_t info[5], uint32_t *arrays)
+{
+    if (!ctx || !info || !ctx->last_task_dims[0]) return DALEK_E_INVALID_ARG;
+    const uint32_t nwin = (uint32_t)ctx->last_task_dims[0], nb = (uint32_t)ctx->last_task_dims[1], nc_total = nwin * nb;
+    const uint32_t *counts = (const uint32_t *)ctx->counts.p, *task_off = (const uint32_t *)ctx->task_off.p;
+    uint32_t ntask = 0, nheavy = 0;
+    CUDA_TRY(ctx, cudaStreamSynchronize(ctx->stream));
+    CUDA_TRY(ctx, cudaMemcpy(&ntask, task_off + nc_total + nwin, 4, cudaMemcpyDeviceToHost));
+    const uint32_t *heavy = counts + ctx->last_task_dims[3];
+    CUDA_TRY(ctx, cudaMemcpy(&nheavy, heavy, 4, cudaMemcpyDeviceToHost));
+    info[0] = nwin; info[1] = nb; info[2] = (uint32_t)ctx->last_task_dims[2]; info[3] = ntask; info[4] = nheavy;
+    if (!arrays) return 0;
+    uint32_t *o = arrays;
+    CUDA_TRY(ctx, cudaMemcpy(o, counts, (size_t)nc_total * 4, cudaMemcpyDeviceToHost)); o += nc_total;
+    CUDA_TRY(ctx, cudaMemcpy(o, ctx->ntasks.p, (size_t)nc_total * 4, cudaMemcpyDeviceToHost)); o += nc_total;
+    CUDA_TRY(ctx, cudaMemcpy(o, task_off, ((size_t)nc_total + nwin + 1) * 4, cudaMemcpyDeviceToHost)); o += nc_total + nwin + 1;
+    CUDA_TRY(ctx, cudaMemcpy(o, ctx->tasks.p, (size_t)ntask * 8, cudaMemcpyDeviceToHost)); o += 2 * (size_t)ntask;
+    CUDA_TRY(ctx, cudaMemcpy(o, (const uint32_t *)ctx->task_order.p + 3 * TASK_BINS, (size_t)ntask * 4, cudaMemcpyDeviceToHost));
+    o += ntask;
+    CUDA_TRY(ctx, cudaMemcpy(o, heavy + 1, (size_t)nheavy * 4, cudaMemcpyDeviceToHost));
     return 0;
 }
 
diff --git a/curve25519_dalek_b200/engine.py b/curve25519_dalek_b200/engine.py
--- a/curve25519_dalek_b200/engine.py
+++ b/curve25519_dalek_b200/engine.py
@@ -34,6 +34,7 @@
     lib.dalek_b200_last_kernel_ms.argtypes = [vp, C.POINTER(C.c_float), C.POINTER(C.c_int)]
     lib.dalek_b200_last_call_ms.argtypes = [vp, C.POINTER(C.c_float)]
     lib.dalek_b200_last_stage_ms.argtypes = [vp, C.c_char_p, C.POINTER(C.c_float)]
+    lib.dalek_b200_msm_task_lists.argtypes = [vp, C.POINTER(C.c_uint32), vp]
     for name in ("dalek_b200_edwards_vartime_msm", "dalek_b200_edwards_ct_msm", "dalek_b200_edwards_vartime_msm_dev"):
         getattr(lib, name).argtypes = [vp, vp, vp, C.c_int, sz, vp, vp]
     lib.dalek_b200_msm_window_count.argtypes = [vp, sz]
@@ -191,6 +192,19 @@
         self.lib.dalek_b200_last_kernel_ms(self.h, C.byref(ms), C.byref(n))
         return ms.value, n.value
 
+    def msm_task_lists(self):
+        import numpy as np
+        info = (C.c_uint32 * 5)()
+        self._check(self.lib.dalek_b200_msm_task_lists(self.h, info, None))
+        nwin, nb, task_len, ntask, nheavy = list(info)
+        nbk = nwin * nb
+        buf = np.zeros(3 * nbk + nwin + 1 + 3 * ntask + nheavy, dtype=np.uint32)
+        self._check(self.lib.dalek_b200_msm_task_lists(self.h, info, buf.ctypes.data))
+        cut = np.cumsum([nbk, nbk, nbk, nwin + 1, 2 * ntask, ntask])
+        counts, ntasks, task_off, win_base, tasks, order, heavy = np.split(buf, cut)
+        return {"nwin": nwin, "nb": nb, "task_len": task_len, "counts": counts, "ntasks": ntasks, "task_off": task_off,
+                "win_base": win_base, "tasks": tasks.reshape(-1, 2), "order": order, "heavy": heavy}
+
     def edwards_vartime_msm(self, scalars, points, n, point_fmt=POINTS_COMPRESSED, device_ptrs=False, want_limbs=False):
         out = (C.c_uint8 * 32)()
         limbs = (C.c_uint64 * 20)() if want_limbs else None
diff --git a/include/dalek_b200.h b/include/dalek_b200.h
--- a/include/dalek_b200.h
+++ b/include/dalek_b200.h
@@ -33,6 +33,7 @@
 int dalek_b200_last_kernel_ms(const dalek_b200_ctx *ctx, float *ms, int *launches);
 int dalek_b200_last_stage_ms(const dalek_b200_ctx *ctx, const char *stage, float *ms);
 int dalek_b200_last_call_ms(const dalek_b200_ctx *ctx, float *ms);
+int dalek_b200_msm_task_lists(dalek_b200_ctx *ctx, uint32_t info[5], uint32_t *arrays);
 
 int dalek_b200_edwards_vartime_msm(dalek_b200_ctx *ctx, const uint8_t *scalars, const void *points,
                                    int point_fmt, size_t n, uint8_t out_compressed[32],
```

Result: no change. 372.6 million, median of 6 (-0.6%).
